# RuurdBijlsma/clip-embedder-rs

Measured on AMD Instinct MI355X. Metric: images/sec embedding, ViT-B/32-224 vision tower, batch 256 per GPU, higher is better.
Workload: dtype bf16; 1 GPU; BASELINE.json configs[1]: ViT-B/32-224 VisionEmbedder, batch 256 synthetic 224x224 per GPU, device-resident input; global_batch=256, seq_len=50, parallelism=dp1, 2 concurrent sub-batch lane(s)/GPU (committed MI355X tile table)

## Files before the change

clip-embedder-rs_amd/csrc/engine/api.hip:

```cpp
#include "engine.hpp"

namespace clipgpu {

namespace {

void destroy_engine(clipgpu_engine* e) {
  for (hipEvent_t ev : e->prof.pool) (void)hipEventDestroy(ev);
  destroy_comms(*e);
  for (auto& r : e->reps) destroy_replica(r);
  delete e;
}

std::unique_lock<std::mutex> device_call(clipgpu_engine* e, int tower, int64_t B, const char* null_arg = nullptr) {
  need_tower(e, tower);
  if (B <= 0) throw ClipErr(CLIPGPU_ERR_INVALID, "Empty batch");
  if (B > e->max_batch) throw ClipErr(CLIPGPU_ERR_INVALID, "B exceeds max_batch");
  if (null_arg) throw ClipErr(CLIPGPU_ERR_INVALID, null_arg);
  std::unique_lock<std::mutex> lk(e->mu);
  HIP_CHECK(hipSetDevice(e->reps[0].device));
  return lk;
}

bool file_exists(const std::string& p) {
  struct stat st;
  return ::stat(p.c_str(), &st) == 0 && S_ISREG(st.st_mode);
}

constexpr int kResidualDefault = CLIPGPU_RESIDUAL_F16;

}

}

using namespace clipgpu;

extern "C" {

int clipgpu_abi_version(void) { return CLIPGPU_ABI_VERSION; }

int clipgpu_options_init(clipgpu_options* o) {
  return guarded([&]() {
    if (!o) throw ClipErr(CLIPGPU_ERR_INVALID, "opts is NULL");
    std::memset(o, 0, sizeof(*o));
    o->struct_size = sizeof(*o);
  });
}

int clipgpu_create(const char* model_dir, int tower, const int* device_ids, int n_devices, int dtype, int max_batch,
                   clipgpu_engine** out) {
  return clipgpu_create_ex(model_dir, tower, device_ids, n_devices, dtype, max_batch, nullptr, out);
}

int clipgpu_create_ex(const char* model_dir, int tower, const int* device_ids, int n_devices, int dtype,
                      int max_batch, const clipgpu_options* opts_in, clipgpu_engine** out) {
  return guarded([&]() {
    if (!out) throw ClipErr(CLIPGPU_ERR_INVALID, "out is NULL");
    *out = nullptr;
    clipgpu_options opts;
    std::memset(&opts, 0, sizeof(opts));
    opts.struct_size = sizeof(opts);
    if (opts_in) {
      if (opts_in->struct_size != offsetof(clipgpu_options, graphs) &&
          opts_in->struct_size != offsetof(clipgpu_options, residual) && opts_in->struct_size != sizeof(opts))
        throw ClipErr(CLIPGPU_ERR_INVALID, "clipgpu_options.struct_size: call clipgpu_options_init first");
      std::memcpy(&opts, opts_in, opts_in->struct_size);
    }
    if (opts.mx_sites & ~(CLIPGPU_MX_QKV | CLIPGPU_MX_FC | CLIPGPU_MX_PROJ))
      throw ClipErr(CLIPGPU_ERR_INVALID, "clipgpu_options.mx_sites: unknown bits");
    if (opts.lanes < 0 || opts.lanes > 4) throw ClipErr(CLIPGPU_ERR_INVALID, "clipgpu_options.lanes must be 0..4");
    if (opts.tuning < 0 || opts.tuning > 2) throw ClipErr(CLIPGPU_ERR_INVALID, "clipgpu_options.tuning must be 0, 1 or 2");
    for (int32_t v : {opts.graphs, opts.prune_last, opts.trim_text})
      if (v < -1 || v > 1) throw ClipErr(CLIPGPU_ERR_INVALID, "clipgpu_options graphs / prune_last / trim_text: -1, 0 or 1");
    for (int i = 0; i < 5; ++i) {
      const int t = i < 4 ? opts.gemm_tiles[i] : opts.patch_tile;
      if (t != 0 && t != -1 && !gemm_tile_built(t))
        throw ClipErr(CLIPGPU_ERR_INVALID, "clipgpu_options.gemm_tiles / patch_tile: " + std::to_string(t) +
                                               " is not a GEMM tile this library builds");
    }
    if (opts.mx_layers != 0 && dtype != CLIPGPU_DTYPE_FP8)
      throw ClipErr(CLIPGPU_ERR_INVALID, "clipgpu_options.mx_layers needs dtype CLIPGPU_DTYPE_FP8");
    if (opts.residual < 0 || opts.residual > CLIPGPU_RESIDUAL_F16)
      throw ClipErr(CLIPGPU_ERR_INVALID, "clipgpu_options.residual must be 0, 1 (f32) or 2 (f16)");
    if (opts.ln_fold < -1 || opts.ln_fold > 1)
      throw ClipErr(CLIPGPU_ERR_INVALID, "clipgpu_options.ln_fold must be -1, 0 or 1");
    if (opts.communicator < 0 || opts.communicator > 1)
      throw ClipErr(CLIPGPU_ERR_INVALID, "clipgpu_options.communicator must be 0 or 1");
    if (!model_dir) throw ClipErr(CLIPGPU_ERR_INVALID, "model_dir is NULL");
    if (tower != CLIPGPU_TOWER_VISION && tower != CLIPGPU_TOWER_TEXT) throw ClipErr(CLIPGPU_ERR_INVALID, "bad tower");
    if (dtype != CLIPGPU_DTYPE_BF16 && dtype != CLIPGPU_DTYPE_F16 && dtype != CLIPGPU_DTYPE_FP8)
      throw ClipErr(CLIPGPU_ERR_INVALID, "bad dtype");
    if (max_batch <= 0) throw ClipErr(CLIPGPU_ERR_INVALID, "max_batch must be > 0");
    const std::string dir(model_dir);
    struct stat st;
    if (::stat(dir.c_str(), &st) != 0 || !S_ISDIR(st.st_mode))
      throw ClipErr(CLIPGPU_ERR_CONFIG, "Model folder not found: '" + dir + "'");
    for (const char* f : {"open_clip_config.json", "model_config.json"})
      if (!file_exists(dir + "/" + f))
        throw ClipErr(CLIPGPU_ERR_CONFIG, std::string("Missing model file '") + f + "' in folder '" + dir + "'");
    OpenClipConfig oc;
    try {
      oc = load_open_clip_config(dir + "/open_clip_config.json");
    } catch (const std::runtime_error& ex) {
      throw ClipErr(CLIPGPU_ERR_CONFIG, ex.what());
    }
    std::unique_ptr<clipgpu_engine, void (*)(clipgpu_engine*)> e(new clipgpu_engine(), destroy_engine);
    e->spec = tower == CLIPGPU_TOWER_VISION ? oc.vision : oc.text;
    e->pre = oc.pre;
    e->dt = dtype == CLIPGPU_DTYPE_F16 ? DT_F16 : DT_BF16;
    e->mx = dtype == CLIPGPU_DTYPE_FP8;
    if (e->mx) {
      const uint32_t bits = opts.mx_sites ? opts.mx_sites : (CLIPGPU_MX_QKV | CLIPGPU_MX_FC | CLIPGPU_MX_PROJ);
      e->mx_site[GS_QKV] = (bits & CLIPGPU_MX_QKV) != 0;
      e->mx_site[GS_FC] = (bits & CLIPGPU_MX_FC) != 0;
      e->mx_site[GS_PROJ] = (bits & CLIPGPU_MX_PROJ) != 0;
      if (e->mx_site[GS_PROJ] && !e->mx_site[GS_FC])
        throw ClipErr(CLIPGPU_ERR_INVALID, "MX sites: proj in MX needs fc in MX");
      if (e->spec.layers < 32 && (opts.mx_layers >> e->spec.layers) != 0)
        throw ClipErr(CLIPGPU_ERR_INVALID, "clipgpu_options.mx_layers: bit set at or beyond the tower's " +
                                               std::to_string(e->spec.layers) + " layers");
      e->mx_layers = opts.mx_layers ? (uint64_t)opts.mx_layers : ~0ull;
    } else if (opts.mx_sites) {
      throw ClipErr(CLIPGPU_ERR_INVALID, "clipgpu_options.mx_sites needs dtype CLIPGPU_DTYPE_FP8");
    }
    e->max_batch = max_batch;
    if (opts.lanes > 0) {
      e->lanes = opts.lanes;
      e->lanes_pinned = true;
    } else {
      e->lanes = 2;
    }
    e->tuning = opts.tuning;
    e->dev_lanes = e->lanes;
    e->graphs = opts.graphs != -1;
    e->prune = opts.prune_last != -1;
    e->trim = opts.trim_text != -1;
    {
      const int res = opts.residual ? opts.residual : kResidualDefault;
      const bool f16_ok = e->spec.family != FAMILY_SIGLIP;
      if (opts.residual == CLIPGPU_RESIDUAL_F16 && !f16_ok)
        throw ClipErr(CLIPGPU_ERR_INVALID, "clipgpu_options.residual = f16: CLIP-family engines only");
      e->x16 = res == CLIPGPU_RESIDUAL_F16 && f16_ok;
      const bool fold_ok = e->x16 && !e->mx && (e->spec.act == ACT_QUICK_GELU || e->spec.act == ACT_GELU);
      if (opts.ln_fold == 1 && !fold_ok)
        throw ClipErr(CLIPGPU_ERR_INVALID,
                      "clipgpu_options.ln_fold = 1: needs a bf16 / f16 engine, the f16 residual stream and a "
                      "QuickGELU / GELU MLP");
      e->lnf = fold_ok && opts.ln_fold != -1;
    }
    for (int i = 0; i < 4; ++i) e->pin_tiles[i] = opts.gemm_tiles[i];
    e->pin_patch = opts.patch_tile;
    const TowerSpec& s = e->spec;
    if (!s.unsupported.empty()) throw ClipErr(CLIPGPU_ERR_CONFIG, s.unsupported);
    if (s.heads <= 0 || s.width % s.heads || s.width % 64)
      throw ClipErr(CLIPGPU_ERR_CONFIG, "Configuration error: width must be a multiple of 64 and of heads");
    const int hd = s.width / s.heads;
    if (hd != 64 && hd != 72 && hd != 80)
      throw ClipErr(CLIPGPU_ERR_CONFIG, "Configuration error: head dim " + std::to_string(hd) + " not supported (64, 72, 80)");
    if (s.width > 1280) throw ClipErr(CLIPGPU_ERR_CONFIG, "Configuration error: width > 1280 not supported yet");
    if (e->mx && (s.width % 128 || mlp_pad(s) % 128))
      throw ClipErr(CLIPGPU_ERR_CONFIG, "Configuration error: the fp8 path needs width and MLP width % 128 == 0");
    if (s.tokens() > 1024) throw ClipErr(CLIPGPU_ERR_CONFIG, "Configuration error: > 1024 tokens not supported yet");
    if (s.tower == TOWER_VISION) {
      if (s.image_size % s.patch_size)
        throw ClipErr(CLIPGPU_ERR_CONFIG, "Configuration error: image_size must be a multiple of patch_size");
      e->in_bytes_per_row = (size_t)3 * s.image_size * s.image_size * 4;
    } else {
      e->in_bytes_per_row = (size_t)s.context_length * 8;
    }
    TensorMap m;
    try {
      m = load_tower_weights(dir, s);
    } catch (const std::runtime_error& ex) {
      throw ClipErr(CLIPGPU_ERR_CONFIG, ex.what());
    }
    int ndev = 0;
    HIP_CHECK(hipGetDeviceCount(&ndev));
    std::vector<int> devs;
    if (device_ids && n_devices > 0) devs.assign(device_ids, device_ids + n_devices);
    else devs.push_back(0);
    for (int d : devs)
      if (d < 0 || d >= ndev) throw ClipErr(CLIPGPU_ERR_DEVICE, "device id " + std::to_string(d) + " not available");
    e->reps.resize(devs.size());
    for (size_t i = 0; i < devs.size(); ++i) {
      Replica& r = e->reps[i];
      r.device = devs[i];
      HIP_CHECK(hipSetDevice(r.device));
      HIP_CHECK(hipStreamCreateWithFlags(&r.stream, hipStreamNonBlocking));
      upload_weights(*e, r, m);
      alloc_workspace(*e, r);
      if (i == 0) {
        if (e->tuning) {
          autotune_tiles(*e, r);
          apply_tile_pins(*e);
          tune_forward(*e, r);
        } else {
          table_tiles(*e);
          apply_tile_pins(*e);
        }
      }
    }
// ... 111 lines not shown
```

clip-embedder-rs_amd/csrc/engine/engine.hpp:

```cpp
#pragma once
#include <hip/hip_runtime.h>
#include <rccl/rccl.h>

#include <algorithm>
#include <cstring>
#include <memory>
#include <mutex>
#include <string>
#include <sys/stat.h>
#include <thread>
#include <vector>

#include "../../../include/clipgpu.h"
#include "../../../include/clipgpu_testing.h"
#include "../bounce.hpp"
#include "../hip_check.hpp"
#include "../host/api_util.hpp"
#include "../host/copy_pool.hpp"
#include "../host/json.hpp"
#include "../host/model.hpp"
#include "../host/resize_plan.hpp"
#include "../kernels/common.hpp"
#include "../kernels/kernels.hpp"


namespace clipgpu {

struct MxW {
  uint8_t* q = nullptr;
  uint8_t* s = nullptr;
};

struct LayerW {
  float *ln1_w, *ln1_b, *bqkv, *bo, *ln2_w, *ln2_b, *b1, *b2;
  float *cs_qkv = nullptr, *cs_1 = nullptr;
  void *wqkv, *wo, *w1, *w2;
  MxW mqkv, m1, m2;
};

struct MapHeadW {
  float* q = nullptr;
  void *wkv = nullptr, *wproj = nullptr, *w1 = nullptr, *w2 = nullptr;
  float *bkv = nullptr, *bproj = nullptr, *norm_w = nullptr, *norm_b = nullptr, *b1 = nullptr, *b2 = nullptr;
};

struct DevWeights {
  void* conv_w = nullptr;
  float* conv_b = nullptr;
  MapHeadW map;
  float *cls = nullptr, *pos = nullptr, *lnpre_w = nullptr, *lnpre_b = nullptr;
  float* tok = nullptr;
  std::vector<LayerW> layers;
  float *lnpost_w = nullptr, *lnpost_b = nullptr;
  void* proj_t = nullptr;
  float* proj_b = nullptr;
};

struct HostSet {
  void* in = nullptr;
  void* pin_in = nullptr;
  float* pin_out = nullptr;
  float* out = nullptr;
  hipEvent_t done[4] = {nullptr, nullptr, nullptr, nullptr};
  hipEvent_t copied[4] = {nullptr, nullptr, nullptr, nullptr};
  bool owns_device = false;
};

struct Replica {
  int device = 0;
  hipStream_t stream = nullptr;
  char* arena = nullptr;
  char* work = nullptr;
  DevWeights w;
  void* x = nullptr;
  float* xs = nullptr;
  void* h = nullptr;
  uint8_t* hs = nullptr;
  uint8_t* bigs = nullptr;
  void* big = nullptr;
  void* pooled = nullptr;
  float* emb = nullptr;
  HostSet hset[2];
  hipStream_t lane[4] = {nullptr, nullptr, nullptr, nullptr};
  hipEvent_t fork = nullptr, join[4] = {nullptr, nullptr, nullptr, nullptr};
  hipStream_t copy = nullptr, copy2 = nullptr;
  struct ImageSlot {
    char* pin = nullptr;
    size_t pin_cap = 0;
    char* dev = nullptr;
    size_t dev_cap = 0;
    uint8_t* tmp = nullptr;
    size_t tmp_cap = 0;
  } islot[4];
  struct GraphCache* graphs = nullptr;
  hipEvent_t gin = nullptr, gout = nullptr;
  ncclComm_t comm = nullptr;
  hipEvent_t coll = nullptr;
};

struct GraphCache {
  struct Entry {
    std::vector<uint64_t> key;
    hipGraphExec_t exec;
    uint64_t last_use;
  };
  std::vector<Entry> entries;
  uint64_t clock = 0;
  static constexpr size_t kMax = 32;
  void clear() {
    for (auto& en : entries) (void)hipGraphExecDestroy(en.exec);
    entries.clear();
  }
};

enum ProfCat { PC_PATCH = 0, PC_STEM, PC_QKV, PC_ATTN, PC_OUT_PROJ, PC_LN, PC_C_FC, PC_C_PROJ, PC_HEAD, PC_TAIL, PC_N };
struct Profiler {
  unsigned mask = 0;
  std::vector<hipEvent_t> pool;
  size_t used = 0;
  struct Rec { int cat; hipEvent_t a, b; hipStream_t st; };
  std::vector<Rec> pending;
  double total_ms[PC_N] = {0};
  long long count[PC_N] = {0};
  hipEvent_t get() {
    if (used == pool.size()) {
      hipEvent_t ev;
      if (hipEventCreate(&ev) != hipSuccess) return nullptr;
      pool.push_back(ev);
    }
    return pool[used++];
  }
};

}

struct clipgpu_engine {
  clipgpu::Profiler prof;
  int tile[4] = {0, 0, 0, 0};
  int mxtile[4] = {0, 0, 0, 0};
  int tile_patch = 0;
  int tuned_rows = 0;
  int lanes = 1;
  int dev_lanes = 1;
  bool lanes_pinned = false;
  bool graphs = true;
  bool prune = true;
  bool trim = true;
  bool x16 = false;
  bool lnf = false;

  int tuning = 0;
  int pin_tiles[4] = {0, 0, 0, 0};
  int pin_patch = 0;
  uint64_t mx_layers = ~0ull;
  bool comm_pending = false;
  std::vector<int> comm_devs;
  bool force_bcast = false;
  std::vector<int> host_part;
  bool rgb8_resize_always = false;
  clipgpu::TowerSpec spec;
  clipgpu::PreprocessCfg pre;
  clipgpu::DType dt = clipgpu::DT_BF16;
  bool mx = false;
  bool mx_site[4] = {false, false, false, false};
  int max_batch = 0;
  size_t in_bytes_per_row = 0;
  std::vector<clipgpu::Replica> reps;
  int comm_nranks = 0, comm_rank0 = 0;
  std::mutex mu;
};

#pragma GCC visibility push(hidden)
namespace clipgpu {

enum GemmSite { GS_QKV = 0, GS_OUT, GS_FC, GS_PROJ, GS_N };

inline bool mx_at(const clipgpu_engine& e, int l, int site) {
  return e.mx_site[site] && l >= 0 && l < 64 && ((e.mx_layers >> l) & 1ull);
}

inline size_t align256(size_t n) { return (n + 255) & ~size_t(255); }
inline int round64(int n) { return (n + 63) / 64 * 64; }
inline int mlp_pad(const TowerSpec& s) { return round64(s.mlp_width); }
inline int kpatch(const TowerSpec& s) { return 3 * s.patch_size * s.patch_size; }
inline int kpatch_pad(const TowerSpec& s) { return round64(kpatch(s)); }
inline size_t big_wide(const TowerSpec& s) {
  size_t w = std::max((size_t)3 * s.width, (size_t)mlp_pad(s));
  if (s.tower == TOWER_VISION) {
    const size_t G = (size_t)s.image_size / s.patch_size, T = (size_t)s.tokens();
    w = std::max(w, (G * G * (size_t)kpatch_pad(s) + T - 1) / T);
  }
  return w;
}

inline size_t xbytes(const clipgpu_engine& e) { return e.x16 ? 2 : 4; }
inline void* xrows(const clipgpu_engine& e, void* x, size_t rows) {
  return (char*)x + rows * (size_t)e.spec.width * xbytes(e);
}

enum InKind { IN_F32 = 0, IN_U8 = 1, IN_IDS = 2 };

struct HostRows {
// ... 115 lines not shown
```

clip-embedder-rs_amd/csrc/engine/forward.hip:

```cpp
#include "engine.hpp"

namespace clipgpu {

namespace {

struct ProfScope {
  Profiler* p;
  int cat;
  hipStream_t st;
  bool gemm;
  hipEvent_t a = nullptr, b = nullptr;
  ProfScope(const clipgpu_engine& e, int c, hipStream_t s, bool gemm_scope = false)
      : p(const_cast<Profiler*>(&e.prof)), cat(c), st(s), gemm(gemm_scope) {
    if (p->mask & (1u << cat)) {
      a = p->get();
      b = a ? p->get() : nullptr;
      if (!b) {
        a = nullptr;
      } else if (gemm) {
        g_gemm_events.start = a;
        g_gemm_events.stop = b;
      } else {
        (void)hipEventRecord(a, st);
      }
// ... 7 lines not shown
  }
};

GemmParams rows_gemm(const void* A, long lda, const void* W, const float* bias, void* out, long ldo, int M, int N,
                     int K) {
  GemmParams g{};
  g.A = A;
  g.lda = lda;
  g.W = W;
  g.ldw = K;
  g.bias = bias;
  g.out = out;
  g.ldo = ldo;
  g.M = M;
  g.N = N;
  g.K = K;
  return g;
}

}

SiteShape site_shape(const clipgpu_engine& e, int site) {
  const int D = e.spec.width, MLP = mlp_pad(e.spec);
  switch (site) {
    case GS_QKV: return {3 * D, D};
    case GS_OUT: return {D, D};
    case GS_FC: return {MLP, D};
    default: return {D, MLP};
  }
}

int site_epi(const clipgpu_engine& e, int site) {
  if (site == GS_OUT || site == GS_PROJ) return EPI_RESID;
  return e.lnf ? EPI_LNF : EPI_STORE16;
}

#ifndef CLIPGPU_SITE_GROUPS
#define CLIPGPU_SITE_GROUPS 1
#endif
constexpr int kSiteGroup[4] = {CLIPGPU_SITE_GROUPS ? 1 : 0, 0, 0, CLIPGPU_SITE_GROUPS ? 1 : 0};

GemmParams site_gemm(const clipgpu_engine& e, const Replica& r, const LayerW& L, int site, int rows) {
  const int D = e.spec.width, MLP = mlp_pad(e.spec);
  GemmParams g;
  const void* ln_in = e.lnf ? r.x : r.h;
  switch (site) {
    case GS_QKV: g = rows_gemm(ln_in, D, L.wqkv, L.bqkv, r.big, 3 * D, rows, 3 * D, D); break;
    case GS_OUT: g = rows_gemm(r.h, D, L.wo, L.bo, r.x, D, rows, D, D); break;
    case GS_FC: g = rows_gemm(ln_in, D, L.w1, L.b1, r.big, MLP, rows, MLP, D); break;
    default: g = rows_gemm(r.big, MLP, L.w2, L.b2, r.x, D, rows, D, MLP); break;
  }
  if (e.lnf && (site == GS_QKV || site == GS_FC)) {
    g.cs = site == GS_QKV ? L.cs_qkv : L.cs_1;
    g.rowstats = r.xs;
  }
  g.group = kSiteGroup[site];
  g.x16 = e.x16 ? 1 : 0;
  g.prio = e.spec.tower == TOWER_VISION ? 1 : 0;
  return g;
}

int site_epi_mx(const clipgpu_engine& e, int l, int site) {
  return site == GS_PROJ ? EPI_RESID : (site == GS_FC && mx_at(e, l, GS_PROJ) ? EPI_STOREQ : EPI_STORE16);
}
static inline uint8_t* ln_q(const clipgpu_engine& e, int l, int consumer_site, uint8_t* hs) {
  return mx_at(e, l, consumer_site) ? hs : nullptr;
}

MxGemmParams site_gemm_mx(const clipgpu_engine& e, const Replica& r, const LayerW& L, int site, int rows) {
  const int D = e.spec.width, MLP = mlp_pad(e.spec);
  MxGemmParams g{};
  g.M = rows;
  if (site == GS_PROJ) {
    g.A = (const uint8_t*)r.big; g.lda = MLP; g.As = r.bigs; g.ldas = MLP / 32;
    g.W = L.m2.q; g.ldw = MLP; g.Ws = L.m2.s; g.ldws = MLP / 32;
    g.bias = L.b2; g.out = r.x; g.ldo = D; g.N = D; g.K = MLP;
    g.x16 = e.x16 ? 1 : 0;
    return g;
  }
  g.A = (const uint8_t*)r.h; g.lda = D; g.As = r.hs; g.ldas = D / 32;
  g.K = D;
  if (site == GS_QKV) {
    g.W = L.mqkv.q; g.ldw = D; g.Ws = L.mqkv.s; g.ldws = D / 32;
    g.bias = L.bqkv; g.out = r.big; g.ldo = 3 * D; g.N = 3 * D;
  } else {
    g.W = L.m1.q; g.ldw = D; g.Ws = L.m1.s; g.ldws = D / 32;
    g.bias = L.b1; g.out = r.big; g.ldo = MLP; g.outs = r.bigs; g.ldos = MLP / 32; g.N = MLP;
  }
  return g;
}

#ifdef CLIPGPU_ABLATE
unsigned g_ablate = 0;
#define ABLATED(bit) ((g_ablate >> (bit)) & 1u)
extern "C" int clipgpu_test_ablate(unsigned mask) {
  g_ablate = mask;
  return 0;
}
#else
#define ABLATED(bit) false
#endif

namespace {

struct PoolSrc {
  const void* x;
  int tokens;
  const int64_t* ids;
};

inline size_t prune_off_x(const TowerSpec& s, int B) { return align256((size_t)B * mlp_pad(s) * 2); }
inline size_t prune_off_h(const TowerSpec& s, int B) {
  return prune_off_x(s, B) + align256((size_t)B * s.width * 4);
}
inline size_t prune_off_xs(const TowerSpec& s, int B) {
  return prune_off_h(s, B) + align256((size_t)B * s.width * 2);
}
inline bool prune_last(const clipgpu_engine& e, int B, int T) {
  const TowerSpec& s = e.spec;
  return e.prune && s.family != FAMILY_SIGLIP && s.layers > 0 &&
         prune_off_xs(s, B) + ((size_t)B + 256) * 8 <= (size_t)B * T * big_wide(s) * 2;
}

PoolSrc trunk(const clipgpu_engine& e, const Replica& r, int B, int causal, const int64_t* ids, hipStream_t st,
              int T, int pool_pos = 0) {
  const TowerSpec& s = e.spec;
  const int D = s.width;
  const bool prune = prune_last(e, B, T);
  for (int l = 0; l < s.layers; ++l) {
    const LayerW& L = r.w.layers[l];
    const bool compact = prune && l + 1 == s.layers;
    Replica c = r;
    int rows = B * T;
    auto gemm = [&](int site, int cat, const char* what) {
      if (ABLATED(site == GS_QKV ? 3 : site == GS_OUT ? 2 : site == GS_FC ? 4 : 5)) return;
      ProfScope ps(e, rows == B * T ? cat : PC_TAIL, st, true);
      const bool tuned = 2 * rows > e.tuned_rows;
      if (mx_at(e, l, site)) {
        MxGemmParams g = site_gemm_mx(e, c, L, site, rows);
        g.tile = tuned ? e.mxtile[site] : MX_TILE_AUTO;
        check(launch_gemm_mx(e.dt, site_epi_mx(e, l, site), site == GS_FC ? s.act : ACT_NONE, g, st), what);
        return;
      }
      GemmParams g = site_gemm(e, c, L, site, rows);
      g.tile = tuned ? e.tile[site] : TILE_AUTO;
      check(launch_gemm(e.dt, A_ROWS, site_epi(e, site), site == GS_FC ? s.act : ACT_NONE, g, st), what);
    };
    gemm(GS_QKV, PC_QKV, "qkv gemm");
    if (!ABLATED(1)) { ProfScope ps(e, PC_ATTN, st);
      check(launch_attention(e.dt, r.big, r.h, B, T, s.heads, D, causal, st), "attention"); }
    if (compact) {
      c.x = (char*)r.big + prune_off_x(s, B);
      c.h = (char*)r.big + prune_off_h(s, B);
      c.xs = (float*)((char*)r.big + prune_off_xs(s, B));
      rows = B;
      ProfScope ps(e, PC_TAIL, st);
      check(launch_gather_pooled(xrows(e, r.x, pool_pos), e.x16, (char*)r.h + (size_t)pool_pos * D * 2, ids, T, c.x, c.h,
                                 B, D, st),
            "gather pooled rows");
    }
    gemm(GS_OUT, PC_OUT_PROJ, "out_proj gemm");
    if (!ABLATED(0)) {
      ProfScope ps(e, compact ? PC_TAIL : PC_LN, st);
      if (e.lnf)
        check(launch_ln_stats(c.x, 1, s.ln_eps, c.xs, rows, D, st), "ln_2 statistics");
      else
        check(launch_ln_rows(e.dt, c.x, e.x16, L.ln2_w, L.ln2_b, s.ln_eps, c.h, rows, D, st, ln_q(e, l, GS_FC, c.hs)),
              "ln_2");
    }
    gemm(GS_FC, PC_C_FC, "c_fc gemm");
    gemm(GS_PROJ, PC_C_PROJ, "c_proj gemm");
    if (l + 1 < s.layers && !ABLATED(0)) {
      ProfScope ps(e, PC_LN, st);
      if (e.lnf)
        check(launch_ln_stats(r.x, 1, s.ln_eps, r.xs, rows, D, st), "ln_1 statistics");
      else
        check(launch_ln_rows(e.dt, r.x, e.x16, r.w.layers[l + 1].ln1_w, r.w.layers[l + 1].ln1_b, s.ln_eps, r.h, rows,
                             D, st, ln_q(e, l + 1, GS_QKV, r.hs)),
              "ln_1");
    }
    if (compact) return PoolSrc{c.x, 1, nullptr};
  }
  return PoolSrc{xrows(e, r.x, pool_pos), T, ids};
}

void head(const clipgpu_engine& e, const Replica& r, int B, const PoolSrc& src, float* d_out, hipStream_t st) {
  const TowerSpec& s = e.spec;
  const int D = s.width, E = s.embed_dim;
  ProfScope ps(e, PC_HEAD, st);
  check(launch_pool_ln(e.dt, src.x, e.x16, src.ids, src.tokens, r.w.lnpost_w, r.w.lnpost_b, s.ln_eps, r.pooled, B, D,
                       st),
        "pool+ln");
  check(launch_gemm(e.dt, A_ROWS, EPI_STORE32, ACT_NONE, rows_gemm(r.pooled, D, r.w.proj_t, r.w.proj_b, r.emb, E, B, E, D),
                    st),
        "proj gemm");
  check(launch_l2norm(r.emb, d_out, B, E, st), "l2norm");
}

void head_map(const clipgpu_engine& e, const Replica& r, int B, float* d_out, hipStream_t st) {
  const TowerSpec& s = e.spec;
  const int D = s.width, T = s.tokens(), M = mlp_pad(s);
  const MapHeadW& mw = r.w.map;
  ProfScope ps(e, PC_HEAD, st);
  check(launch_ln_rows(e.dt, r.x, 0, r.w.lnpost_w, r.w.lnpost_b, s.ln_eps, r.h, B * T, D, st), "norm");
  check(launch_gemm(e.dt, A_ROWS, EPI_STORE16, ACT_NONE, rows_gemm(r.h, D, mw.wkv, mw.bkv, r.big, 2 * D, B * T, 2 * D, D),
                    st), "attn_pool kv gemm");
  check(launch_map_attention(e.dt, mw.q, r.big, r.pooled, B, T, s.heads, D, st), "attn_pool attention");
  check(launch_gemm(e.dt, A_ROWS, EPI_STORE32, ACT_NONE, rows_gemm(r.pooled, D, mw.wproj, mw.bproj, r.x, D, B, D, D), st),
        "attn_pool proj gemm");
  check(launch_ln_rows(e.dt, r.x, 0, mw.norm_w, mw.norm_b, s.ln_eps, r.h, B, D, st), "attn_pool norm");
  check(launch_gemm(e.dt, A_ROWS, EPI_STORE16, s.act, rows_gemm(r.h, D, mw.w1, mw.b1, r.big, M, B, M, D), st),
        "attn_pool fc1 gemm");
  check(launch_gemm(e.dt, A_ROWS, EPI_RESID, ACT_NONE, rows_gemm(r.big, M, mw.w2, mw.b2, r.x, D, B, D, M), st),
        "attn_pool fc2 gemm");
  check(launch_l2norm((const float*)r.x, d_out, B, D, st), "l2norm");
}

}

GemmParams patch_gemm(const clipgpu_engine& e, const Replica& r, int rows) {
  const TowerSpec& s = e.spec;
  const int Kp = kpatch_pad(s);
  GemmParams g = rows_gemm(r.big, Kp, r.w.conv_w, r.w.conv_b, r.x, s.width, rows, s.width, Kp);
  g.G = s.grid();
  g.pos = r.w.pos;
  g.cls = s.cls() ? 1 : 0;
  g.x16 = e.x16 ? 1 : 0;
  return g;
}

void vision_forward(const clipgpu_engine& e, const Replica& r, const void* pixels, int asrc, const float* mean,
                    const float* stdv, int B, float* d_out, hipStream_t st) {
  const TowerSpec& s = e.spec;
  const int D = s.width, G = s.grid(), P = s.patch_size, Kp = kpatch_pad(s);
  { ProfScope ps(e, PC_PATCH, st);
    check(launch_patch_rows(e.dt, asrc, pixels, mean, stdv, r.big, B, s.image_size, P, kpatch(s), Kp, st),
          "patch rows");
    GemmParams g = patch_gemm(e, r, B * G * G);
    g.tile = 2 * B * s.tokens() > e.tuned_rows ? e.tile_patch : TILE_AUTO;
    check(launch_gemm(e.dt, A_ROWS, EPI_PATCH, ACT_NONE, g, st), "patch gemm"); }
  if (s.family == FAMILY_SIGLIP) {
    { ProfScope ps(e, PC_STEM, st);
      check(launch_ln_rows(e.dt, r.x, e.x16, r.w.layers[0].ln1_w, r.w.layers[0].ln1_b, s.ln_eps, r.h, B * s.tokens(), D, st,
                           ln_q(e, 0, GS_QKV, r.hs)),
            "ln_1"); }
    trunk(e, r, B, 0, nullptr, st, s.tokens());
    head_map(e, r, B, d_out, st);
    return;
  }
  {
  ProfScope ps(e, PC_STEM, st);
  check(launch_vision_embed_ln(e.dt, r.x, e.x16, r.w.cls, r.w.pos, r.w.lnpre_w, r.w.lnpre_b, r.w.layers[0].ln1_w,
                               r.w.layers[0].ln1_b, s.ln_eps, e.lnf ? nullptr : r.h, B, s.tokens(), D, st,
                               ln_q(e, 0, GS_QKV, r.hs), r.xs),
        "embed+ln_pre");
  }
  head(e, r, B, trunk(e, r, B, 0, nullptr, st, s.tokens()), d_out, st);
}

void text_forward(const clipgpu_engine& e, const Replica& r, const int64_t* d_ids, int B, float* d_out,
                  hipStream_t st, int T) {
  const TowerSpec& s = e.spec;
  if (T <= 0) T = s.context_length;
  {
  ProfScope ps(e, PC_STEM, st);
  check(launch_text_embed_ln(e.dt, d_ids, r.w.tok, r.w.pos, r.w.layers[0].ln1_w, r.w.layers[0].ln1_b, s.ln_eps,
                             r.x, e.x16, e.lnf ? nullptr : r.h, B, T, s.width, s.vocab_size, st,
                             ln_q(e, 0, GS_QKV, r.hs), r.xs),
        "token embed+ln_1");
  }
  head(e, r, B, trunk(e, r, B, s.causal ? 1 : 0, s.pool_last ? nullptr : d_ids, st, T, s.pool_last ? T - 1 : 0),
       d_out, st);
}

Replica lane_view(const clipgpu_engine& e, const Replica& r, int b0) {
  const TowerSpec& s = e.spec;
  const size_t rows = (size_t)b0 * s.tokens(), D = s.width;
  const size_t wide = big_wide(s);
  Replica v = r;
  v.x = (char*)r.x + rows * D * xbytes(e);
  v.xs = r.xs + rows * 2;
  v.h = (char*)r.h + rows * D * 2;
  v.big = (char*)r.big + rows * wide * 2;
  if (r.hs) v.hs = r.hs + rows * D / 32;
  if (r.bigs) v.bigs = r.bigs + rows * (size_t)mlp_pad(s) / 32;
  v.pooled = (char*)r.pooled + (size_t)b0 * D * 2;
  v.emb = r.emb + (size_t)b0 * s.embed_dim;
  return v;
}

namespace {

inline void lane_range(int B, int lanes, int i, int& b0, int& b1) {
  b0 = (int)((long)B * i / lanes);
  b1 = (int)((long)B * (i + 1) / lanes);
}

inline int lanes_for(const clipgpu_engine& e, int B) {
  return B < 8 * e.dev_lanes ? 1 : e.dev_lanes;
}

template <typename F>
void run_lanes(const clipgpu_engine& e, const Replica& r, int B, hipStream_t st, F fwd) {
  const int L = lanes_for(e, B);
  const bool serial = e.prof.mask != 0 && !(e.prof.mask & CLIPGPU_PROFILE_CONCURRENT);
  if (L == 1 || serial) {
    for (int i = 0; i < L; ++i) {
      int b0, b1;
      lane_range(B, L, i, b0, b1);
      fwd(lane_view(e, r, b0), b0, b1 - b0, st);
    }
    return;
  }
  HIP_CHECK(hipEventRecord(r.fork, st));
  for (int i = 0; i < L; ++i) {
    int b0, b1;
    lane_range(B, L, i, b0, b1);
    HIP_CHECK(hipStreamWaitEvent(r.lane[i], r.fork, 0));
    fwd(lane_view(e, r, b0), b0, b1 - b0, r.lane[i]);
    HIP_CHECK(hipEventRecord(r.join[i], r.lane[i]));
  }
  for (int i = 0; i < L; ++i) HIP_CHECK(hipStreamWaitEvent(st, r.join[i], 0));
}

}

void vision_forward_lanes(const clipgpu_engine& e, const Replica& r, const void* pixels, int asrc, const float* mean,
                          const float* stdv, int B, float* d_out, hipStream_t st) {
  const size_t S = e.spec.image_size;
  const size_t row_bytes = 3 * S * S * (asrc == A_IMG_F32 ? 4 : 1);
  const int E = e.spec.embed_dim;
  run_lanes(e, r, B, st, [&](const Replica& v, int b0, int n, hipStream_t ls) {
    vision_forward(e, v, (const char*)pixels + b0 * row_bytes, asrc, mean, stdv, n, d_out + (size_t)b0 * E, ls);
  });
// ... 12 lines not shown
```

clip-embedder-rs_amd/csrc/engine/weights.hip:

```cpp
#include "engine.hpp"

namespace clipgpu {

namespace {

const HostTensor& need(const TensorMap& m, const std::string& k) {
  auto it = m.find(k);
  if (it == m.end()) throw ClipErr(CLIPGPU_ERR_CONFIG, "Configuration error: missing tensor " + k);
  return it->second;
}

struct Bump {
  char* base;
  size_t off = 0;
  size_t cap;
  void* take(size_t n) {
    void* p = base + off;
    off += align256(n);
    if (off > cap) throw ClipErr(CLIPGPU_ERR_DEVICE, "internal: arena overflow");
    return p;
  }
};

size_t weight_bytes(const TowerSpec& s, const TensorMap& m) {
// ... 189 lines not shown
    w.layers.push_back(L);
  }
  if (siglip) {
    const std::string t = "visual.trunk.", a = "visual.trunk.attn_pool.";
    w.lnpost_w = f32(t + "norm.weight");
    w.lnpost_b = f32(t + "norm.bias");
    {
      const HostTensor& lat = need(m, a + "latent");
      const HostTensor& wq = need(m, a + "q.weight");
      const HostTensor& bq = need(m, a + "q.bias");
      std::vector<float> q((size_t)D);
      for (int j = 0; j < D; ++j) {
        double acc = bq.data[(size_t)j];
        for (int i = 0; i < D; ++i) acc += (double)lat.data[(size_t)i] * wq.data[(size_t)j * D + i];
        q[(size_t)j] = (float)acc;
      }
      w.map.q = (float*)a_take_f32(q);
    }
    w.map.wkv = w16(a + "kv.weight");
    w.map.bkv = f32(a + "kv.bias");
    w.map.wproj = w16(a + "proj.weight");
    w.map.bproj = f32(a + "proj.bias");
    w.map.norm_w = f32(a + "norm.weight");
    w.map.norm_b = f32(a + "norm.bias");
    w.map.w1 = w16_pad(a + "mlp.fc1.weight", mlp_pad(s), D);
    w.map.b1 = f32_pad(a + "mlp.fc1.bias", mlp_pad(s));
    w.map.w2 = w16_pad(a + "mlp.fc2.weight", D, mlp_pad(s));
    w.map.b2 = f32(a + "mlp.fc2.bias");
  } else if (s.tower == TOWER_VISION) {
    w.lnpost_w = f32("visual.ln_post.weight");
    w.lnpost_b = f32("visual.ln_post.bias");
    w.proj_t = w16_transposed("visual.proj");
  } else {
    w.lnpost_w = f32("ln_final.weight");
    w.lnpost_b = f32("ln_final.bias");
    if (s.proj_bias) {
      w.proj_t = w16("text_projection.weight");
      w.proj_b = f32("text_projection.bias");
    } else {
      w.proj_t = w16_transposed("text_projection");
    }
  }
}

void alloc_workspace(clipgpu_engine& e, Replica& r) {
  const TowerSpec& s = e.spec;
  const size_t B = (size_t)((e.max_batch + e.lanes - 1) / e.lanes * e.lanes);
  const size_t rows = B * (size_t)s.tokens(), D = s.width;
  const size_t wide = big_wide(s);
  const size_t E = s.embed_dim;
  const size_t MLP = (size_t)mlp_pad(s);
  const size_t sizes[] = {rows * D * 4, rows * D * 2, rows * wide * 2, B * D * 2, B * E * 4, B * E * 4,
                          B * e.in_bytes_per_row, e.mx ? rows * D / 32 : 0, e.mx ? rows * MLP / 32 : 0,
                          (rows + 256) * 8};
  size_t total = 0;
  for (size_t z : sizes) total += align256(z);
  HIP_CHECK(hipMalloc(&r.work, total));
  HIP_CHECK(hipMemset(r.work, 0, total));
  Bump a{r.work, 0, total};
  r.x = a.take(sizes[0]);
  r.h = a.take(sizes[1]);
  r.big = a.take(sizes[2]);
  r.pooled = a.take(sizes[3]);
  r.emb = (float*)a.take(sizes[4]);
  HostSet& hs = r.hset[0];
  hs.out = (float*)a.take(sizes[5]);
  hs.in = a.take(sizes[6]);
  r.hs = e.mx ? (uint8_t*)a.take(sizes[7]) : nullptr;
  r.bigs = e.mx ? (uint8_t*)a.take(sizes[8]) : nullptr;
  r.xs = (float*)a.take(sizes[9]);
  for (int i = 0; i < e.lanes; ++i) {
    HIP_CHECK(hipStreamCreateWithFlags(&r.lane[i], hipStreamNonBlocking));
    HIP_CHECK(hipEventCreateWithFlags(&r.join[i], hipEventDisableTiming));
  }
  for (int i = 0; i < 4; ++i) {
    HIP_CHECK(hipEventCreateWithFlags(&hs.done[i], hipEventDisableTiming));
    HIP_CHECK(hipEventCreateWithFlags(&hs.copied[i], hipEventDisableTiming));
  }
  HIP_CHECK(hipStreamCreateWithFlags(&r.copy, hipStreamNonBlocking));
  HIP_CHECK(hipStreamCreateWithFlags(&r.copy2, hipStreamNonBlocking));
  HIP_CHECK(hipEventCreateWithFlags(&r.fork, hipEventDisableTiming));
  HIP_CHECK(hipEventCreateWithFlags(&r.gin, hipEventDisableTiming));
  HIP_CHECK(hipEventCreateWithFlags(&r.gout, hipEventDisableTiming));
  r.graphs = new GraphCache();
  HIP_CHECK(hipHostMalloc(&hs.pin_in, B * e.in_bytes_per_row, hipHostMallocDefault));
  HIP_CHECK(hipHostMalloc((void**)&hs.pin_out, B * E * 4, hipHostMallocDefault));
}

void destroy_replica(Replica& r) {
  if (!r.stream) return;
  (void)hipSetDevice(r.device);
  (void)hipDeviceSynchronize();
  if (r.arena) (void)hipFree(r.arena);
  if (r.work) (void)hipFree(r.work);
  for (HostSet& hs : r.hset) {
    if (hs.pin_in) (void)hipHostFree(hs.pin_in);
    if (hs.pin_out) (void)hipHostFree(hs.pin_out);
    if (hs.owns_device && hs.in) (void)hipFree(hs.in);
    if (hs.owns_device && hs.out) (void)hipFree(hs.out);
  }
  if (r.stream) (void)hipStreamDestroy(r.stream);
  if (r.copy) (void)hipStreamDestroy(r.copy);
  if (r.copy2) (void)hipStreamDestroy(r.copy2);
  for (int i = 0; i < 4; ++i) {
    if (r.lane[i]) (void)hipStreamDestroy(r.lane[i]);
    if (r.join[i]) (void)hipEventDestroy(r.join[i]);
    for (HostSet& hs : r.hset) {
      if (hs.done[i]) (void)hipEventDestroy(hs.done[i]);
      if (hs.copied[i]) (void)hipEventDestroy(hs.copied[i]);
    }
  }
  if (r.fork) (void)hipEventDestroy(r.fork);
  if (r.gin) (void)hipEventDestroy(r.gin);
  if (r.gout) (void)hipEventDestroy(r.gout);
  if (r.coll) (void)hipEventDestroy(r.coll);
  if (r.graphs) {
    r.graphs->clear();
    delete r.graphs;
  }
  for (auto& sl : r.islot) {
    if (sl.pin) (void)hipHostFree(sl.pin);
    if (sl.dev) (void)hipFree(sl.dev);
    if (sl.tmp) (void)hipFree(sl.tmp);
// ... 6 lines not shown
```

clip-embedder-rs_amd/csrc/kernels/common.hpp:

```cpp
#pragma once
#include <hip/hip_runtime.h>
#include <stdint.h>

namespace clipgpu {

typedef float f32x4 __attribute__((ext_vector_type(4)));
typedef float f32x16 __attribute__((ext_vector_type(16)));
typedef __bf16 bf16x8 __attribute__((ext_vector_type(8)));
typedef _Float16 f16x8 __attribute__((ext_vector_type(8)));
typedef __bf16 bf16x4 __attribute__((ext_vector_type(4)));
typedef _Float16 f16x4 __attribute__((ext_vector_type(4)));

template <typename T> struct Vec8;
template <> struct Vec8<__bf16> { typedef bf16x8 type; };
template <> struct Vec8<_Float16> { typedef f16x8 type; };
template <typename T> struct Vec4;
template <> struct Vec4<__bf16> { typedef bf16x4 type; };
template <> struct Vec4<_Float16> { typedef f16x4 type; };

__device__ __forceinline__ float4 ldx4(const float* p) { return *(const float4*)p; }
__device__ __forceinline__ float4 ldx4(const _Float16* p) {
  const f16x4 h = *(const f16x4*)p;
  return make_float4((float)h[0], (float)h[1], (float)h[2], (float)h[3]);
}
// ... 37 lines not shown
  return e < 127 ? __uint_as_float((uint32_t)(127 - e) << 23) : __uint_as_float(0x00400000u);
}
__device__ __forceinline__ uint32_t mx_pack4(float a, float b, float c, float d, float inv) {
  int w = __builtin_amdgcn_cvt_pk_fp8_f32(a * inv, b * inv, 0, false);
  w = __builtin_amdgcn_cvt_pk_fp8_f32(c * inv, d * inv, w, true);
  return (uint32_t)w;
}

template <int CTRL>
__device__ __forceinline__ float dpp_f32(float v) {
  return __builtin_bit_cast(float, __builtin_amdgcn_update_dpp(0, __builtin_bit_cast(int, v), CTRL, 0xF, 0xF, false));
}
__device__ __forceinline__ float row16_sum(float v) {
  v += dpp_f32<0x128>(v);
  v += dpp_f32<0x124>(v);
  v += dpp_f32<0x122>(v);
  v += dpp_f32<0x121>(v);
  return v;
}
__device__ __forceinline__ float row16_max(float v) {
  v = fmaxf(v, dpp_f32<0x128>(v));
  v = fmaxf(v, dpp_f32<0x124>(v));
  v = fmaxf(v, dpp_f32<0x122>(v));
  v = fmaxf(v, dpp_f32<0x121>(v));
  return v;
}
__device__ __forceinline__ void swap16(float& a, float& b) {
  asm volatile("s_nop 1\n\tv_permlane16_swap_b32 %0, %1" : "+v"(a), "+v"(b));
}
__device__ __forceinline__ void swap32(float& a, float& b) {
  asm volatile("s_nop 1\n\tv_permlane32_swap_b32 %0, %1" : "+v"(a), "+v"(b));
}
__device__ __forceinline__ float xsum16(float v) {
  float a = v, b = v;
  swap16(a, b);
  return a + b;
}
__device__ __forceinline__ float xsum32(float v) {
  float a = v, b = v;
  swap32(a, b);
  return a + b;
}
__device__ __forceinline__ float xmax16(float v) {
  float a = v, b = v;
  swap16(a, b);
  return fmaxf(a, b);
}
__device__ __forceinline__ float xmax32(float v) {
  float a = v, b = v;
  swap32(a, b);
  return fmaxf(a, b);
}
__device__ __forceinline__ float wave_sum(float v) { return xsum32(xsum16(row16_sum(v))); }
__device__ __forceinline__ float wave_max(float v) { return xmax32(xmax16(row16_max(v))); }
__device__ __forceinline__ float group16_sum(float v) { return row16_sum(v); }
__device__ __forceinline__ float group16_max(float v) { return row16_max(v); }

typedef float f32x2 __attribute__((ext_vector_type(2)));
__device__ __forceinline__ float lnf_out(float acc, float mean, float rstd, float cs, float bias) {
  return fmaf(fmaf(-mean, cs, acc), rstd, bias);
}

enum Act { ACT_NONE = 0, ACT_QUICK_GELU = 1, ACT_GELU = 2, ACT_GELU_TANH = 3 };

__device__ __forceinline__ float fast_sigmoid_mul(float x, float z) {
  return x * __builtin_amdgcn_rcpf(1.0f + __expf(-z));
}
__device__ __forceinline__ float sigmoid_mul_exp2(float x, float t) {
  return x * __builtin_amdgcn_rcpf(1.0f + __builtin_amdgcn_exp2f(t));
}
__device__ __forceinline__ float fast_erf(float x) {
  const float ax = fabsf(x);
  const float t = __builtin_amdgcn_rcpf(fmaf(0.3275911f, ax, 1.0f));
  float p = fmaf(1.061405429f, t, -1.453152027f);
  p = fmaf(p, t, 1.421413741f);
  p = fmaf(p, t, -0.284496736f);
  p = fmaf(p, t, 0.254829592f);
  const float y = 1.0f - p * t * __expf(-ax * ax);
  return copysignf(y, x);
}

template <int ACT>
__device__ __forceinline__ float apply_act(float x) {
#ifdef CLIPGPU_TEST_NO_ACT
  return x;
#endif
  if constexpr (ACT == ACT_QUICK_GELU) {
    return sigmoid_mul_exp2(x, x * -2.4554669596f);
  } else if constexpr (ACT == ACT_GELU) {
    return 0.5f * x * (1.0f + fast_erf(x * 0.70710678118654752f));
  } else if constexpr (ACT == ACT_GELU_TANH) {
    const float k0 = 0.7978845608028654f, k1 = 0.044715f;
    return fast_sigmoid_mul(x, 2.0f * k0 * fmaf(k1 * x, x * x, x));
  } else {
    return x;
  }
}

__device__ __forceinline__ int xcd_remap(int pid, int nwg) {
  const int xcd = pid & 7, q = nwg >> 3, r = nwg & 7;
  const int start = xcd < r ? xcd * (q + 1) : r * (q + 1) + (xcd - r) * q;
  return start + (pid >> 3);
}

}
```

clip-embedder-rs_amd/csrc/kernels/gemm.hip:

```cpp
#include <algorithm>
#include <cstdlib>
#include <type_traits>
#include <utility>

#include <hip/hip_ext.h>

#include "common.hpp"
#include "kernels.hpp"
#include "gemm_util.hpp"

namespace clipgpu {

thread_local GemmLaunchEvents g_gemm_events;

#ifdef CLIPGPU_GEMM_STAMPS
constexpr int kStampBlocks = 2048, kStampSlots = 64;
__device__ unsigned long long g_gemm_stamps[kStampBlocks * kStampSlots];
#define GEMM_STAMP(slot)                                                                        \
  do {                                                                                          \
    if (threadIdx.x == 0 && blockIdx.x < kStampBlocks && (slot) < kStampSlots)                   \
      g_gemm_stamps[blockIdx.x * kStampSlots + (slot)] = __builtin_amdgcn_s_memtime();        \
  } while (0)
#define GEMM_STAMP_REAL(slot)                                                                   \
  do {                                                                                          \
// ... 36 lines not shown
#define CLIPGPU_GEMM_SPREAD_ALL 0
#endif
#ifndef CLIPGPU_GEMM_NONPERSIST
#define CLIPGPU_GEMM_NONPERSIST 0
#endif
#ifndef CLIPGPU_GEMM_EPI_DMA_WAIT
#define CLIPGPU_GEMM_EPI_DMA_WAIT 1
#endif

template <typename T>
__device__ __forceinline__ T to16(float v) { return (T)v; }
__device__ __forceinline__ float4 widen4(float4 v) { return v; }
__device__ __forceinline__ float4 widen4(f16x4 h) { return make_float4((float)h[0], (float)h[1], (float)h[2], (float)h[3]); }

template <int NW, int OCC>
struct PipeBounds {
  static constexpr int waves_per_eu = NW == 8 && OCC >= 2 ? 4 : 2;
};

template <typename T, int BM, int BN, int WGM, int WGN, int EPI, int ACT, int NS = 2, int OCC = 2, int RS = 0,
          int HM = 0>
__global__ __launch_bounds__(WGM* WGN * 64, (PipeBounds<WGM * WGN, OCC>::waves_per_eu)) void gemm_pipe_kernel(
    GemmParams p) {
  typedef typename Vec8<T>::type V8;
  constexpr bool LNF = epi_lnf(EPI);
  static_assert(!LNF || std::is_same<T, _Float16>::value, "LayerNorm fold: f16 operands");
  typedef typename std::conditional<EPI == EPI_LNF_BF, __bf16, T>::type OT;
  constexpr int SROWP = LNF ? (BM * 8 + 1023) / 1024 * 1024 : 0;
  constexpr int EXTRA = LNF ? 4096 + 2 * SROWP : 2048;
  constexpr int NW = WGM * WGN;
  constexpr int A_BYTES = BM * BK * 2, B_BYTES = BN * BK * 2, STAGE = A_BYTES + B_BYTES;
  constexpr int PW = BN / 8, PA = BM / 8, PT = PW + PA;
  constexpr int NP = (PT + NW - 1) / NW;
  constexpr bool EVEN = PT % NW == 0;
  constexpr bool WSPLIT = PW % NW == 0;
  constexpr int TM = BM / WGM, TN = BN / WGN, MI = TM / 16, NI = TN / 16;
  constexpr int LG = NI == 2 ? 1 : NI == 4 ? 2 : 3;
  constexpr int NG = MI;
  constexpr bool SPREAD = MI * NI >= 32 || (CLIPGPU_GEMM_SPREAD_W8 && NW == 8 && OCC < 2) || CLIPGPU_GEMM_SPREAD_ALL;
  (void)LG;
  static_assert(BM % 8 == 0 && BN % 8 == 0 && MI >= 1 && BN <= 256 && PT >= NW, "bad tile");
  static_assert(NI == 2 || NI == 3 || NI == 4 || NI == 6 || NI == 8, "column permutation: NI in {2,3,4,6,8}");
  static_assert(NS == 2 || NS == 3, "2 or 3 LDS stages");
  __shared__ __attribute__((aligned(16))) char smem[NS * STAGE + EXTRA];

  const int tid = threadIdx.x;
  const int lane = tid & 63;
  const int wave = __builtin_amdgcn_readfirstlane(tid >> 6);
  const int lda_i = (int)p.lda, ldw_i = (int)p.ldw, nb = gridDim.x;
  const char* const Ab = (const char*)p.A;
  const char* const Wb = (const char*)p.W;
  const float* const bias_p = p.bias;
  const float* const cs_p = p.cs;
  const float* const rs_p = p.rowstats;
  asm volatile("" ::"s"(lda_i), "s"(ldw_i), "s"(nb), "s"(Ab), "s"(Wb), "s"(bias_p));
  if constexpr (LNF) asm volatile("" ::"s"(cs_p), "s"(rs_p));
  const int nTn = (p.N + BN - 1) / BN;
  const int grp = p.group > 0 ? p.group : CLIPGPU_TILE_GROUP;
  asm volatile("" ::"s"(grp));
  const int nTm = (p.M + BM - 1) / BM;
  const int ntiles = nTn * nTm;
  const int nk = p.K / BK;

  static_assert(!HM || (NS == 2 && WGM == 2), "half tiles: 2 x N waves, 2-stage schedule");
  int t_first, t_stride, t_end;
  int hm_F = 0, hm_start = 0, hm_nbx = 1, hm_j = 0;
  if constexpr (HM) {
    const int x = blockIdx.x & 7, nbx = nb >> 3, j = blockIdx.x >> 3;
    const int q = ntiles >> 3, r = ntiles & 7;
    hm_start = x < r ? x * (q + 1) : r * (q + 1) + (x - r) * q;
    const int cnt = q + (x < r ? 1 : 0);
    hm_F = cnt / nbx;
    hm_nbx = nbx;
    hm_j = j;
    t_first = 0;
    t_stride = 1;
    t_end = hm_F + (j < 2 * (cnt % nbx) ? 1 : 0);
  } else if (nb % 8 == 0 && nb < ntiles) {
    const int x = blockIdx.x & 7, nbx = nb >> 3;
    const int q = ntiles >> 3, r = ntiles & 7;
    const int start = x < r ? x * (q + 1) : r * (q + 1) + (x - r) * q;
    t_first = start + (blockIdx.x >> 3);
    t_stride = nbx;
    t_end = start + q + (x < r ? 1 : 0);
  } else {
    t_first = xcd_remap(blockIdx.x, nb);
    t_stride = ntiles;
    t_end = t_first + 1;
  }
  if (t_first >= t_end) return;
  const int total = ((t_end - t_first + t_stride - 1) / t_stride) * nk;
  auto unit_coords = [&](int u, int& m0, int& n0) {
    if constexpr (HM) {
      if (u < hm_F) {
        tile_coords(hm_start + hm_j + u * hm_nbx, nTm, nTn, BM, BN, m0, n0, grp);
      } else {
        tile_coords(hm_start + hm_F * hm_nbx + (hm_j >> 1), nTm, nTn, BM, BN, m0, n0, grp);
        m0 += (hm_j & 1) * (BM / 2);
      }
      return;
    }
    tile_coords(u, nTm, nTn, BM, BN, m0, n0, grp);
  };

  auto swW = [](int r) {
    if constexpr (NI == 3 || NI == 6) {
      const int j = (r % (16 * NI)) / (4 * NI);
      return ((j == 1 || j == 2) ? 1 : 0) ^ (2 * j + ((r & 3) >> 1));
    } else {
// ... 3 lines not shown

  uint32_t poff[NP];
  auto piece_is_w = [&](int i, int q) { return WSPLIT ? (i < PW / NW) : (q < PW); };
  auto set_tile = [&](int m0, int n0) {
#pragma unroll
    for (int i = 0; i < NP; ++i) {
      const int q = wave + NW * i;
      if (!EVEN && q >= PT) {
        poff[i] = 0;
      } else if (piece_is_w(i, q)) {
        const int r = q * 8 + (lane >> 3);
        const int c = (lane & 7) ^ swW(r);
        poff[i] = (uint32_t)(min(n0 + r, p.N - 1) * ldw_i + c * 8) * 2u;
      } else {
        const int r = (q - PW) * 8 + (lane >> 3);
        const int c = (lane & 7) ^ ((r >> 1) & 7);
        poff[i] = (uint32_t)(min(m0 + r, p.M - 1) * lda_i + c * 8) * 2u;
      }
    }
  };
  int d_g = 0, d_kt = 0, d_t = t_first, d_n0 = 0, d_m0 = 0, d_ti = 0;
  {
    int m0, n0;
    unit_coords(d_t, m0, n0);
    set_tile(m0, n0);
    d_n0 = n0;
    d_m0 = m0;
  }
  const bool last_piece = EVEN || wave < PT % NW;
  int d_stage = 0;
  auto dma_piece = [&](auto ic) {
    constexpr int i = decltype(ic)::value;
    if constexpr (!EVEN && i == NP - 1) {
      if (!last_piece) return;
    }
#ifdef CLIPGPU_GEMM_STAMPS
    if (p.diag & 4) return;
#endif
    const int q = wave + NW * i;
    const bool w = piece_is_w(i, q);
    char* const dst = smem + d_stage * STAGE + (w ? A_BYTES + q * 1024 : (q - PW) * 1024);
    const char* const src = (w ? Wb : Ab) + (size_t)d_kt * (BK * 2);
    GEMM_POISON(dst);
    glds16(src + poff[i], dst);
  };
  auto dma_bias = [&]() {
    if (bias_p != nullptr && wave == 0 && d_kt == 0) {
      const int n = min(d_n0 + lane * 4, ((p.N - 1) / 4) * 4);
      GEMM_POISON(smem + NS * STAGE + (d_ti & 1) * 1024);
      glds16(bias_p + n, smem + NS * STAGE + (d_ti & 1) * 1024);
      if constexpr (LNF) {
        GEMM_POISON(smem + NS * STAGE + 2048 + (d_ti & 1) * 1024);
        glds16(cs_p + n, smem + NS * STAGE + 2048 + (d_ti & 1) * 1024);
        char* const sst = smem + NS * STAGE + 4096 + (d_ti & 1) * SROWP;
#pragma unroll
        for (int i = 0; i < SROWP / 1024; ++i) {
          GEMM_POISON(sst + i * 1024);
          glds16(rs_p + (size_t)d_m0 * 2 + i * 256 + lane * 4, sst + i * 1024);
        }
      }
    }
  };
  auto dma_advance = [&]() {
    ++d_g;
    if (++d_stage == NS) d_stage = 0;
    if (++d_kt == nk) {
      d_kt = 0;
      d_t += t_stride;
      ++d_ti;
      if (d_t < t_end) {
        int m0, n0;
        unit_coords(d_t, m0, n0);
        set_tile(m0, n0);
        d_n0 = n0;
        d_m0 = m0;
      }
    }
  };
  auto dma_step = [&]() {
    if (d_g < total) {
      static_for<NP>([&](auto j) { dma_piece(j); });
      dma_bias();
    }
    dma_advance();
  };

  const int wm = (wave / WGN) * TM, wn = (wave % WGN) * TN;
  const int fr = lane & 15, fq = lane >> 4;
  uint32_t offA[2], offB[2];
  {
    const int rowB = wn + (fr >> 2) * (4 * NI) + (fr & 3);
#pragma unroll
    for (int kk = 0; kk < 2; ++kk) {
      offA[kk] = (uint32_t)((wm + fr) * 128 + (((kk * 4 + fq) ^ (fr >> 1)) << 4));
      offB[kk] = (uint32_t)(A_BYTES + rowB * 128 + (((kk * 4 + fq) ^ swW(rowB)) << 4));
    }
  }
  int wm_cur = wm, mi_lim = MI;
  uint32_t offA_cur[2] = {offA[0], offA[1]};
  auto set_layout = [&](int u) {
    if constexpr (HM) {
      const bool half = u >= hm_F;
      wm_cur = half ? (wave / WGN) * (TM / 2) : wm;
      mi_lim = half ? MI / 2 : MI;
#pragma unroll
      for (int kk = 0; kk < 2; ++kk) offA_cur[kk] = offA[kk] - (uint32_t)((wm - wm_cur) * 128);
    }
    (void)u;
  };
  const uint32_t lds0 = lds_addr(smem);
  f32x4 acc[NI][MI];
  V8 a0[MI], b0[NI], a1[MI], b1[NI];

  auto rd_b = [&](auto kc, V8(&b)[NI], uint32_t buf, int kk) {
    constexpr int k = decltype(kc)::value;
    ds_read_b128<k * 512>(b[k], buf + offB[kk]);
  };
  auto rd_a = [&](auto kc, V8(&a)[MI], uint32_t buf, int kk) {
    constexpr int k = decltype(kc)::value;
    ds_read_b128<k * 2048>(a[k], buf + offA_cur[kk]);
  };
  auto read_b = [&](V8(&b)[NI], uint32_t buf, int kk) { static_for<NI>([&](auto k) { rd_b(k, b, buf, kk); }); };
  auto read_a = [&](V8(&a)[MI], uint32_t buf, int kk) { static_for<MI>([&](auto k) { rd_a(k, a, buf, kk); }); };
  constexpr int NR = NI + MI, RG = RS ? (NG > 2 ? NG - 2 : 1) : NG, RPG = (NR + RG - 1) / RG;
  auto read_k = [&](auto kc, V8(&a)[MI], V8(&b)[NI], uint32_t buf, int kk) {
    constexpr int k = decltype(kc)::value;
    if constexpr (k < NI) rd_b(kc, b, buf, kk);
    else rd_a(std::integral_constant<int, k - NI>{}, a, buf, kk);
  };
  auto reads_after_group = [&](auto gc, V8(&a)[MI], V8(&b)[NI], uint32_t buf, int kk) {
    static_for<RPG>([&](auto j) {
      constexpr int k = (int)decltype(gc)::value * RPG + (int)decltype(j)::value;
      if constexpr ((int)decltype(gc)::value < RG && k < NR) read_k(std::integral_constant<int, k>{}, a, b, buf, kk);
    });
  };
  auto mfma_group = [&](auto gc, V8(&a)[MI], V8(&b)[NI], auto zero) {
    constexpr int g = decltype(gc)::value;
    constexpr bool Z = decltype(zero)::value;
    if (!HM || g < mi_lim) {
#pragma unroll
      for (int ni = 0; ni < NI; ++ni)
        acc[ni][g] = mfma_16x16x32(b[ni], a[g], Z ? f32x4{0.f, 0.f, 0.f, 0.f} : acc[ni][g]);
    }
  };
  auto phase0 = [&](auto zero, uint32_t buf) {
    if constexpr (!RS) read_b(b1, buf, 1);
    static_for<NG>([&](auto g) {
      mfma_group(g, a0, b0, zero);
      __builtin_amdgcn_sched_barrier(0);
      if constexpr (RS) {
        reads_after_group(g, a1, b1, buf, 1);
        __builtin_amdgcn_sched_barrier(0);
      } else {
        rd_a(g, a1, buf, 1);
      }
    });
    lgkm_wait_all(a1, b1);
  };
  auto phase1 = [&](bool next, uint32_t nbuf) {
    const bool dma = d_g < total;
    (void)next;
    if constexpr (!RS) read_b(b0, nbuf, 0);
    if (dma) {
      dma_bias();
      if constexpr (!SPREAD) static_for<NP>([&](auto j) { dma_piece(j); });
    }
    static_for<NG>([&](auto g) {
      mfma_group(g, a1, b1, std::false_type{});
      __builtin_amdgcn_sched_barrier(0);
      if constexpr (RS) reads_after_group(g, a0, b0, nbuf, 0);
      else rd_a(g, a0, nbuf, 0);
      if constexpr (SPREAD) {
        static_for<NP>([&](auto j) {
          if constexpr (((int)j * NG) / NP == (int)g) {
            if (dma) dma_piece(j);
          }
        });
      }
      __builtin_amdgcn_sched_barrier(0);
    });
    dma_advance();
    lgkm_wait_all(a0, b0);
  };

  auto epilogue = [&](int m0, int n0, int bpar) {
    typedef typename std::conditional<epi_x16(EPI), _Float16, float>::type XE;
    const int nc = n0 + wn + fq * (4 * NI);
    const bool nfull = nc + 4 * NI <= p.N;
    f32x4 bias[NI], csv[NI];
    constexpr bool RST_ALL = MI * NI < 32;
    f32x2 rst[RST_ALL ? MI : 1];
    const uint32_t rst_a = lds0 + NS * STAGE + 4096 + bpar * SROWP + (wm_cur + fr) * 8;
#pragma unroll
    for (int ni = 0; ni < NI; ++ni) bias[ni] = f32x4{0.f, 0.f, 0.f, 0.f};
    if (bias_p != nullptr) {
      const uint32_t ba = lds0 + NS * STAGE + bpar * 1024 + (wn + fq * (4 * NI)) * 4;
      static_for<NI>([&](auto ni) { ds_read_b128<(int)ni * 16>(bias[ni], ba); });
      if constexpr (LNF) {
        static_for<NI>([&](auto ni) { ds_read_b128<2048 + (int)ni * 16>(csv[ni], ba); });
        if constexpr (RST_ALL) static_for<MI>([&](auto mi) { ds_read_b64<(int)mi * 128>(rst[mi], rst_a); });
      }
      asm volatile("s_waitcnt lgkmcnt(0)" ::: "memory");
#pragma unroll
      for (int ni = 0; ni < NI; ++ni) asm volatile("" : "+v"(bias[ni]));
      if constexpr (LNF) {
#pragma unroll
        for (int ni = 0; ni < NI; ++ni) asm volatile("" : "+v"(csv[ni]));
        if constexpr (RST_ALL) {
#pragma unroll
          for (int mi = 0; mi < MI; ++mi) asm volatile("" : "+v"(rst[mi]));
        }
      }
    }
    constexpr bool ADDX = epi_resid(EPI) || epi_patch(EPI);
    const int G2 = p.G * p.G;
    auto out_row = [&](int m) -> long {
// ... 42 lines not shown
        if constexpr (RST_ALL) {
          rs = rst[mi];
        } else {
          asm volatile("ds_read_b64 %0, %1\n\ts_waitcnt lgkmcnt(0)" : "=v"(rs) : "v"(rst_a + (uint32_t)mi * 128) : "memory");
        }
      }
      float v[NI][4];
#pragma unroll
      for (int ni = 0; ni < NI; ++ni)
#pragma unroll
        for (int j = 0; j < 4; ++j)
          v[ni][j] = LNF ? lnf_out(acc[ni][mi][j], rs[0], rs[1], csv[ni][j], bias[ni][j])
                         : acc[ni][mi][j] + bias[ni][j];
#ifdef CLIPGPU_GEMM_STAMPS
      if (p.diag & 1) {
        float s = 0.f;
#pragma unroll
        for (int ni = 0; ni < NI; ++ni)
#pragma unroll
          for (int j = 0; j < 4; ++j) s += EPI == EPI_STORE16 ? (float)to16<T>(apply_act<ACT>(v[ni][j])) : v[ni][j];
        if (s == 12345.678f) ((float*)p.out)[0] = s;
        continue;
      }
#endif
      if constexpr (epi_st16(EPI)) {
        OT* o = (OT*)p.out + (long)m * p.ldo + nc;
        if (nfull) {
          if constexpr (NI % 2 == 0) {
#pragma unroll
            for (int h = 0; h < NI / 2; ++h) {
              typename Vec8<OT>::type w;
#pragma unroll
              for (int e = 0; e < 8; ++e) w[e] = to16<OT>(apply_act<ACT>(v[2 * h + e / 4][e % 4]));
              *(typename Vec8<OT>::type*)(o + h * 8) = w;
            }
          } else {
#pragma unroll
            for (int ni = 0; ni < NI; ++ni) {
              typename Vec4<OT>::type w;
#pragma unroll
              for (int j = 0; j < 4; ++j) w[j] = to16<OT>(apply_act<ACT>(v[ni][j]));
              *(typename Vec4<OT>::type*)(o + ni * 4) = w;
            }
          }
        } else {
#pragma unroll
          for (int ni = 0; ni < NI; ++ni)
#pragma unroll
            for (int j = 0; j < 4; ++j)
              if (nc + ni * 4 + j < p.N) o[ni * 4 + j] = to16<OT>(apply_act<ACT>(v[ni][j]));
        }
      } else {
        XE* o = (XE*)p.out + out_row(m) + nc;
        if (nfull) {
#pragma unroll
          for (int ni = 0; ni < NI; ++ni) {
            float4 w = make_float4(v[ni][0], v[ni][1], v[ni][2], v[ni][3]);
            if constexpr (ADDX) {
              const float4 x = widen4(xr[XALL ? mi : mi % XR][ni]);
              w.x += x.x; w.y += x.y; w.z += x.z; w.w += x.w;
            }
            stx4(o + ni * 4, w);
          }
        } else {
#pragma unroll
          for (int ni = 0; ni < NI; ++ni)
#pragma unroll
            for (int j = 0; j < 4; ++j) {
              if (nc + ni * 4 + j >= p.N) continue;
              float r = v[ni][j];
              if constexpr (ADDX) r += (float)add_src(m)[ni * 4 + j];
              o[ni * 4 + j] = (XE)r;
            }
        }
      }
    }
  };
  constexpr int EPI_VM = epi_st16(EPI) ? (NI % 2 ? MI * NI : MI * NI / 2)
                                            : ((epi_resid(EPI) || epi_patch(EPI)) ? 2 * MI * NI : MI * NI);
  auto vm_wait_step = [&](auto xc) {
    constexpr int X = decltype(xc)::value;
    if (EVEN || wave < PT % NW) vm_wait<(NP + X < 63 ? NP + X : 63)>();
    else vm_wait<(NP - 1 + X < 63 ? NP - 1 + X : 63)>();
  };

  GEMM_STAMP_REAL(62);
  GEMM_STAMP_HWID();
  GEMM_STAMP(0);
  if constexpr (NW == 8) {
    if (p.prio && wave >= NW / 2) __builtin_amdgcn_s_setprio(1);
  }
  dma_step();
  vm_wait<0>();
  __builtin_amdgcn_s_barrier();
  dma_step();
  if constexpr (NS == 3) dma_step();
  read_b(b0, lds0, 0);
  read_a(a0, lds0, 0);
  lgkm_wait_all(a0, b0);
  GEMM_STAMP(1);

  int g = 0;
  int gs = 0;
  bool after_full_epi = false;
  int ti = 0;
  for (int t = t_first; t < t_end; t += t_stride, ++ti) {
    int m0, n0;
    unit_coords(t, m0, n0);
    GEMM_STAMP(2 + ti * 4);
    for (int kt = 0; kt < nk; ++kt, ++g) {
      if (kt + 1 == nk) GEMM_STAMP(3 + ti * 4);
      const int gs1 = gs + 1 == NS ? 0 : gs + 1;
      const uint32_t buf = lds0 + gs * STAGE;
      if (kt == 0) phase0(std::true_type{}, buf);
      else phase0(std::false_type{}, buf);
      constexpr int EW = EPI_VM < 63 ? EPI_VM : 63;
      if (NS == 3 && g + 2 < total) {
        if (after_full_epi) vm_wait_step(std::integral_constant<int, EPI_VM>{});
        else vm_wait_step(std::integral_constant<int, 0>{});
      } else {
#if CLIPGPU_GEMM_POISON_SELFTEST
        (void)EW;
#else
        if (after_full_epi) vm_wait<EW>();
        else vm_wait<0>();
#endif
      }
      after_full_epi = false;
#ifdef CLIPGPU_GEMM_STAMPS
      if (!(p.diag & 8)) __builtin_amdgcn_s_barrier();
#else
      __builtin_amdgcn_s_barrier();
#endif
      phase1(kt + 1 < nk, lds0 + gs1 * STAGE);
      gs = gs1;
      if (ti == 0 && kt + 1 < nk && 34 + kt < 61) GEMM_STAMP(34 + kt);
    }
    GEMM_STAMP(4 + ti * 4);
#if CLIPGPU_GEMM_EPI_DMA_WAIT
    if constexpr (NS == 3) vm_wait_step(std::integral_constant<int, 0>{});
    else vm_wait<0>();
#endif
    epilogue(m0, n0, ti & 1);
    after_full_epi = m0 + BM <= p.M && n0 + BN <= p.N && (!HM || t < hm_F);
    if (!after_full_epi) vm_wait<0>();
    if (t + t_stride < t_end) {
      const uint32_t buf = lds0 + gs * STAGE;
      set_layout(t + t_stride);
      read_b(b0, buf, 0);
      read_a(a0, buf, 0);
      lgkm_wait_all(a0, b0);
    }
    GEMM_STAMP(5 + ti * 4);
  }
  GEMM_STAMP_REAL(63);
}

constexpr int pipe_kocc(int NW, int OCC) { return NW == 8 ? (OCC >= 2 ? 2 : 1) : 2; }
inline int pipe_grid(int BM, int BN, int NW, int OCC, int M, int N) {
  const int ntiles = ((N + BN - 1) / BN) * ((M + BM - 1) / BM);
  const int lds = 2 * (BM + BN) * BK * 2 + 2048;
  const int per_cu = std::max(1, std::min(NW == 8 ? pipe_kocc(NW, OCC) : OCC, (160 * 1024) / lds));
  const int resident = device_cus() * per_cu;
  if (CLIPGPU_GEMM_NONPERSIST) return ntiles;
  return ntiles <= resident ? ntiles : resident;
}
inline bool half_round_applies(int M, int N) {
  const int nb = device_cus();
  const int ntiles = ((N + 255) / 256) * ((M + 255) / 256);
  bool ok = nb % 8 == 0 && ntiles % nb != 0;
  const int nbx = nb >> 3, q = ntiles >> 3, r = ntiles & 7;
  for (int x = 0; ok && x < 8; ++x) {
    const int cnt = q + (x < r ? 1 : 0);
    ok = cnt >= nbx && 2 * (cnt % nbx) <= nbx;
  }
  return ok;
}
inline int grid_224(int M, int N) { return std::min(((N + 191) / 192) * ((M + 223) / 224), device_cus()); }

template <typename T, int BM, int BN, int WGM, int WGN, int EPI, int ACT, int OCC = 3, int RS = 0>
hipError_t launch_pipe(const GemmParams& p, hipStream_t s) {
// ... 29 lines not shown
  static_assert(!LNF || std::is_same<T, _Float16>::value, "LayerNorm fold: f16 operands");
  static_assert(!epi_patch(EPI), "the patch GEMM always has K >= 128 (pipelined tiles)");
  typedef typename std::conditional<EPI == EPI_LNF_BF, __bf16, T>::type OT;
  const int lane = threadIdx.x & 63;
  const long wid = (long)blockIdx.x * 4 + (threadIdx.x >> 6);
  const int nTn = GEN ? (p.N + 15) >> 4 : p.N >> 4;
  const long tm = wid / nTn;
  const int tn = (int)(wid - tm * nTn);
  if (tm * 16 >= p.M) return;
  const int fr = lane & 15, fq = lane >> 4;
  const int m = (int)tm * 16 + fr;
  const T* a = (const T*)p.A + (long)min(m, p.M - 1) * p.lda + fq * 8;
  const T* w = (const T*)p.W + (long)(GEN ? min(tn * 16 + fr, p.N - 1) : tn * 16 + fr) * p.ldw + fq * 8;
  const int nc = p.K >> 5;
  V8 w0[U], a0[U], w1[U], a1[U], w2[U], a2[U];
  auto load = [&](V8(&wv)[U], V8(&av)[U], int c) {
#pragma unroll
    for (int u = 0; u < U; ++u) {
      wv[u] = *(const V8*)(w + (c + u) * 32);
      av[u] = *(const V8*)(a + (c + u) * 32);
    }
  };
  load(w0, a0, 0);
  if (U < nc) load(w1, a1, U);
  f32x4 acc = {0.f, 0.f, 0.f, 0.f};
  for (int c0 = 0; c0 < nc; c0 += U) {
    if (c0 + 2 * U < nc) load(w2, a2, c0 + 2 * U);
#pragma unroll
    for (int u = 0; u < U; ++u) acc = mfma_16x16x32(w0[u], a0[u], acc);

#pragma unroll
    for (int u = 0; u < U; ++u) {
      w0[u] = w1[u];
      a0[u] = a1[u];
      w1[u] = w2[u];
      a1[u] = a2[u];
    }
  }
  if (m >= p.M) return;
  const int n = tn * 16 + fq * 4;
  if (GEN && n >= p.N) return;
  const bool vec = !GEN || (n + 4 <= p.N && p.ldo % 4 == 0);
  f32x4 bias = {0.f, 0.f, 0.f, 0.f}, csv = {0.f, 0.f, 0.f, 0.f};
  f32x2 rst = {0.f, 0.f};
  if (p.bias != nullptr) {
    if (!GEN || n + 4 <= p.N) bias = *(const f32x4*)(p.bias + n);
    else
      for (int j = 0; j < 4; ++j) bias[j] = n + j < p.N ? p.bias[n + j] : 0.f;
  }
  if constexpr (LNF) {
    if (!GEN || n + 4 <= p.N) csv = *(const f32x4*)(p.cs + n);
    else
      for (int j = 0; j < 4; ++j) csv[j] = n + j < p.N ? p.cs[n + j] : 0.f;
    rst = *(const f32x2*)(p.rowstats + (long)m * 2);
  }
  float v[4];
#pragma unroll
  for (int j = 0; j < 4; ++j) v[j] = LNF ? lnf_out(acc[j], rst[0], rst[1], csv[j], bias[j]) : acc[j] + bias[j];
  if constexpr (epi_st16(EPI)) {
    OT* o = (OT*)p.out + (long)m * p.ldo + n;
    if (vec) {
      typename Vec4<OT>::type ov;
#pragma unroll
      for (int j = 0; j < 4; ++j) ov[j] = to16<OT>(apply_act<ACT>(v[j]));
      *(typename Vec4<OT>::type*)o = ov;
    } else {
      for (int j = 0; j < 4; ++j)
        if (n + j < p.N) o[j] = to16<OT>(apply_act<ACT>(v[j]));
    }
  } else {
    typedef typename std::conditional<epi_x16(EPI), _Float16, float>::type XE;
    XE* o = (XE*)p.out + (long)m * p.ldo + n;
    if (vec) {
      float4 r = make_float4(v[0], v[1], v[2], v[3]);
      if constexpr (epi_resid(EPI)) {
        const float4 x = ldx4(o);
        r.x += x.x; r.y += x.y; r.z += x.z; r.w += x.w;
      }
      stx4(o, r);
    } else {
      for (int j = 0; j < 4; ++j) {
        if (n + j >= p.N) continue;
        float r = v[j];
        if constexpr (epi_resid(EPI)) r += (float)o[j];
        o[j] = (XE)r;
      }
    }
  }
}

inline bool skinny_ok(const GemmParams& p) {
  return p.M > 0 && p.M <= SKINNY_MAX_M && p.N % 16 == 0 && p.K % (32 * SKINNY_U) == 0 && p.lda % 8 == 0 &&
         p.ldw % 8 == 0 && p.ldo % 4 == 0;
}
inline bool general_ok(const GemmParams& p) { return p.lda % 8 == 0 && p.ldw % 8 == 0; }
inline long skinny_waves(int M, int N) { return (long)((M + 15) / 16) * ((N + 15) / 16); }

template <typename T, int EPI, int ACT, int U = SKINNY_U, int GEN = 0>
hipError_t launch_skinny(const GemmParams& p, hipStream_t s) {
  const long blocks = (skinny_waves(p.M, p.N) + 3) / 4;
  if (blocks > 0x7fffffffL) return hipErrorInvalidValue;
  gemm_launch(gemm_skinny_kernel<T, EPI, ACT, U, GEN>, (int)blocks, 256, s, p);
  return hipGetLastError();
}

template <typename T, int EPI, int ACT>
hipError_t launch_tile(const GemmParams& p, hipStream_t s) {
  if constexpr (!epi_patch(EPI)) {
    if ((p.tile == TILE_AUTO || p.tile == TILE_SKINNY) && skinny_ok(p)) return launch_skinny<T, EPI, ACT>(p, s);
  }
  if (p.tile == TILE_SKINNY) return hipErrorInvalidValue;
  const int tile = p.tile == TILE_AUTO ? pick_gemm_tile(p.M, p.N, p.K) : p.tile;
  if (tile != TILE_GENERAL && !gemm_tile_built(tile)) return hipErrorInvalidValue;
  const bool pipe = tile != TILE_GENERAL && p.K >= 2 * BK && (!epi_st16(EPI) || p.ldo % 8 == 0);
  if (!pipe) {
    if constexpr (epi_patch(EPI)) {
      return hipErrorInvalidValue;
    } else {
      if (!general_ok(p)) return hipErrorInvalidValue;
      return launch_skinny<T, EPI, ACT, 2, 1>(p, s);
    }
  }
  if constexpr (epi_lnf(EPI)) {
    switch (tile) {
      case TILE_256x128: return launch_pipe<T, 256, 128, 4, 2, EPI, ACT>(p, s);
      case TILE_256x256: return launch_pipe<T, 256, 256, 2, 4, EPI, ACT>(p, s);
      case TILE_192x256_W8: return launch_pipe<T, 192, 256, 2, 4, EPI, ACT, 1>(p, s);
      case TILE_256x256_RS: return launch_pipe<T, 256, 256, 2, 4, EPI, ACT, 3, 1>(p, s);
      case TILE_160x128_RS: return launch_pipe<T, 160, 128, 2, 2, EPI, ACT, 3, 1>(p, s);
      case TILE_160x128_W8_RS: return launch_pipe<T, 160, 128, 2, 4, EPI, ACT, 2, 1>(p, s);
      case TILE_256x256_HALF: return launch_pipe_half<T, EPI, ACT>(p, s);
      case TILE_224x192_W8: return launch_pipe<T, 160, 128, 2, 2, EPI, ACT, 3, 1>(p, s);
      default: break;
    }
  } else {
    switch (tile) {
      case TILE_256x128: return launch_pipe<T, 256, 128, 4, 2, EPI, ACT>(p, s);
      case TILE_256x256: return launch_pipe<T, 256, 256, 2, 4, EPI, ACT>(p, s);
      case TILE_192x256_W8: return launch_pipe<T, 192, 256, 2, 4, EPI, ACT, 1>(p, s);
      case TILE_256x256_RS: return launch_pipe<T, 256, 256, 2, 4, EPI, ACT, 3, 1>(p, s);
      case TILE_160x128_RS: return launch_pipe<T, 160, 128, 2, 2, EPI, ACT, 3, 1>(p, s);
      case TILE_160x128_W8_RS: return launch_pipe<T, 160, 128, 2, 4, EPI, ACT, 2, 1>(p, s);
      case TILE_256x256_HALF: return launch_pipe_half<T, EPI, ACT>(p, s);
      case TILE_224x192_W8: return launch_pipe_224<T, EPI, ACT>(p, s);
      default: break;
    }
  }
  return hipErrorInvalidValue;
}

template <typename T>
hipError_t launch_typed(int epi, int act, const GemmParams& p, hipStream_t s) {
  switch (epi) {
    case EPI_STORE16:
      switch (act) {
        case ACT_NONE: return launch_tile<T, EPI_STORE16, ACT_NONE>(p, s);
// ... 46 lines not shown

int gemm_grid(int tile, int M, int N, int K) {
  GemmParams p{};
  p.M = M;
  p.N = N;
  p.K = K;
  p.lda = p.ldw = K;
  p.ldo = N;
  if ((tile == TILE_AUTO || tile == TILE_SKINNY) && skinny_ok(p)) return (int)((skinny_waves(M, N) + 3) / 4);
  if (tile == TILE_AUTO) tile = pick_gemm_tile(M, N, K);
  if (K >= 2 * BK && tile != TILE_GENERAL) {
    switch (tile) {
      case TILE_256x128: return pipe_grid(256, 128, 8, 3, M, N);
      case TILE_256x256: return pipe_grid(256, 256, 8, 3, M, N);
      case TILE_192x256_W8: return pipe_grid(192, 256, 8, 1, M, N);
      case TILE_256x256_RS: return pipe_grid(256, 256, 8, 3, M, N);
      case TILE_160x128_RS: return pipe_grid(160, 128, 4, 3, M, N);
      case TILE_160x128_W8_RS: return pipe_grid(160, 128, 8, 2, M, N);
      case TILE_256x256_HALF: return half_round_applies(M, N) ? device_cus() : pipe_grid(256, 256, 8, 3, M, N);
      case TILE_224x192_W8: return grid_224(M, N);
      default: break;
    }
  }
  return (int)std::min<long>((skinny_waves(M, N) + 3) / 4, 0x7fffffffL);
}

int pick_gemm_tile(int M, int N, int K) {
  (void)K;
  if (M < 2048) return TILE_160x128_RS;
  const int cus = 256;
  auto eff = [&](int bm, int bn) {
    const long tiles = (long)((M + bm - 1) / bm) * ((N + bn - 1) / bn);
    const long rounds = (tiles + cus - 1) / cus;
    return (double)tiles / (double)(rounds * cus);
  };
  return eff(256, 256) >= 0.85 * eff(256, 128) ? TILE_256x256 : TILE_256x128;
}

long g_gemm_chunk_cap = 0;

long gemm_chunk_rows(long lda, int G) {
  long rows = ((1L << 31) - 1) / (2 * lda);
  if (g_gemm_chunk_cap > 0) rows = std::min(rows, g_gemm_chunk_cap);
  rows -= rows % 256;
  if (G > 0) rows -= rows % ((long)G * G);
  return rows;
}

hipError_t launch_dt(DType dt, int epi, int act, const GemmParams& p, hipStream_t s) {
  if (epi == EPI_LNF) return launch_typed<_Float16>(dt == DT_BF16 ? EPI_LNF_BF : EPI_LNF, act, p, s);
  return dt == DT_BF16 ? launch_typed<__bf16>(epi, act, p, s) : launch_typed<_Float16>(epi, act, p, s);
}

hipError_t launch_gemm(DType dt, int asrc, int epi, int act, const GemmParams& p, hipStream_t s) {
  if (p.K % BK != 0 || p.M <= 0 || p.N <= 0) return hipErrorInvalidValue;
  if (epi == EPI_LNF && (p.bias == nullptr || p.cs == nullptr || p.rowstats == nullptr || p.N % 4 != 0))
    return hipErrorInvalidValue;
  if (epi == EPI_LNF_BF) return hipErrorInvalidValue;
  if (p.bias != nullptr && p.N % 4 != 0) return hipErrorInvalidValue;
  if ((long)p.N * p.ldw * 2 >= (1L << 31) || p.lda <= 0) return hipErrorInvalidValue;
  if (asrc != A_ROWS) return hipErrorInvalidValue;
  if ((long)p.M * p.lda * 2 >= (1L << 31) || (g_gemm_chunk_cap > 0 && p.M > g_gemm_chunk_cap)) {
    const int G = epi == EPI_PATCH ? p.G : 0;
    const long chunk = gemm_chunk_rows(p.lda, G);
    if (chunk <= 0) return hipErrorInvalidValue;
    const long osz = (epi_st16(epi) || ((epi == EPI_RESID || epi == EPI_PATCH) && p.x16)) ? 2 : 4;
    for (long m0 = 0; m0 < p.M; m0 += chunk) {
      GemmParams q = p;
      q.M = (int)std::min<long>(chunk, p.M - m0);
      q.A = (const char*)p.A + m0 * p.lda * 2;
      if (epi == EPI_LNF) q.rowstats = p.rowstats + 2 * m0;
      const long orow = G > 0 ? m0 / ((long)G * G) * ((long)G * G + p.cls) : m0;
      q.out = (char*)p.out + orow * p.ldo * osz;
      const hipError_t err = launch_dt(dt, epi, act, q, s);
      if (err != hipSuccess) return err;
    }
    return hipSuccess;
  }
  return launch_dt(dt, epi, act, p, s);
}

#ifdef CLIPGPU_GEMM_STAMPS
hipError_t read_gemm_stamps(unsigned long long* host, int nblocks, bool clear) {
  const size_t n = (size_t)std::min(nblocks, kStampBlocks) * kStampSlots * sizeof(unsigned long long);
  if (clear) {
    static unsigned long long zeros[kStampBlocks * kStampSlots];
    return hipMemcpyToSymbol(HIP_SYMBOL(g_gemm_stamps), zeros, sizeof(zeros));
  }
  return hipMemcpyFromSymbol(host, HIP_SYMBOL(g_gemm_stamps), n);
}
#endif

}
```

clip-embedder-rs_amd/csrc/kernels/kernels.hpp:

```cpp
#pragma once
#include <hip/hip_runtime.h>
#include <stdint.h>

#include <atomic>

namespace clipgpu {

enum DType { DT_BF16 = 0, DT_F16 = 1 };

enum ASrc {
  A_ROWS = 0,
  A_IMG_F32 = 1,
  A_IMG_U8 = 2,
};
enum Epi {
  EPI_STORE16 = 0,
  EPI_RESID = 1,
  EPI_STORE32 = 2,
  EPI_PATCH = 3,
  EPI_STOREQ = 4,
  EPI_RESID16 = 5,
  EPI_PATCH16 = 6,
  EPI_LNF = 7,
  EPI_LNF_BF = 8,
};
constexpr bool epi_resid(int e) { return e == EPI_RESID || e == EPI_RESID16; }
constexpr bool epi_patch(int e) { return e == EPI_PATCH || e == EPI_PATCH16; }
constexpr bool epi_x16(int e) { return e == EPI_RESID16 || e == EPI_PATCH16; }
constexpr bool epi_lnf(int e) { return e == EPI_LNF || e == EPI_LNF_BF; }
constexpr bool epi_st16(int e) { return e == EPI_STORE16 || epi_lnf(e); }

struct GemmParams {
  const void* A; long lda;
  const void* W; long ldw;
  const float* bias;
  void* out; long ldo;
  int M, N, K;
  int G;
  int cls;
  const float* pos;
  int tile;
  int diag;
  int group;
  int prio;
  int x16;
  const float* cs;
  const float* rowstats;
};

enum GemmTile {
  TILE_AUTO = 0,
  TILE_256x128 = 2,
  TILE_256x256 = 3,
  TILE_192x256_W8 = 13,
  TILE_256x256_RS = 14,
  TILE_160x128_RS = 15,
  TILE_160x128_W8_RS = 17,
  TILE_256x256_HALF = 18,
  TILE_224x192_W8 = 26,
  TILE_SKINNY = 100,
  TILE_GENERAL = 101,
};
constexpr int kGemmTiles[] = {TILE_256x128, TILE_256x256, TILE_192x256_W8, TILE_256x256_RS,
                              TILE_160x128_RS, TILE_160x128_W8_RS, TILE_256x256_HALF, TILE_224x192_W8};
inline bool gemm_tile_built(int t) {
  for (int k : kGemmTiles)
    if (k == t) return true;
  return false;
}
int pick_gemm_tile(int M, int N, int K);
extern long g_gemm_chunk_cap;
int gemm_grid(int tile, int M, int N, int K);
int device_cus();

hipError_t launch_gemm(DType dt, int asrc, int epi, int act, const GemmParams& p, hipStream_t s);
struct GemmLaunchEvents {
  hipEvent_t start = nullptr, stop = nullptr;
};
extern thread_local GemmLaunchEvents g_gemm_events;

hipError_t launch_map_attention(DType dt, const float* q, const void* kv, void* out, int B, int N, int H, int D,
                                hipStream_t s);
hipError_t launch_attention(DType dt, const void* qkv, void* out, int B, int N, int H, int D,
                            int causal, hipStream_t s);

hipError_t launch_ln_stats(const void* x, int x16, float eps, float* stats, int rows, int D, hipStream_t s);
hipError_t launch_ln_rows(DType dt, const void* x, int x16, const float* w, const float* b, float eps,
                          void* out16, int rows, int D, hipStream_t s, uint8_t* qs = nullptr);

hipError_t launch_vision_embed_ln(DType dt, void* x, int x16, const float* cls, const float* pos,
                                  const float* lnpre_w, const float* lnpre_b,
                                  const float* ln1_w, const float* ln1_b, float eps,
                                  void* h, int B, int tokens, int D, hipStream_t s, uint8_t* qs = nullptr,
                                  float* stats = nullptr);

hipError_t launch_text_embed_ln(DType dt, const int64_t* ids, const float* tok, const float* pos,
                                const float* ln1_w, const float* ln1_b, float eps, void* x, int x16,
                                void* h, int B, int T, int D, int vocab, hipStream_t s, uint8_t* qs = nullptr,
                                float* stats = nullptr);

hipError_t launch_pool_ln(DType dt, const void* x, int x16, const int64_t* ids, int tokens,
                          const float* w, const float* b, float eps, void* out16, int B, int D,
                          hipStream_t s);

hipError_t launch_gather_pooled(const void* x, int x16, const void* h16, const int64_t* ids, int tokens, void* xc,
                                void* hc16, int B, int D, hipStream_t s);

hipError_t launch_patch_rows(DType dt, int src, const void* img, const float* mean, const float* stdv, void* out,
                             int B, int S, int P, int Kv, int Kp, hipStream_t s);

struct ResizeImage {
  long src, tmp;
  long h_bounds, h_coef;
  long v_bounds, v_coef;
  int W, th, yfirst, h_ksize, v_ksize, need_h, need_v, h_prec, v_prec, pad[3];
};
hipError_t launch_resize(const uint8_t* raw, uint8_t* tmp, const int* ints, const ResizeImage* d_imgs, int n,
                         int max_th, int S, uint8_t* out, hipStream_t s);

enum SimAct { SIM_SOFTMAX = 0, SIM_SIGMOID = 1, SIM_LOGITS = 2 };
hipError_t launch_similarity(const float* img, int ni, const float* txt, int nt, int E, float scale, float bias,
                             int activation, int axis, float* out, hipStream_t s);

constexpr int kTopkMax = 128;
struct TopkPlan { int span_cols, n_spans; };
extern std::atomic<long> g_topk_span_cols;
TopkPlan topk_plan(long N, int q_tiles, int max_blocks);
hipError_t launch_topk(const float* q, int nq, const float* g, int N, int E, float scale, float bias, int k,
                       const TopkPlan& p, void* ws, int64_t* out_idx, float* out_score, hipStream_t s);

hipError_t launch_l2norm(const float* in, float* out, int B, int E, hipStream_t s);

hipError_t launch_cast_f32(DType dt, const float* in, void* out, long n, hipStream_t s);
hipError_t launch_pull_copy(const void* src_mapped, void* dst, size_t bytes, hipStream_t s);

#ifdef CLIPGPU_GEMM_STAMPS
hipError_t read_gemm_stamps(unsigned long long* host, int nblocks, bool clear);
#endif

struct MxGemmParams {
  const uint8_t* A; long lda; const uint8_t* As; long ldas;
  const uint8_t* W; long ldw; const uint8_t* Ws; long ldws;
  const float* bias;
  void* out; long ldo;
  uint8_t* outs; long ldos;
  int M, N, K;
  int tile;
  int x16;
};
enum MxTile {
  MX_TILE_AUTO = 0,
  MX_TILE_256x256 = 1,
// ... 10 lines not shown
```

clip-embedder-rs_amd/csrc/kernels/rowwise.hip:

```cpp
#include <type_traits>

#include "common.hpp"
#include "kernels.hpp"

namespace clipgpu {

namespace {

constexpr int MAXV = 5;

template <int NV>
struct Row {
  float4 v[NV];
};

template <int NV>
__device__ __forceinline__ bool in_row(int i, int lane, int D4) {
  return i + 1 < NV || i * 64 + lane < D4;
}

template <int NV>
__device__ __forceinline__ void load_row(const float* src, int D4, int lane, Row<NV>& r) {
#pragma unroll
  for (int i = 0; i < NV; ++i)
    r.v[i] = in_row<NV>(i, lane, D4) ? ((const float4*)src)[i * 64 + lane] : make_float4(0.f, 0.f, 0.f, 0.f);
}

typedef _Float16 Half4 __attribute__((ext_vector_type(4)));
template <int NV>
__device__ __forceinline__ void load_row(const _Float16* src, int D4, int lane, Row<NV>& r) {
#pragma unroll
  for (int i = 0; i < NV; ++i) {
    if (in_row<NV>(i, lane, D4)) {
      const Half4 h = ((const Half4*)src)[i * 64 + lane];
      r.v[i] = make_float4((float)h[0], (float)h[1], (float)h[2], (float)h[3]);
    } else {
      r.v[i] = make_float4(0.f, 0.f, 0.f, 0.f);
    }
  }
}

template <int NV>
__device__ __forceinline__ void ln_stats_regs(const Row<NV>& in, float eps, int D, int lane, float& mean_out,
                                              float& rstd_out) {
  const int D4 = D >> 2;
  float s = 0.f;
#pragma unroll
  for (int i = 0; i < NV; ++i) s += in.v[i].x + in.v[i].y + in.v[i].z + in.v[i].w;
  const float mean = wave_sum(s) / (float)D;
  float q = 0.f;
#pragma unroll
  for (int i = 0; i < NV; ++i) {
    if (in_row<NV>(i, lane, D4)) {
      const float a = in.v[i].x - mean, bb = in.v[i].y - mean, cc = in.v[i].z - mean, d = in.v[i].w - mean;
      q += a * a + bb * bb + cc * cc + d * d;
    }
  }
  const float var = wave_sum(q) / (float)D;
  mean_out = mean;
  rstd_out = 1.0f / sqrtf(var + eps);
}

template <int NV>
__device__ __forceinline__ void layer_norm_regs(const Row<NV>& in, Row<NV>& out, const Row<NV>& g, const Row<NV>& b,
                                                float eps, int D, int lane) {
  float mean, rstd;
  ln_stats_regs(in, eps, D, lane, mean, rstd);
#pragma unroll
  for (int i = 0; i < NV; ++i) {
    out.v[i].x = (in.v[i].x - mean) * rstd * g.v[i].x + b.v[i].x;
    out.v[i].y = (in.v[i].y - mean) * rstd * g.v[i].y + b.v[i].y;
    out.v[i].z = (in.v[i].z - mean) * rstd * g.v[i].z + b.v[i].z;
    out.v[i].w = (in.v[i].w - mean) * rstd * g.v[i].w + b.v[i].w;
  }
}

template <typename T, int NV>
__device__ __forceinline__ void store_row16(T* dst, const Row<NV>& r, int D4, int lane) {
  typedef typename Vec4<T>::type V4;
#pragma unroll
  for (int i = 0; i < NV; ++i) {
    if (in_row<NV>(i, lane, D4)) {
      V4 o;
      o[0] = (T)r.v[i].x; o[1] = (T)r.v[i].y; o[2] = (T)r.v[i].z; o[3] = (T)r.v[i].w;
      ((V4*)dst)[i * 64 + lane] = o;
    }
  }
}

template <int NV>
__device__ __forceinline__ void store_row_mx(uint8_t* q, uint8_t* qs, const Row<NV>& r, int D4, int lane) {
#pragma unroll
  for (int i = 0; i < NV; ++i) {
    const float4 v = r.v[i];
    float amax = fmaxf(fmaxf(fabsf(v.x), fabsf(v.y)), fmaxf(fabsf(v.z), fabsf(v.w)));
    amax = fmaxf(amax, __shfl_xor(amax, 1, 64));
    amax = fmaxf(amax, __shfl_xor(amax, 2, 64));
    amax = fmaxf(amax, __shfl_xor(amax, 4, 64));
    if (in_row<NV>(i, lane, D4)) {
      const int e = mx_exp(amax);
      const int c = i * 64 + lane;
      ((uint32_t*)q)[c] = mx_pack4(v.x, v.y, v.z, v.w, mx_inv(e));
      if ((lane & 7) == 0) qs[c >> 3] = (uint8_t)(e + 127);
    }
  }
}

template <typename T, int NV>
__device__ __forceinline__ void store_ln_out(T* out, uint8_t* qs, long row, int D, const Row<NV>& r, int lane) {
  if (qs != nullptr) store_row_mx((uint8_t*)out + row * D, qs + row * (D >> 5), r, D >> 2, lane);
  else store_row16(out + row * D, r, D >> 2, lane);
}

// ... 36 lines not shown
  }
}


template <typename T, int NV, typename XT>
__global__ __launch_bounds__(256) void ln_rows_kernel(const XT* __restrict__ x, const float* w, const float* b,
                                                      float eps,
                                                      T* __restrict__ out, uint8_t* __restrict__ qs, int rows,
                                                      int D) {
  const int stride = gridDim.x * 4, lane = threadIdx.x & 63;
  int row = blockIdx.x * 4 + (threadIdx.x >> 6);
  if (row >= rows) return;
  const int D4 = D >> 2;
  Row<NV> r, g, bb;
  load_row(x + (long)row * D, D4, lane, r);
  load_row(w, D4, lane, g);
  load_row(b, D4, lane, bb);
  for (;;) {
    const int next = row + stride;
    Row<NV> nr;
    if (next < rows) load_row(x + (long)next * D, D4, lane, nr);
    Row<NV> o;
    layer_norm_regs(r, o, g, bb, eps, D, lane);
    store_ln_out(out, qs, row, D, o, lane);
    if (next >= rows) break;
    row = next;
    r = nr;
  }
}

template <typename T, int NV, typename XT>
__global__ __launch_bounds__(256) void ln_stats_kernel(const XT* __restrict__ x, float eps, float* __restrict__ stats,
                                                       int rows, int D) {
  const int stride = gridDim.x * 4, lane = threadIdx.x & 63;
  int row = blockIdx.x * 4 + (threadIdx.x >> 6);
  if (row >= rows) return;
  const int D4 = D >> 2;
  Row<NV> r;
  load_row(x + (long)row * D, D4, lane, r);
  for (;;) {
    const int next = row + stride;
    Row<NV> nr;
    if (next < rows) load_row(x + (long)next * D, D4, lane, nr);
    float mean, rstd;
    ln_stats_regs(r, eps, D, lane, mean, rstd);
    if (lane == 0) *(float2*)(stats + 2L * row) = make_float2(mean, rstd);
    if (next >= rows) break;
    row = next;
    r = nr;
  }
}

template <typename T, int NV, typename XT>
__global__ __launch_bounds__(256) void vision_embed_ln_kernel(XT* __restrict__ x, const float* cls,
                                                              const float* pos, const float* lnpre_w,
                                                              const float* lnpre_b, const float* ln1_w,
                                                              const float* ln1_b, float eps, T* __restrict__ h,
                                                              uint8_t* __restrict__ qs, int rows, int tokens, int D,
                                                              float* __restrict__ stats) {
  const int row = blockIdx.x * 4 + (threadIdx.x >> 6), lane = threadIdx.x & 63;
  if (row >= rows) return;
  const int D4 = D >> 2;
  Row<NV> r, y, z, g0, b0, g1, b1;
  if (row % tokens == 0) {
    Row<NV> c, p;
    load_row(cls, D4, lane, c);
    load_row(pos, D4, lane, p);
    r = c;
    add_row(r, p);
  } else {
    load_row(x + (long)row * D, D4, lane, r);
  }
  load_row(lnpre_w, D4, lane, g0);
  load_row(lnpre_b, D4, lane, b0);
  if (h != nullptr) {
    load_row(ln1_w, D4, lane, g1);
    load_row(ln1_b, D4, lane, b1);
  }
  layer_norm_regs(r, y, g0, b0, eps, D, lane);
  round_rowx<XT>(y);
  store_rowx(x + (long)row * D, y, D4, lane);
  if (h == nullptr) {
    float mean, rstd;
    ln_stats_regs(y, eps, D, lane, mean, rstd);
    if (lane == 0) *(float2*)(stats + 2L * row) = make_float2(mean, rstd);
    return;
  }
  layer_norm_regs(y, z, g1, b1, eps, D, lane);
  store_ln_out(h, qs, row, D, z, lane);
}

template <typename T, int NV, typename XT>
__global__ __launch_bounds__(256) void text_embed_ln_kernel(const int64_t* __restrict__ ids, const float* tok,
                                                            const float* pos, const float* ln1_w,
                                                            const float* ln1_b, float eps, XT* __restrict__ x,
                                                            T* __restrict__ h, uint8_t* __restrict__ qs, int rows,
                                                            int Tctx, int D, int vocab, float* __restrict__ stats) {
  const int row = blockIdx.x * 4 + (threadIdx.x >> 6), lane = threadIdx.x & 63;
  if (row >= rows) return;
  const int D4 = D >> 2;
  long id = ids[row];
  id = id < 0 ? 0 : (id >= vocab ? vocab - 1 : id);
  Row<NV> e, p, y, g, bb;
  load_row(tok + id * D, D4, lane, e);
  load_row(pos + (long)(row % Tctx) * D, D4, lane, p);
  if (h != nullptr) {
    load_row(ln1_w, D4, lane, g);
    load_row(ln1_b, D4, lane, bb);
  }
  add_row(e, p);
  round_rowx<XT>(e);
  store_rowx(x + (long)row * D, e, D4, lane);
  if (h == nullptr) {
    float mean, rstd;
    ln_stats_regs(e, eps, D, lane, mean, rstd);
    if (lane == 0) *(float2*)(stats + 2L * row) = make_float2(mean, rstd);
    return;
  }
  layer_norm_regs(e, y, g, bb, eps, D, lane);
  store_ln_out(h, qs, row, D, y, lane);
}

__device__ inline int pooled_token(const int64_t* __restrict__ ids, int bi, int tokens, int lane) {
  if (ids == nullptr) return 0;
  long best = -1;
  int bidx = 0x7fffffff;
  for (int t = lane; t < tokens; t += 64) {
    const long v = ids[(long)bi * tokens + t];
    if (v > best) { best = v; bidx = t; }
  }
#pragma unroll
  for (int o = 32; o > 0; o >>= 1) {
    const long ov = __shfl_xor(best, o, 64);
    const int oi = __shfl_xor(bidx, o, 64);
    if (ov > best || (ov == best && oi < bidx)) { best = ov; bidx = oi; }
  }
  return bidx;
}

template <typename T, int NV, typename XT>
__global__ __launch_bounds__(256) void pool_ln_kernel(const XT* __restrict__ x,
                                                      const int64_t* __restrict__ ids, int tokens, const float* w,
                                                      const float* b, float eps, T* __restrict__ out, int B, int D) {
  const int bi = blockIdx.x * 4 + (threadIdx.x >> 6), lane = threadIdx.x & 63;
  if (bi >= B) return;
  const int D4 = D >> 2;
  const int src = pooled_token(ids, bi, tokens, lane);
  Row<NV> r, y, g, bb;
  load_row(x + ((long)bi * tokens + src) * D, D4, lane, r);
  load_row(w, D4, lane, g);
  load_row(b, D4, lane, bb);
  layer_norm_regs(r, y, g, bb, eps, D, lane);
  store_row16(out + (long)bi * D, y, D4, lane);
}

__global__ __launch_bounds__(256) void gather_pooled_kernel(const char* __restrict__ x,
                                                            const uint16_t* __restrict__ h,
                                                            const int64_t* __restrict__ ids, int tokens,
                                                            char* __restrict__ xc, uint16_t* __restrict__ hc, int B,
                                                            int D, int xbytes) {
  const int bi = blockIdx.x * 4 + (threadIdx.x >> 6), lane = threadIdx.x & 63;
  if (bi >= B) return;
  const long src = (long)bi * tokens + pooled_token(ids, bi, tokens, lane);
  const long rb = (long)D * xbytes;
  const uint2* xs = (const uint2*)(x + src * rb);
  uint2* xd = (uint2*)(xc + (long)bi * rb);
// ... 30 lines not shown
    auto go_ = [&](auto nvc) {                                                                          \
      constexpr int NVC = decltype(nvc)::value;                                                         \
      hipLaunchKernelGGL((KERNEL<T, NVC, XT>), GRID, dim3(256), 0, s, __VA_ARGS__);                     \
    };                                                                                                  \
    switch (nv_) {                                                                                      \
      case 1: go_(std::integral_constant<int, 1>{}); break;                                             \
      case 2: go_(std::integral_constant<int, 2>{}); break;                                             \
      case 3: go_(std::integral_constant<int, 3>{}); break;                                             \
      case 4: go_(std::integral_constant<int, 4>{}); break;                                             \
      default: go_(std::integral_constant<int, 5>{}); break;                                            \
    }                                                                                                   \
  } while (0)
template <typename F>
inline void dispatch_dx(DType dt, int x16, F f) {
  if (dt == DT_BF16) {
    if (x16) f((__bf16*)nullptr, (_Float16*)nullptr);
    else f((__bf16*)nullptr, (float*)nullptr);
  } else {
    if (x16) f((_Float16*)nullptr, (_Float16*)nullptr);
    else f((_Float16*)nullptr, (float*)nullptr);
  }
}
#define CLIPGPU_TX_TYPES                                  \
  using T = std::remove_pointer_t<decltype(tp_)>;          \
  using XT = std::remove_pointer_t<decltype(xp_)>;         \
  (void)tp_;                                              \
  (void)xp_

hipError_t launch_ln_rows(DType dt, const void* x, int x16, const float* w, const float* b, float eps, void* out16,
                          int rows, int D, hipStream_t s, uint8_t* qs) {
  if (D % 4 || D > 256 * MAXV || D <= 0 || (qs != nullptr && D % 32)) return hipErrorInvalidValue;
  dim3 grid = rows_grid(rows);
  const int cap = device_cus() * 8;
  if ((int)grid.x > cap) grid.x = cap;
  dispatch_dx(dt, x16, [&](auto tp_, auto xp_) {
    CLIPGPU_TX_TYPES;
    CLIPGPU_ROW_LAUNCH_X(ln_rows_kernel, T, XT, grid, D, (const XT*)x, w, b, eps, (T*)out16, qs, rows, D);
  });
  return hipGetLastError();
}

hipError_t launch_ln_stats(const void* x, int x16, float eps, float* stats, int rows, int D, hipStream_t s) {
  if (D % 4 || D > 256 * MAXV || D <= 0 || rows <= 0 || stats == nullptr) return hipErrorInvalidValue;
  dim3 grid = rows_grid(rows);
  const int cap = device_cus() * 8;
  if ((int)grid.x > cap) grid.x = cap;
  dispatch_dx(DT_BF16, x16, [&](auto tp_, auto xp_) {
    CLIPGPU_TX_TYPES;
    CLIPGPU_ROW_LAUNCH_X(ln_stats_kernel, T, XT, grid, D, (const XT*)x, eps, stats, rows, D);
  });
  return hipGetLastError();
}

hipError_t launch_vision_embed_ln(DType dt, void* x, int x16, const float* cls, const float* pos, const float* lnpre_w,
                                  const float* lnpre_b, const float* ln1_w, const float* ln1_b, float eps,
                                  void* h, int B, int tokens, int D, hipStream_t s, uint8_t* qs, float* stats) {
  if (h == nullptr && stats == nullptr) return hipErrorInvalidValue;
  if (D % 4 || D > 256 * MAXV || D <= 0 || (qs != nullptr && D % 32)) return hipErrorInvalidValue;
  const int rows = B * tokens;
  dispatch_dx(dt, x16, [&](auto tp_, auto xp_) {
    CLIPGPU_TX_TYPES;
    CLIPGPU_ROW_LAUNCH_X(vision_embed_ln_kernel, T, XT, rows_grid(rows), D, (XT*)x, cls, pos, lnpre_w, lnpre_b, ln1_w,
                         ln1_b, eps, (T*)h, qs, rows, tokens, D, stats);
  });
  return hipGetLastError();
}

hipError_t launch_text_embed_ln(DType dt, const int64_t* ids, const float* tok, const float* pos,
                                const float* ln1_w, const float* ln1_b, float eps, void* x, int x16, void* h,
                                int B, int Tctx, int D, int vocab, hipStream_t s, uint8_t* qs, float* stats) {
  if (h == nullptr && stats == nullptr) return hipErrorInvalidValue;
  if (D % 4 || D > 256 * MAXV || D <= 0 || (qs != nullptr && D % 32)) return hipErrorInvalidValue;
  const int rows = B * Tctx;
  dispatch_dx(dt, x16, [&](auto tp_, auto xp_) {
    CLIPGPU_TX_TYPES;
    CLIPGPU_ROW_LAUNCH_X(text_embed_ln_kernel, T, XT, rows_grid(rows), D, ids, tok, pos, ln1_w, ln1_b, eps, (XT*)x,
                         (T*)h, qs, rows, Tctx, D, vocab, stats);
  });
  return hipGetLastError();
}

hipError_t launch_gather_pooled(const void* x, int x16, const void* h16, const int64_t* ids, int tokens, void* xc,
                                void* hc16, int B, int D, hipStream_t s) {
  if (D % 4 || D <= 0 || B <= 0 || tokens <= 0) return hipErrorInvalidValue;
  hipLaunchKernelGGL(gather_pooled_kernel, rows_grid(B), dim3(256), 0, s, (const char*)x, (const uint16_t*)h16, ids,
                     tokens, (char*)xc, (uint16_t*)hc16, B, D, x16 ? 2 : 4);
  return hipGetLastError();
}

hipError_t launch_pool_ln(DType dt, const void* x, int x16, const int64_t* ids, int tokens,
                          const float* w, const float* b, float eps, void* out16, int B, int D, hipStream_t s) {
  if (D % 4 || D > 256 * MAXV || D <= 0) return hipErrorInvalidValue;
  dispatch_dx(dt, x16, [&](auto tp_, auto xp_) {
    CLIPGPU_TX_TYPES;
    CLIPGPU_ROW_LAUNCH_X(pool_ln_kernel, T, XT, rows_grid(B), D, (const XT*)x, ids, tokens, w, b, eps, (T*)out16, B, D);
  });
  return hipGetLastError();
}

hipError_t launch_l2norm(const float* in, float* out, int B, int E, hipStream_t s) {
  hipLaunchKernelGGL(l2norm_kernel, rows_grid(B), dim3(256), 0, s, in, out, B, E);
  return hipGetLastError();
}

__global__ __launch_bounds__(256) void pull_copy_kernel(const uint4* __restrict__ src, uint4* __restrict__ dst,
                                                        long n16) {
  for (long i = (long)blockIdx.x * 256 + threadIdx.x; i < n16; i += (long)gridDim.x * 256) dst[i] = src[i];
}

hipError_t launch_pull_copy(const void* src_mapped, void* dst, size_t bytes, hipStream_t s) {
  if (((uintptr_t)src_mapped | (uintptr_t)dst | bytes) & 15) return hipErrorInvalidValue;
  const long n16 = (long)(bytes / 16);
  const long blocks = (n16 + 255) / 256 < 2048 ? (n16 + 255) / 256 : 2048;
  if (n16 == 0) return hipSuccess;
  hipLaunchKernelGGL(pull_copy_kernel, dim3((unsigned)blocks), dim3(256), 0, s, (const uint4*)src_mapped, (uint4*)dst,
                     n16);
  return hipGetLastError();
}

hipError_t launch_cast_f32(DType dt, const float* in, void* out, long n, hipStream_t s) {
  const long blocks = (n + 255) / 256 < 4096 ? (n + 255) / 256 : 4096;
  if (dt == DT_BF16)
    hipLaunchKernelGGL(cast_kernel<__bf16>, dim3((unsigned)blocks), dim3(256), 0, s, in, (__bf16*)out, n);
  else
    hipLaunchKernelGGL(cast_kernel<_Float16>, dim3((unsigned)blocks), dim3(256), 0, s, in, (_Float16*)out, n);
  return hipGetLastError();
}

}
```

clip-embedder-rs_amd/csrc/testing.hip:

```cpp
#include <hip/hip_runtime.h>

#include <chrono>
#include <csignal>
#include <cstdio>
#include <dlfcn.h>
#include <execinfo.h>
#include <unistd.h>
#include <cstdlib>
#include <cstring>
#include <exception>
#include <vector>

#include "../../include/clipgpu.h"
#include "../../include/clipgpu_testing.h"
#include "bounce.hpp"
#include "hip_check.hpp"
#include "host/copy_pool.hpp"
#include "host/api_util.hpp"
#include "kernels/common.hpp"
#include "kernels/kernels.hpp"
#include "kernels/topk_key.hpp"

using namespace clipgpu;

// ... 31 lines not shown
    r = __builtin_amdgcn_s_memrealtime();
  }
  const unsigned long long t1 = __builtin_amdgcn_s_memtime();
  const int lane = threadIdx.x;
  if (lane < 2) out[lane] = lane == 0 ? t1 - t0 : r - r0;
}

void up(void* d, const void* h, size_t n) { HIP_CHECK(copy_h2d(d, h, n)); }
void down(void* h, const void* d, size_t n) { HIP_CHECK(copy_d2h(h, d, n)); }

void up16(DType dt, void* d16, const float* h, size_t n) {
  DevBuf tmp(n * 4);
  up(tmp.p, h, n * 4);
  HIP_CHECK(launch_cast_f32(dt, tmp.as<float>(), d16, (long)n, nullptr));
  HIP_CHECK(hipDeviceSynchronize());
}

template <typename T>
__global__ void widen(const T* in, float* out, long n) {
  for (long i = (long)blockIdx.x * blockDim.x + threadIdx.x; i < n; i += (long)gridDim.x * blockDim.x)
    out[i] = (float)in[i];
}

void down16(DType dt, float* h, const void* d16, size_t n) {
  DevBuf tmp(n * 4);
  if (dt == DT_BF16) hipLaunchKernelGGL(widen<__bf16>, dim3(1024), dim3(256), 0, nullptr, (const __bf16*)d16, tmp.as<float>(), (long)n);
  else hipLaunchKernelGGL(widen<_Float16>, dim3(1024), dim3(256), 0, nullptr, (const _Float16*)d16, tmp.as<float>(), (long)n);
  HIP_CHECK(hipGetLastError());
  HIP_CHECK(hipDeviceSynchronize());
  down(h, tmp.p, n * 4);
}

void launched(hipError_t e, const char* what) {
  if (e == hipErrorInvalidValue) {
    (void)hipGetLastError();
    throw ClipErr(CLIPGPU_ERR_INVALID, std::string(what) + ": refused (hipErrorInvalidValue)");
  }
  check(e, what);
}

void up_stream(int x16, void* d, const float* h, size_t n) {
  if (x16) up16(DT_F16, d, h, n);
  else up(d, h, n * 4);
}
void down_stream(int x16, float* h, const void* d, size_t n) {
  if (x16) down16(DT_F16, h, d, n);
  else down(h, d, n * 4);
}

void require(bool ok, const char* msg) {
  if (!ok) throw ClipErr(CLIPGPU_ERR_INVALID, msg);
}

}

extern "C" {

int clipgpu_test_ln_rows(int dtype, int x16, int64_t rows, int64_t D, float eps, const float* x, const float* w,
                         const float* b, float* out, float* stats, uint8_t* q, uint8_t* qs) {
  return guarded([&]() {
    const DType dt = dt_of(dtype);
    require(rows > 0 && D > 0 && rows * D < INT32_MAX && x && w && b && out && stats && (q == nullptr) == (qs == nullptr),
            "bad LN arguments");
    DevBuf dx(rows * D * 4), dw(D * 4), db(D * 4), dO(rows * D * 2), dS(rows * 8), dq(rows * D), ds(rows * (D / 32 + 1));
    up_stream(x16, dx.p, x, rows * D);
    up(dw.p, w, D * 4);
    up(db.p, b, D * 4);
    if (qs != nullptr)
      launched(launch_ln_rows(dt, dx.p, x16, dw.as<float>(), db.as<float>(), eps, dq.p, (int)rows, (int)D, nullptr,
                              ds.as<uint8_t>()),
               "launch_ln_rows (MX)");
    launched(launch_ln_rows(dt, dx.p, x16, dw.as<float>(), db.as<float>(), eps, dO.p, (int)rows, (int)D, nullptr),
             "launch_ln_rows");
    launched(launch_ln_stats(dx.p, x16, eps, dS.as<float>(), (int)rows, (int)D, nullptr), "launch_ln_stats");
    HIP_CHECK(hipDeviceSynchronize());
    down16(dt, out, dO.p, rows * D);
    down(stats, dS.p, rows * 8);
    if (qs != nullptr) {
      down(q, dq.p, rows * D);
      down(qs, ds.p, rows * (D / 32));
    }
  });
}

}

namespace {
template <typename Go>
void run_stem(DType dt, int x16, int mode, int64_t rows, int64_t D, const void* dx, Go go, const char* what,
              float* x_out, float* h_out, float* stats_out, uint8_t* q_out, uint8_t* qs_out) {
  require(mode >= 0 && mode <= 2 && x_out, "bad stem mode");
  require(mode == 0 ? h_out != nullptr : mode == 1 ? stats_out != nullptr : (q_out && qs_out), "missing stem output");
  DevBuf dH(rows * D * 2), dS(rows * 8), ds(rows * (D / 32 + 1));
  launched(go(mode == 1 ? nullptr : dH.p, mode == 2 ? ds.as<uint8_t>() : nullptr, mode == 1 ? dS.as<float>() : nullptr),
           what);
  HIP_CHECK(hipDeviceSynchronize());
  down_stream(x16, x_out, dx, rows * D);
  if (mode == 0) down16(dt, h_out, dH.p, rows * D);
  if (mode == 1) down(stats_out, dS.p, rows * 8);
  if (mode == 2) {
    down(q_out, dH.p, rows * D);
    down(qs_out, ds.p, rows * (D / 32));
  }
}
}

extern "C" {

int clipgpu_test_vision_stem(int dtype, int x16, int mode, int64_t B, int64_t tokens, int64_t D, float eps,
                             const float* x_in, const float* cls, const float* pos, const float* lnpre_w,
                             const float* lnpre_b, const float* ln1_w, const float* ln1_b, float* x_out, float* h_out,
                             float* stats_out, uint8_t* q_out, uint8_t* qs_out) {
  return guarded([&]() {
    const DType dt = dt_of(dtype);
    require(B > 0 && tokens > 0 && D > 0 && B * tokens * D < INT32_MAX, "bad stem shape");
    const int64_t rows = B * tokens;
    DevBuf dx(rows * D * 4), dc(D * 4), dp(D * 4), g0(D * 4), b0(D * 4), g1(D * 4), b1(D * 4);
    up_stream(x16, dx.p, x_in, rows * D);
    const float* hs[6] = {cls, pos, lnpre_w, lnpre_b, ln1_w, ln1_b};
    DevBuf* dev[6] = {&dc, &dp, &g0, &b0, &g1, &b1};
    for (int i = 0; i < 6; ++i) up(dev[i]->p, hs[i], D * 4);
    run_stem(dt, x16, mode, rows, D, dx.p,
             [&](void* h, uint8_t* qs, float* stats) {
               return launch_vision_embed_ln(dt, dx.p, x16, dc.as<float>(), dp.as<float>(), g0.as<float>(),
                                             b0.as<float>(), g1.as<float>(), b1.as<float>(), eps, h, (int)B,
                                             (int)tokens, (int)D, nullptr, qs, stats);
             },
             "launch_vision_embed_ln", x_out, h_out, stats_out, q_out, qs_out);
  });
}

int clipgpu_test_text_stem(int dtype, int x16, int mode, int64_t B, int64_t T, int64_t D, int64_t vocab, int64_t npos,
                           float eps, const int64_t* ids, const float* tok, const float* pos, const float* ln1_w,
                           const float* ln1_b, float* x_out, float* h_out, float* stats_out, uint8_t* q_out,
                           uint8_t* qs_out) {
  return guarded([&]() {
    const DType dt = dt_of(dtype);
    require(B > 0 && T > 0 && D > 0 && vocab > 0 && npos >= T && B * T * D < INT32_MAX && vocab * D < INT32_MAX,
            "bad stem shape");
    const int64_t rows = B * T;
    DevBuf dx(rows * D * 4), di(rows * 8), dtok(vocab * D * 4), dp(npos * D * 4), g1(D * 4), b1(D * 4);
    up(di.p, ids, rows * 8);
    up(dtok.p, tok, vocab * D * 4);
    up(dp.p, pos, npos * D * 4);
    up(g1.p, ln1_w, D * 4);
    up(b1.p, ln1_b, D * 4);
    run_stem(dt, x16, mode, rows, D, dx.p,
             [&](void* h, uint8_t* qs, float* stats) {
               return launch_text_embed_ln(dt, di.as<int64_t>(), dtok.as<float>(), dp.as<float>(), g1.as<float>(),
                                           b1.as<float>(), eps, dx.p, x16, h, (int)B, (int)T, (int)D, (int)vocab,
                                           nullptr, qs, stats);
             },
             "launch_text_embed_ln", x_out, h_out, stats_out, q_out, qs_out);
  });
}

int clipgpu_test_pool(int dtype, int x16, int64_t B, int64_t tokens, int64_t D, const float* x, const uint16_t* h16_bits,
                      const int64_t* ids, const float* w, const float* b, float eps, float* pooled_out,
                      void* xc_out_bits, uint16_t* hc_out_bits) {
  return guarded([&]() {
    const DType dt = dt_of(dtype);
    require(B > 0 && tokens > 0 && D > 0 && B * tokens * D < INT32_MAX && x, "bad pool shape");
    require((xc_out_bits == nullptr) == (hc_out_bits == nullptr) && (hc_out_bits == nullptr) == (h16_bits == nullptr) &&
                (pooled_out || xc_out_bits) && (!pooled_out || (w && b)),
            "bad pool arguments");
    const int64_t rows = B * tokens, xb = x16 ? 2 : 4;
    DevBuf dx(rows * D * 4), dh(rows * D * 2), di(rows * 8), dw(D * 4), db(D * 4), dP(B * D * 2), dxc(B * D * 4),
        dhc(B * D * 2);
    up_stream(x16, dx.p, x, rows * D);
    if (ids) up(di.p, ids, rows * 8);
    const int64_t* dids = ids ? di.as<int64_t>() : nullptr;
    if (pooled_out) {
      up(dw.p, w, D * 4);
      up(db.p, b, D * 4);
      launched(launch_pool_ln(dt, dx.p, x16, dids, (int)tokens, dw.as<float>(), db.as<float>(), eps, dP.p, (int)B,
                              (int)D, nullptr),
               "launch_pool_ln");
    }
    if (xc_out_bits) {
      up(dh.p, h16_bits, rows * D * 2);
      launched(launch_gather_pooled(dx.p, x16, dh.p, dids, (int)tokens, dxc.p, dhc.p, (int)B, (int)D, nullptr),
               "launch_gather_pooled");
    }
    HIP_CHECK(hipDeviceSynchronize());
    if (pooled_out) down16(dt, pooled_out, dP.p, B * D);
    if (xc_out_bits) {
      down(xc_out_bits, dxc.p, B * D * xb);
      down(hc_out_bits, dhc.p, B * D * 2);
    }
  });
}

int clipgpu_test_map_attention(int dtype, int64_t B, int64_t N, int64_t H, int64_t D, const float* q, const float* kv,
                               float* out) {
  return guarded([&]() {
    const DType dt = dt_of(dtype);
    require(B > 0 && N > 0 && H > 0 && D > 0 && B * N * 2 * D < INT32_MAX && q && kv && out, "bad MAP arguments");
    DevBuf dq(D * 4), dkv(B * N * 2 * D * 2), dO(B * D * 2);
    up(dq.p, q, D * 4);
    up16(dt, dkv.p, kv, B * N * 2 * D);
    launched(launch_map_attention(dt, dq.as<float>(), dkv.p, dO.p, (int)B, (int)N, (int)H, (int)D, nullptr),
             "launch_map_attention");
    HIP_CHECK(hipDeviceSynchronize());
    down16(dt, out, dO.p, B * D);
// ... 37 lines not shown
    g.A = dA.p; g.lda = K; g.W = dW.p; g.ldw = K; g.bias = bias ? dB.as<float>() : nullptr;
    g.out = dO.p; g.ldo = N; g.M = (int)M; g.N = (int)N; g.K = (int)K;
    int epi = EPI_STORE16;
    if (mode == 1) {
      epi = EPI_RESID;
      if (resid) up(dO.p, resid, M * N * 4);
    } else if (mode == 2) {
      epi = EPI_STORE32;
    } else if (mode == 3) {
      epi = EPI_RESID;
      g.x16 = 1;
      if (resid) up16(DT_F16, dO.p, resid, M * N);
    } else if (mode != 0) {
      throw ClipErr(CLIPGPU_ERR_INVALID, "bad mode");
    }
    HIP_CHECK(launch_gemm(dt, A_ROWS, epi, mode == 0 ? act : 0, g, nullptr));
    HIP_CHECK(hipDeviceSynchronize());
    if (mode == 0) down16(dt, out, dO.p, M * N);
    else if (mode == 3) down16(DT_F16, out, dO.p, M * N);
    else down(out, dO.p, M * N * 4);
  });
}

int clipgpu_test_gemm_chunk_rows(int64_t rows) {
  return guarded([&]() {
    if (rows < 0) throw ClipErr(CLIPGPU_ERR_INVALID, "rows < 0");
    g_gemm_chunk_cap = (long)rows;
  });
}

int clipgpu_test_topk_span_cols(int64_t cols) {
  return guarded([&]() {
    if (cols < 0 || cols % 64) throw ClipErr(CLIPGPU_ERR_INVALID, "cols must be a multiple of 64 (0 = default)");
    g_topk_span_cols.store((long)cols);
  });
}

int clipgpu_test_topk_key(float score, uint32_t index, uint64_t* key) {
  return guarded([&]() {
    if (!key) throw ClipErr(CLIPGPU_ERR_INVALID, "NULL key");
    uint32_t bits;
    std::memcpy(&bits, &score, 4);
    *key = topk_key(bits, index);
  });
}

int clipgpu_test_gemm_lnf(int dtype, int act, int64_t M, int64_t N, int64_t K, const float* x, const float* wf,
                          const float* cs, const float* bias, float eps, int tile, float* out) {
  return guarded([&]() {
    const DType dt = dt_of(dtype);
    if (M <= 0 || N <= 0 || K <= 0 || K % 64 || N % 4) throw ClipErr(CLIPGPU_ERR_INVALID, "bad GEMM shape");
    if (tile != 0 && tile != TILE_SKINNY && tile != TILE_GENERAL && !gemm_tile_built(tile))
      throw ClipErr(CLIPGPU_ERR_INVALID, "bad tile");
    DevBuf dA(M * K * 2), dW(N * K * 2), dB(N * 4), dC(N * 4), dO(M * N * 2), dS((M + 256) * 8);
    up16(DT_F16, dA.p, x, M * K);
    up16(DT_F16, dW.p, wf, N * K);
    up(dB.p, bias, N * 4);
    up(dC.p, cs, N * 4);
    HIP_CHECK(launch_ln_stats(dA.p, 1, eps, dS.as<float>(), (int)M, (int)K, nullptr));
    GemmParams g{};
    g.tile = tile;
    g.A = dA.p; g.lda = K; g.W = dW.p; g.ldw = K; g.bias = dB.as<float>(); g.cs = dC.as<float>();
    g.rowstats = dS.as<float>();
    g.out = dO.p; g.ldo = N; g.M = (int)M; g.N = (int)N; g.K = (int)K;
    HIP_CHECK(launch_gemm(dt, A_ROWS, EPI_LNF, act, g, nullptr));
    HIP_CHECK(hipDeviceSynchronize());
    down16(dt, out, dO.p, M * N);
  });
}

int clipgpu_test_attention(int dtype, int64_t B, int64_t N, int64_t H, int64_t HD, int causal, const float* qkv,
                           float* out) {
  return guarded([&]() {
    const DType dt = dt_of(dtype);
    require(B > 0 && N > 0 && H > 0 && HD > 0 && B * N * 3 * H * HD < INT32_MAX && qkv && out,
            "bad attention arguments");
    const int64_t D = H * HD;
    constexpr size_t GUARD = 4096;
    const size_t out_bytes = (size_t)(B * N * D) * 2;
    DevBuf dq(B * N * 3 * D * 2), dO(out_bytes + GUARD);
    HIP_CHECK(hipMemset((char*)dO.p + out_bytes, 0xA5, GUARD));
    up16(dt, dq.p, qkv, B * N * 3 * D);
    launched(launch_attention(dt, dq.p, dO.p, (int)B, (int)N, (int)H, (int)D, causal, nullptr), "launch_attention");
    HIP_CHECK(hipDeviceSynchronize());
    std::vector<unsigned char> guard(GUARD);
    down(guard.data(), (char*)dO.p + out_bytes, GUARD);
    for (size_t i = 0; i < GUARD; ++i)
      if (guard[i] != 0xA5)
        throw ClipErr(CLIPGPU_ERR_DEVICE, "launch_attention wrote past its output (guard byte " + std::to_string(i) + ")");
    down16(dt, out, dO.p, B * N * D);
  });
}

int clipgpu_test_layernorm(int dtype, int64_t rows, int64_t D, float eps, const float* x, const float* w,
                           const float* b, float* out) {
  return guarded([&]() {
    const DType dt = dt_of(dtype);
    DevBuf dx(rows * D * 4), dw(D * 4), db(D * 4), dO(rows * D * 2);
    up(dx.p, x, rows * D * 4);
    up(dw.p, w, D * 4);
    up(db.p, b, D * 4);
    HIP_CHECK(launch_ln_rows(dt, dx.as<float>(), 0, dw.as<float>(), db.as<float>(), eps, dO.p, (int)rows, (int)D, nullptr));
    HIP_CHECK(hipDeviceSynchronize());
    down16(dt, out, dO.p, rows * D);
  });
}

int clipgpu_test_patch_embed(int dtype, int mode, int64_t B, int64_t S, int64_t P, int64_t D, const void* pixels,
                             const float mean[3], const float stdv[3], const float* conv_w, const float* pos,
                             float* x_out) {
  return guarded([&]() {
    const DType dt = dt_of(dtype);
    const int64_t G = S / P, K = 3 * P * P, Kp = (K + 63) / 64 * 64, tokens = G * G + 1;
    const size_t pix_bytes = mode == 0 ? (size_t)B * 3 * S * S * 4 : (size_t)B * S * S * 3;
    DevBuf dpix(pix_bytes), dw(D * Kp * 2), dpos(tokens * D * 4), dx(B * tokens * D * 4);
    up(dpix.p, pixels, pix_bytes);
    std::vector<float> wpad((size_t)(D * Kp), 0.f);
    for (int64_t r = 0; r < D; ++r)
      for (int64_t k = 0; k < K; ++k) wpad[(size_t)(r * Kp + k)] = conv_w[r * K + k];
    up16(dt, dw.p, wpad.data(), D * Kp);
// ... 423 lines not shown
```

clip-embedder-rs_amd/open_clip_inference/_lib.py:

```python
from __future__ import annotations

import ctypes
import os
from ctypes import POINTER, c_char_p, c_double, c_float, c_int, c_int64, c_uint64, c_void_p

from .error import ClipError, error_for_status

_HERE = os.path.dirname(os.path.abspath(__file__))
LIB_PATH = os.environ.get("CLIPGPU_LIB", os.path.join(os.path.dirname(_HERE), "lib", "libclipgpu.so"))

TOWER_VISION = 0
TOWER_TEXT = 1
DTYPE_BF16 = 0
DTYPE_F16 = 1
DTYPE_FP8 = 2

_PROTOS = [
    ("clipgpu_last_error", c_char_p, []),
    ("clipgpu_abi_version", c_int, []),
    ("clipgpu_build_source_hash", c_char_p, []),
    ("clipgpu_create", c_int, [c_char_p, c_int, POINTER(c_int), c_int, c_int, c_int, POINTER(c_void_p)]),
    ("clipgpu_options_init", c_int, [c_void_p]),
    ("clipgpu_create_ex", c_int, [c_char_p, c_int, POINTER(c_int), c_int, c_int, c_int, c_void_p, POINTER(c_void_p)]),
    ("clipgpu_engine_info", c_int, [c_void_p, POINTER(c_int), POINTER(c_int), POINTER(ctypes.c_uint32)]),
    ("clipgpu_destroy", None, [c_void_p]),
    ("clipgpu_embed_dim", c_int, [c_void_p]),
    ("clipgpu_input_size", c_int, [c_void_p]),
    ("clipgpu_num_devices", c_int, [c_void_p]),
    ("clipgpu_embed_pixels", c_int, [c_void_p, c_void_p, c_int64, c_int64, c_void_p]),
    ("clipgpu_embed_u8", c_int, [c_void_p, c_void_p, c_int64, c_int64, POINTER(c_float), POINTER(c_float), c_void_p]),
    ("clipgpu_host_register", c_int, [c_void_p, ctypes.c_size_t]),
    ("clipgpu_host_unregister", c_int, [c_void_p]),
    ("clipgpu_embed_tokens", c_int, [c_void_p, c_void_p, c_void_p, c_int64, c_int64, c_void_p]),
    ("clipgpu_embed_pixels_device", c_int, [c_void_p, c_void_p, c_int64, c_void_p, c_void_p]),
    ("clipgpu_embed_u8_device", c_int, [c_void_p, c_void_p, c_int64, POINTER(c_float), POINTER(c_float), c_void_p, c_void_p]),
    ("clipgpu_embed_tokens_device", c_int, [c_void_p, c_void_p, c_int64, c_void_p, c_void_p]),
    ("clipgpu_embed_images_rgb8", c_int, [c_void_p, POINTER(c_void_p), POINTER(c_int), POINTER(c_int), c_int64, c_void_p]),
    ("clipgpu_preprocess_rgb8", c_int, [c_void_p, c_int, c_int, c_int, c_char_p, c_char_p, POINTER(c_float), POINTER(c_float), c_void_p]),
    ("clipgpu_resize_rgb8", c_int, [c_void_p, c_int, c_int, c_int, c_char_p, c_char_p, c_void_p]),
    ("clipgpu_preprocess_batch", c_int, [POINTER(c_void_p), POINTER(c_int), POINTER(c_int), c_int64, c_int, c_char_p, c_char_p, POINTER(c_float), POINTER(c_float), c_void_p]),
    ("clipgpu_resize_rgb8_image", c_int, [c_void_p, c_int, c_int, c_int, c_char_p, c_char_p, c_void_p]),
    ("clipgpu_preprocess_batch_image", c_int, [POINTER(c_void_p), POINTER(c_int), POINTER(c_int), c_int64, c_int, c_char_p, c_char_p, POINTER(c_float), POINTER(c_float), c_void_p]),
    ("clipgpu_tokenizer_create", c_int, [c_char_p, c_int, c_int64, POINTER(c_void_p)]),
    ("clipgpu_tokenizer_destroy", None, [c_void_p]),
    ("clipgpu_tokenize", c_int, [c_void_p, POINTER(c_char_p), c_void_p, c_int64, c_int, c_void_p, c_void_p]),
    ("clipgpu_tokenizer_token_id", c_int64, [c_void_p, c_char_p]),
    ("clipgpu_tokenizer_vocab_size", c_int64, [c_void_p]),
    ("clipgpu_similarity", c_int, [c_int, c_void_p, c_int64, c_void_p, c_int64, c_int64, c_float, c_float, c_int, c_int, c_void_p]),
    ("clipgpu_similarity_device", c_int, [c_void_p, c_int64, c_void_p, c_int64, c_int64, c_float, c_float, c_int, c_int, c_void_p, c_void_p]),
    ("clipgpu_index_create", c_int, [c_int, c_int64, c_int64, POINTER(c_void_p)]),
    ("clipgpu_index_destroy", None, [c_void_p]),
    ("clipgpu_index_size", c_int64, [c_void_p]),
    ("clipgpu_index_clear", c_int, [c_void_p]),
    ("clipgpu_index_add", c_int, [c_void_p, c_void_p, c_int64]),
    ("clipgpu_index_add_device", c_int, [c_void_p, c_void_p, c_int64, c_void_p]),
    ("clipgpu_index_search", c_int, [c_void_p, c_void_p, c_int64, c_int64, c_float, c_float, c_void_p, c_void_p]),
    ("clipgpu_index_search_device", c_int, [c_void_p, c_void_p, c_int64, c_int64, c_float, c_float, c_void_p, c_void_p,
                                            c_void_p]),
    ("clipgpu_comm_unique_id", c_int, [c_void_p]),
    ("clipgpu_comm_init_rank", c_int, [c_void_p, c_void_p, c_int, c_int]),
    ("clipgpu_comm_info", c_int, [c_void_p, POINTER(c_int), POINTER(c_int)]),
    ("clipgpu_embed_pixels_gather_device", c_int, [c_void_p, POINTER(c_void_p), POINTER(c_int64), POINTER(c_void_p), POINTER(c_void_p)]),
    ("clipgpu_embed_tokens_gather_device", c_int, [c_void_p, POINTER(c_void_p), POINTER(c_int64), POINTER(c_void_p), POINTER(c_void_p)]),
    ("clipgpu_facade_scores", c_int, [c_void_p, c_int64, c_void_p, c_int64, c_float, c_float, c_int, c_void_p]),
    ("clipgpu_profile_enable", c_int, [c_void_p, ctypes.c_uint]),
    ("clipgpu_profile_read", c_int, [c_void_p, c_int, POINTER(c_double), POINTER(c_int64)]),
    ("clipgpu_profile_category_name", c_char_p, [c_int]),
    ("clipgpu_synth_tensor", c_int, [c_uint64, c_char_p, c_double, c_double, c_void_p, c_int64]),
    ("clipgpu_test_gemm", c_int, [c_int, c_int, c_int, c_int64, c_int64, c_int64, c_void_p, c_void_p, c_void_p, c_void_p, c_void_p]),
    ("clipgpu_test_gemm_chunk_rows", c_int, [c_int64]),
    ("clipgpu_test_topk_span_cols", c_int, [c_int64]),
    ("clipgpu_test_topk_key", c_int, [c_float, ctypes.c_uint32, POINTER(c_uint64)]),
    ("clipgpu_test_gemm_lnf", c_int, [c_int, c_int, c_int64, c_int64, c_int64, c_void_p, c_void_p, c_void_p,
                               c_void_p, c_float, c_int, c_void_p]),
    ("clipgpu_test_attention", c_int, [c_int, c_int64, c_int64, c_int64, c_int64, c_int, c_void_p, c_void_p]),
    ("clipgpu_test_layernorm", c_int, [c_int, c_int64, c_int64, c_float, c_void_p, c_void_p, c_void_p, c_void_p]),
    ("clipgpu_test_ln_rows", c_int, [c_int, c_int, c_int64, c_int64, c_float] + [c_void_p] * 7),
    ("clipgpu_test_vision_stem", c_int, [c_int, c_int, c_int, c_int64, c_int64, c_int64, c_float] + [c_void_p] * 12),
    ("clipgpu_test_text_stem", c_int, [c_int, c_int, c_int, c_int64, c_int64, c_int64, c_int64, c_int64, c_float]
                                      + [c_void_p] * 10),
    ("clipgpu_test_pool", c_int, [c_int, c_int, c_int64, c_int64, c_int64, c_void_p, c_void_p, c_void_p, c_void_p,
                                  c_void_p, c_float, c_void_p, c_void_p, c_void_p]),
    ("clipgpu_test_map_attention", c_int, [c_int, c_int64, c_int64, c_int64, c_int64, c_void_p, c_void_p, c_void_p]),
    ("clipgpu_test_l2norm", c_int, [c_int64, c_int64, c_void_p, c_void_p]),
    ("clipgpu_test_cast", c_int, [c_int, c_int64, c_void_p, c_void_p]),
    ("clipgpu_test_gemm_grid", c_int, [c_int, c_int64, c_int64, c_int64, POINTER(c_int)]),
    ("clipgpu_test_gemm_bench", c_int, [c_int, c_int, c_int, c_int64, c_int64, c_int64, c_int, c_int, POINTER(c_double)]),
    ("clipgpu_test_h2d_bench", c_int, [c_int64, c_int, c_int, POINTER(c_double)]),
    ("clipgpu_test_host_copy", c_int, [c_int64, c_int, c_int, POINTER(c_double)]),
    ("clipgpu_test_install_crash_handler", c_int, []),
    ("clipgpu_test_gemm_bench_ld", c_int, [c_int, c_int, c_int, c_int64, c_int64, c_int64, c_int64, c_int64, c_int, c_int,
                                           POINTER(c_double)]),
    ("clipgpu_test_engine_tiles", c_int, [c_void_p, POINTER(c_int)]),
    ("clipgpu_test_engine_lanes", c_int, [c_void_p, POINTER(c_int)]),
    ("clipgpu_test_engine_residual", c_int, [c_void_p, POINTER(c_int), POINTER(c_int)]),
    ("clipgpu_test_host_plan", c_int, [c_void_p, c_int, POINTER(c_int), c_int]),
    ("clipgpu_test_force_broadcast", c_int, [c_void_p, c_int]),
    ("clipgpu_test_rgb8_resize_always", c_int, [c_void_p, c_int]),
    ("clipgpu_test_comm_lazy", c_int, [c_void_p]),
    ("clipgpu_test_profile_timeline", c_int, [c_void_p, c_int64, POINTER(c_double), POINTER(c_double), POINTER(c_int),
                                              POINTER(c_int), POINTER(c_int64)]),
    ("clipgpu_test_gather_plan", c_int, [c_int, POINTER(c_int64), POINTER(c_int64), POINTER(c_int)]),
    ("clipgpu_test_read_weights", c_int, [c_char_p, c_int, c_char_p, c_void_p, c_int64]),
    ("clipgpu_test_patch_embed", c_int, [c_int, c_int, c_int64, c_int64, c_int64, c_int64, c_void_p, POINTER(c_float), POINTER(c_float), c_void_p, c_void_p, c_void_p]),
    ("clipgpu_test_resize_rgb8_gpu", c_int, [POINTER(c_void_p), POINTER(c_int), POINTER(c_int), c_int64, c_int, c_char_p, c_char_p, c_void_p]),
    ("clipgpu_test_lane_reduce", c_int, [c_void_p, c_void_p]),
    ("clipgpu_test_patch_rows", c_int, [c_int, c_int, c_int64, c_int64, c_int64, c_void_p, POINTER(c_float), POINTER(c_float), c_void_p]),
    ("clipgpu_test_clock_probe", c_int, [c_void_p, c_int64, c_void_p]),
    ("clipgpu_test_attention_bench", c_int, [c_int, c_int64, c_int64, c_int64, c_int64, c_int, c_int, POINTER(c_double)]),
    ("clipgpu_test_quant_rows", c_int, [c_int64, c_int64, c_void_p, c_void_p, c_void_p]),
    ("clipgpu_test_layernorm_mx", c_int, [c_int64, c_int64, c_float, c_void_p, c_void_p, c_void_p, c_void_p, c_void_p]),
    ("clipgpu_test_gemm_mx", c_int, [c_int, c_int, c_int, c_int64, c_int64, c_int64, c_void_p, c_void_p, c_void_p, c_void_p, c_void_p, c_void_p, c_void_p, c_void_p, c_void_p]),
    ("clipgpu_test_gemm_mx_bench", c_int, [c_int, c_int, c_int64, c_int64, c_int64, c_int, c_int, POINTER(c_double)]),
]

SYMBOLS = [p[0] for p in _PROTOS]

_lib = None


def lib():
    global _lib
    if _lib is None:
        if not os.path.exists(LIB_PATH):
            raise ClipError(f"clipgpu native library not found at {LIB_PATH}; "
                            "run `make -C clip-embedder-rs_amd` (or __graft_entry__.build())")
        L = ctypes.CDLL(LIB_PATH)
# ... 56 lines not shown
```

clip-embedder-rs_amd/open_clip_inference/engine.py:

```python
from __future__ import annotations

import ctypes
from ctypes import POINTER, c_char_p, c_int, c_void_p
from typing import Optional, Sequence

import numpy as np

from . import _lib
from ._lib import check, f3, lib


class Options(ctypes.Structure):
    _fields_ = [("struct_size", ctypes.c_uint32), ("mx_sites", ctypes.c_uint32), ("lanes", ctypes.c_int32),
                ("tuning", ctypes.c_int32), ("communicator", ctypes.c_int32),
                ("graphs", ctypes.c_int32), ("prune_last", ctypes.c_int32), ("trim_text", ctypes.c_int32),
                ("gemm_tiles", ctypes.c_int32 * 4), ("patch_tile", ctypes.c_int32), ("mx_layers", ctypes.c_uint32),
                ("residual", ctypes.c_int32), ("ln_fold", ctypes.c_int32)]


def _tristate(v) -> int:
    return 0 if v is None else (1 if v else -1)


MX_SITE_BITS = {"qkv": 1, "fc": 2, "proj": 4}


def mx_site_bits(sites) -> int:
    if sites is None:
        return 0
    if isinstance(sites, str):
        sites = [s for s in sites.split(",") if s]
    bits = 0
    for s in sites:
        if s not in MX_SITE_BITS:
            raise ValueError(f"unknown MX site {s!r}: one of {sorted(MX_SITE_BITS)}")
        bits |= MX_SITE_BITS[s]
    return bits


class Engine:
    def __init__(self, model_dir: str, tower: int, devices: Optional[Sequence[int]] = None,
                 dtype: str = "bf16", max_batch: int = 256, mx_sites=None, lanes: int = 0, tuning=False,
                 communicator: bool = False, graphs: Optional[bool] = None, prune_last: Optional[bool] = None,
                 trim_text: Optional[bool] = None, gemm_tiles: Optional[Sequence[int]] = None, patch_tile: int = 0,
                 mx_layers=None, residual: Optional[str] = None, ln_fold: Optional[bool] = None):
        self.model_dir = model_dir
        self.tower = tower
        self.devices = list(devices) if devices else [0]
        self.dtype = dtype
        self.max_batch = int(max_batch)
        self.opts = {"mx_sites": mx_sites, "lanes": int(lanes), "tuning": tuning, "communicator": bool(communicator),
                     "graphs": graphs, "prune_last": prune_last, "trim_text": trim_text,
                     "gemm_tiles": list(gemm_tiles) if gemm_tiles else None, "patch_tile": int(patch_tile),
                     "mx_layers": mx_layers, "residual": residual,
                     "ln_fold": ln_fold}
        dt = {"bf16": _lib.DTYPE_BF16, "f16": _lib.DTYPE_F16, "fp16": _lib.DTYPE_F16, "fp8": _lib.DTYPE_FP8}[dtype]
        devs = (c_int * len(self.devices))(*self.devices)
        opts = Options()
        check(lib().clipgpu_options_init(ctypes.byref(opts)))
        opts.mx_sites = mx_site_bits(mx_sites)
        opts.lanes = int(lanes)
        opts.tuning = int(tuning) if not isinstance(tuning, bool) else (1 if tuning else 0)
        opts.communicator = 1 if communicator else 0
        opts.graphs = _tristate(graphs)
        opts.prune_last = _tristate(prune_last)
        opts.trim_text = _tristate(trim_text)
        if gemm_tiles:
            if len(gemm_tiles) != 4:
                raise ValueError("gemm_tiles: four GemmTile ids (qkv, out_proj, c_fc, c_proj)")
            for i, t in enumerate(gemm_tiles):
                opts.gemm_tiles[i] = int(t)
        opts.patch_tile = int(patch_tile)
        if mx_layers is not None:
            if not isinstance(mx_layers, int):
                layers = [int(l) for l in mx_layers]
                if any(l < 0 or l >= 32 for l in layers):
                    raise ValueError("mx_layers: layer indices 0..31 (clipgpu_options.mx_layers is a 32-bit mask)")
                mx_layers = sum(1 << l for l in set(layers))
            if mx_layers < 0 or mx_layers > 0xFFFFFFFF:
                raise ValueError("mx_layers: a 32-bit layer mask (clipgpu_options.mx_layers)")
            if mx_layers == 0:
                raise ValueError("mx_layers: at least one layer (None = every layer)")
            opts.mx_layers = int(mx_layers)
        if residual not in (None, "f32", "f16"):
            raise ValueError('residual: "f32" or "f16"')
        opts.residual = {None: 0, "f32": 1, "f16": 2}[residual]
        opts.ln_fold = _tristate(ln_fold)
        h = c_void_p()
        check(lib().clipgpu_create_ex(model_dir.encode(), tower, devs, len(self.devices), dt, self.max_batch,
                                      ctypes.byref(opts), ctypes.byref(h)))
        self._h = h

    def info(self):
        tiles = (c_int * 4)()
        lanes = c_int()
        bits = ctypes.c_uint32()
        check(lib().clipgpu_engine_info(self.handle, tiles, ctypes.byref(lanes), ctypes.byref(bits)))
        sites = [s for s, b in MX_SITE_BITS.items() if bits.value & b]
        return list(tiles), lanes.value, sites

    @property
    def handle(self):
        if self._h is None:
            raise RuntimeError("engine destroyed")
        return self._h

    def close(self):
        if getattr(self, "_h", None) is not None:
            lib().clipgpu_destroy(self._h)
            self._h = None

    def __del__(self):
        try:
            self.close()
        except Exception:
            pass

    @property
    def embed_dim(self) -> int:
        return lib().clipgpu_embed_dim(self.handle)

    @property
    def input_size(self) -> int:
        return lib().clipgpu_input_size(self.handle)

    def _out(self, B: int, out: Optional[np.ndarray]) -> np.ndarray:
        if out is None:
            return np.empty((B, self.embed_dim), np.float32)
        if out.dtype != np.float32 or out.shape != (B, self.embed_dim) or not out.flags["C_CONTIGUOUS"]:
            raise ValueError(f"out must be a C-contiguous float32 [{B}, {self.embed_dim}] array")
        return out

    def embed_pixels(self, nchw: np.ndarray, out: Optional[np.ndarray] = None) -> np.ndarray:
        x = np.ascontiguousarray(nchw, dtype=np.float32)
        if x.ndim != 4 or x.shape[1] != 3 or x.shape[2] != x.shape[3]:
            from .error import ShapeError
            raise ShapeError(f"Shape error: expected [B,3,S,S], got {x.shape}")
        out = self._out(x.shape[0], out)
        check(lib().clipgpu_embed_pixels(self.handle, x.ctypes.data, x.shape[0], x.shape[2], out.ctypes.data))
        return out
# ... 213 lines not shown
```

include/clipgpu.h:

```cpp
#ifndef CLIPGPU_H
#define CLIPGPU_H

#include <stddef.h>
#include <stdint.h>

#ifdef __cplusplus
extern "C" {
#endif

#define CLIPGPU_ABI_VERSION 4

enum clipgpu_status {
  CLIPGPU_OK = 0,
  CLIPGPU_ERR_INVALID = 1,
  CLIPGPU_ERR_CONFIG = 2,
  CLIPGPU_ERR_IO = 3,
  CLIPGPU_ERR_DEVICE = 4,
  CLIPGPU_ERR_TOKENIZER = 5
};

enum clipgpu_tower { CLIPGPU_TOWER_VISION = 0, CLIPGPU_TOWER_TEXT = 1 };
enum clipgpu_dtype { CLIPGPU_DTYPE_BF16 = 0, CLIPGPU_DTYPE_F16 = 1, CLIPGPU_DTYPE_FP8 = 2 };

typedef struct clipgpu_engine clipgpu_engine;
typedef struct clipgpu_tokenizer clipgpu_tokenizer;

const char* clipgpu_last_error(void);
int clipgpu_abi_version(void);
const char* clipgpu_build_source_hash(void);

int clipgpu_create(const char* model_dir, int tower, const int* device_ids, int n_devices, int dtype,
                   int max_batch, clipgpu_engine** out);
void clipgpu_destroy(clipgpu_engine* e);

#define CLIPGPU_MX_QKV 1u
#define CLIPGPU_MX_FC 2u
#define CLIPGPU_MX_PROJ 4u
#define CLIPGPU_RESIDUAL_F32 1
#define CLIPGPU_RESIDUAL_F16 2
typedef struct clipgpu_options {
  uint32_t struct_size;
  uint32_t mx_sites;
  int32_t lanes;
  int32_t tuning;
  int32_t communicator;
  int32_t graphs;
  int32_t prune_last;
  int32_t trim_text;
  int32_t gemm_tiles[4];
  int32_t patch_tile;
  uint32_t mx_layers;
  int32_t residual;
  int32_t ln_fold;
} clipgpu_options;
int clipgpu_options_init(clipgpu_options* opts);
int clipgpu_create_ex(const char* model_dir, int tower, const int* device_ids, int n_devices, int dtype,
                      int max_batch, const clipgpu_options* opts, clipgpu_engine** out);
int clipgpu_engine_info(const clipgpu_engine* e, int tiles[4], int* lanes, uint32_t* mx_sites);

int clipgpu_embed_dim(const clipgpu_engine* e);
int clipgpu_input_size(const clipgpu_engine* e);
int clipgpu_num_devices(const clipgpu_engine* e);

int clipgpu_embed_pixels(clipgpu_engine* e, const float* nchw, int64_t B, int64_t S, float* out);

int clipgpu_embed_u8(clipgpu_engine* e, const uint8_t* nhwc, int64_t B, int64_t S, const float mean[3],
                     const float std[3], float* out);

int clipgpu_host_register(void* ptr, size_t bytes);
int clipgpu_host_unregister(void* ptr);

int clipgpu_embed_tokens(clipgpu_engine* e, const int64_t* ids, const int64_t* mask, int64_t B, int64_t T,
                         float* out);

int clipgpu_embed_pixels_device(clipgpu_engine* e, const float* d_nchw, int64_t B, float* d_out, void* stream);
int clipgpu_embed_u8_device(clipgpu_engine* e, const uint8_t* d_nhwc, int64_t B, const float mean[3],
                            const float std[3], float* d_out, void* stream);
int clipgpu_embed_tokens_device(clipgpu_engine* e, const int64_t* d_ids, int64_t B, float* d_out, void* stream);

int clipgpu_embed_images_rgb8(clipgpu_engine* e, const uint8_t* const* images, const int* widths, const int* heights,
                              int64_t n, float* out);

int clipgpu_preprocess_rgb8(const uint8_t* rgb, int width, int height, int size, const char* interpolation,
                            const char* resize_mode, const float mean[3], const float std[3], float* out_chw);
int clipgpu_resize_rgb8(const uint8_t* rgb, int width, int height, int size, const char* interpolation,
                        const char* resize_mode, uint8_t* out_rgb);
int clipgpu_preprocess_batch(const uint8_t* const* images, const int* widths, const int* heights, int64_t n,
                             int size, const char* interpolation, const char* resize_mode, const float mean[3],
                             const float std[3], float* out);
int clipgpu_resize_rgb8_image(const uint8_t* rgb, int width, int height, int size, const char* interpolation,
                              const char* resize_mode, uint8_t* out_rgb);
int clipgpu_preprocess_batch_image(const uint8_t* const* images, const int* widths, const int* heights, int64_t n,
                                   int size, const char* interpolation, const char* resize_mode, const float mean[3],
                                   const float std[3], float* out);

int clipgpu_tokenizer_create(const char* tokenizer_json, int context_length, int64_t pad_id,
                             clipgpu_tokenizer** out);
void clipgpu_tokenizer_destroy(clipgpu_tokenizer* t);
int clipgpu_tokenize(clipgpu_tokenizer* t, const char* const* texts, const int64_t* lengths, int64_t n,
                     int lowercase, int64_t* ids, int64_t* mask);
int64_t clipgpu_tokenizer_token_id(const clipgpu_tokenizer* t, const char* token);
int64_t clipgpu_tokenizer_vocab_size(const clipgpu_tokenizer* t);

enum clipgpu_sim_activation { CLIPGPU_SIM_SOFTMAX = 0, CLIPGPU_SIM_SIGMOID = 1, CLIPGPU_SIM_LOGITS = 2 };
int clipgpu_similarity(int device, const float* img, int64_t n_img, const float* txt, int64_t n_txt, int64_t E,
                       float logit_scale, float logit_bias, int activation, int axis, float* out);
// ... 41 lines not shown
```

include/clipgpu_testing.h:

```cpp
#ifndef CLIPGPU_TESTING_H
#define CLIPGPU_TESTING_H

#include <stdint.h>

#ifdef __cplusplus
extern "C" {
#endif

int clipgpu_test_gemm(int dtype, int mode, int act, int64_t M, int64_t N, int64_t K, const float* A,
                      const float* W, const float* bias, const float* resid, float* out);
int clipgpu_test_gemm_lnf(int dtype, int act, int64_t M, int64_t N, int64_t K, const float* x, const float* wf,
                          const float* cs, const float* bias, float eps, int tile, float* out);

int clipgpu_test_gemm_chunk_rows(int64_t rows);

int clipgpu_test_attention(int dtype, int64_t B, int64_t N, int64_t H, int64_t HD, int causal, const float* qkv,
                           float* out);

int clipgpu_test_layernorm(int dtype, int64_t rows, int64_t D, float eps, const float* x, const float* w,
                           const float* b, float* out);

int clipgpu_test_ln_rows(int dtype, int x16, int64_t rows, int64_t D, float eps, const float* x, const float* w,
                         const float* b, float* out, float* stats, uint8_t* q, uint8_t* qs);

int clipgpu_test_vision_stem(int dtype, int x16, int mode, int64_t B, int64_t tokens, int64_t D, float eps,
                             const float* x_in, const float* cls, const float* pos, const float* lnpre_w,
                             const float* lnpre_b, const float* ln1_w, const float* ln1_b, float* x_out, float* h_out,
                             float* stats_out, uint8_t* q_out, uint8_t* qs_out);
int clipgpu_test_text_stem(int dtype, int x16, int mode, int64_t B, int64_t T, int64_t D, int64_t vocab, int64_t npos,
                           float eps, const int64_t* ids, const float* tok, const float* pos, const float* ln1_w,
                           const float* ln1_b, float* x_out, float* h_out, float* stats_out, uint8_t* q_out,
                           uint8_t* qs_out);
int clipgpu_test_pool(int dtype, int x16, int64_t B, int64_t tokens, int64_t D, const float* x,
                      const uint16_t* h16_bits, const int64_t* ids, const float* w, const float* b, float eps,
                      float* pooled_out, void* xc_out_bits, uint16_t* hc_out_bits);
int clipgpu_test_map_attention(int dtype, int64_t B, int64_t N, int64_t H, int64_t D, const float* q, const float* kv,
                               float* out);
int clipgpu_test_l2norm(int64_t B, int64_t E, const float* in, float* out);
int clipgpu_test_cast(int dtype, int64_t n, const float* in, float* out);

int clipgpu_test_patch_embed(int dtype, int mode, int64_t B, int64_t S, int64_t P, int64_t D, const void* pixels,
                             const float mean[3], const float std[3], const float* conv_w, const float* pos,
                             float* x_out);

int clipgpu_test_resize_rgb8_gpu(const uint8_t* const* images, const int* widths, const int* heights, int64_t n,
                                 int size, const char* interpolation, const char* resize_mode, uint8_t* out);

int clipgpu_test_lane_reduce(const float* in64, float* out512);

int clipgpu_test_patch_rows(int dtype, int mode, int64_t B, int64_t S, int64_t P, const void* pixels,
                            const float mean[3], const float std[3], float* rows_out);

int clipgpu_test_gemm_bench(int dtype, int epi, int act, int64_t M, int64_t N, int64_t K, int tile, int iters,
                            double* us_per_launch);
int clipgpu_test_gemm_grid(int tile, int64_t M, int64_t N, int64_t K, int* grid);
int clipgpu_test_gemm_bench_ld(int dtype, int epi, int act, int64_t M, int64_t N, int64_t K, int64_t lda,
                               int64_t ldw, int tile, int iters, double* us_per_launch);

int clipgpu_test_host_copy(int64_t bytes, int mode, int iters, double* us_per_copy);
int clipgpu_test_install_crash_handler(void);
int clipgpu_test_h2d_bench(int64_t bytes, int mode, int iters, double* us_per_copy);
int clipgpu_test_clock_probe(void* stream, int64_t duration_us, uint64_t* d_out);

int clipgpu_test_attention_bench(int dtype, int64_t B, int64_t N, int64_t H, int64_t HD, int causal, int iters,
                                 double* us_per_launch);
// ... 36 lines not shown
```

Baseline: 93580 images/s.

## Fuse LayerNorm row-sum statistics into residual GEMM epilogue

The out_proj and c_proj GEMMs with the f16 residual epilogue now accumulate per-row sums and split sums of squares in f64 and write them atomically to a stats buffer. This replaces the separate ln_stats pass that reread the residual stream before the folded-LN QKV and FC GEMMs. The folded-LN GEMM prologue now finalises mean and rstd from these sums itself. The cost is extra epilogue work (f64 math, wave reductions, atomics), a clear buffer that is double-buffered between the two sites, and a larger stats workspace. It is on by default and falls back to a standalone sums kernel when the tile cannot fuse.

```diff
diff --git a/clip-embedder-rs_amd/csrc/engine/api.hip b/clip-embedder-rs_amd/csrc/engine/api.hip
--- a/clip-embedder-rs_amd/csrc/engine/api.hip
+++ b/clip-embedder-rs_amd/csrc/engine/api.hip
@@ -34,6 +34,11 @@
 
 using namespace clipgpu;
 
+#ifndef CLIPGPU_LN_STATS_FUSED_DEFAULT
+#define CLIPGPU_LN_STATS_FUSED_DEFAULT 1
+#endif
+constexpr bool kLnStatsFusedDefault = CLIPGPU_LN_STATS_FUSED_DEFAULT != 0;
+
 extern "C" {
 
 int clipgpu_abi_version(void) { return CLIPGPU_ABI_VERSION; }
@@ -61,7 +66,8 @@
     opts.struct_size = sizeof(opts);
     if (opts_in) {
       if (opts_in->struct_size != offsetof(clipgpu_options, graphs) &&
-          opts_in->struct_size != offsetof(clipgpu_options, residual) && opts_in->struct_size != sizeof(opts))
+          opts_in->struct_size != offsetof(clipgpu_options, residual) &&
+          opts_in->struct_size != offsetof(clipgpu_options, ln_stats) && opts_in->struct_size != sizeof(opts))
         throw ClipErr(CLIPGPU_ERR_INVALID, "clipgpu_options.struct_size: call clipgpu_options_init first");
       std::memcpy(&opts, opts_in, opts_in->struct_size);
     }
@@ -83,6 +89,8 @@
       throw ClipErr(CLIPGPU_ERR_INVALID, "clipgpu_options.residual must be 0, 1 (f32) or 2 (f16)");
     if (opts.ln_fold < -1 || opts.ln_fold > 1)
       throw ClipErr(CLIPGPU_ERR_INVALID, "clipgpu_options.ln_fold must be -1, 0 or 1");
+    if (opts.ln_stats < -1 || opts.ln_stats > 1)
+      throw ClipErr(CLIPGPU_ERR_INVALID, "clipgpu_options.ln_stats must be -1, 0 or 1");
     if (opts.communicator < 0 || opts.communicator > 1)
       throw ClipErr(CLIPGPU_ERR_INVALID, "clipgpu_options.communicator must be 0 or 1");
     if (!model_dir) throw ClipErr(CLIPGPU_ERR_INVALID, "model_dir is NULL");
@@ -146,6 +154,7 @@
                       "clipgpu_options.ln_fold = 1: needs a bf16 / f16 engine, the f16 residual stream and a "
                       "QuickGELU / GELU MLP");
       e->lnf = fold_ok && opts.ln_fold != -1;
+      e->fuse_stats = opts.ln_stats ? opts.ln_stats == 1 : kLnStatsFusedDefault;
     }
     for (int i = 0; i < 4; ++i) e->pin_tiles[i] = opts.gemm_tiles[i];
     e->pin_patch = opts.patch_tile;
diff --git a/clip-embedder-rs_amd/csrc/engine/engine.hpp b/clip-embedder-rs_amd/csrc/engine/engine.hpp
--- a/clip-embedder-rs_amd/csrc/engine/engine.hpp
+++ b/clip-embedder-rs_amd/csrc/engine/engine.hpp
@@ -73,7 +73,9 @@
   char* work = nullptr;
   DevWeights w;
   void* x = nullptr;
-  float* xs = nullptr;
+  double* xs = nullptr;
+  double* xs2 = nullptr;
+  long xs_ld = 0;
   void* h = nullptr;
   uint8_t* hs = nullptr;
   uint8_t* bigs = nullptr;
@@ -148,6 +150,7 @@
   bool trim = true;
   bool x16 = false;
   bool lnf = false;
+  bool fuse_stats = true;
 
   int tuning = 0;
   int pin_tiles[4] = {0, 0, 0, 0};
diff --git a/clip-embedder-rs_amd/csrc/engine/forward.hip b/clip-embedder-rs_amd/csrc/engine/forward.hip
--- a/clip-embedder-rs_amd/csrc/engine/forward.hip
+++ b/clip-embedder-rs_amd/csrc/engine/forward.hip
@@ -83,7 +83,8 @@
   }
   if (e.lnf && (site == GS_QKV || site == GS_FC)) {
     g.cs = site == GS_QKV ? L.cs_qkv : L.cs_1;
-    g.rowstats = r.xs;
+    g.rowsums = LnSums{site == GS_QKV ? r.xs : r.xs2, r.xs_ld};
+    g.ln_eps = e.spec.ln_eps;
   }
   g.group = kSiteGroup[site];
   g.x16 = e.x16 ? 1 : 0;
@@ -150,7 +151,7 @@
 inline bool prune_last(const clipgpu_engine& e, int B, int T) {
   const TowerSpec& s = e.spec;
   return e.prune && s.family != FAMILY_SIGLIP && s.layers > 0 &&
-         prune_off_xs(s, B) + ((size_t)B + 256) * 8 <= (size_t)B * T * big_wide(s) * 2;
+         prune_off_xs(s, B) + 3 * ((size_t)B + 256) * 8 <= (size_t)B * T * big_wide(s) * 2;
 }
 
 PoolSrc trunk(const clipgpu_engine& e, const Replica& r, int B, int causal, const int64_t* ids, hipStream_t st,
@@ -163,19 +164,27 @@
     const bool compact = prune && l + 1 == s.layers;
     Replica c = r;
     int rows = B * T;
-    auto gemm = [&](int site, int cat, const char* what) {
-      if (ABLATED(site == GS_QKV ? 3 : site == GS_OUT ? 2 : site == GS_FC ? 4 : 5)) return;
+    auto gemm = [&](int site, int cat, const char* what) -> bool {
+      if (ABLATED(site == GS_QKV ? 3 : site == GS_OUT ? 2 : site == GS_FC ? 4 : 5)) return false;
       ProfScope ps(e, rows == B * T ? cat : PC_TAIL, st, true);
       const bool tuned = 2 * rows > e.tuned_rows;
       if (mx_at(e, l, site)) {
         MxGemmParams g = site_gemm_mx(e, c, L, site, rows);
         g.tile = tuned ? e.mxtile[site] : MX_TILE_AUTO;
         check(launch_gemm_mx(e.dt, site_epi_mx(e, l, site), site == GS_FC ? s.act : ACT_NONE, g, st), what);
-        return;
+        return false;
       }
       GemmParams g = site_gemm(e, c, L, site, rows);
       g.tile = tuned ? e.tile[site] : TILE_AUTO;
+      bool fused = false;
+      if (e.lnf && e.fuse_stats && !compact && (site == GS_OUT || (site == GS_PROJ && l + 1 < s.layers))) {
+        g.stats_out = LnSums{site == GS_OUT ? r.xs2 : r.xs, r.xs_ld};
+        g.stats_clear = LnSums{site == GS_OUT ? r.xs : r.xs2, r.xs_ld};
+        fused = gemm_fuses_stats(site_epi(e, site), g);
+        if (!fused) g.stats_out = g.stats_clear = LnSums();
+      }
       check(launch_gemm(e.dt, A_ROWS, site_epi(e, site), site == GS_FC ? s.act : ACT_NONE, g, st), what);
+      return fused;
     };
     gemm(GS_QKV, PC_QKV, "qkv gemm");
     if (!ABLATED(1)) { ProfScope ps(e, PC_ATTN, st);
@@ -183,28 +192,30 @@
     if (compact) {
       c.x = (char*)r.big + prune_off_x(s, B);
       c.h = (char*)r.big + prune_off_h(s, B);
-      c.xs = (float*)((char*)r.big + prune_off_xs(s, B));
+      c.xs2 = (double*)((char*)r.big + prune_off_xs(s, B));
+      c.xs_ld = (long)B + 256;
       rows = B;
       ProfScope ps(e, PC_TAIL, st);
       check(launch_gather_pooled(xrows(e, r.x, pool_pos), e.x16, (char*)r.h + (size_t)pool_pos * D * 2, ids, T, c.x, c.h,
                                  B, D, st),
             "gather pooled rows");
     }
-    gemm(GS_OUT, PC_OUT_PROJ, "out_proj gemm");
-    if (!ABLATED(0)) {
+    const bool stats2 = gemm(GS_OUT, PC_OUT_PROJ, "out_proj gemm");
+    if (!ABLATED(0) && !stats2) {
       ProfScope ps(e, compact ? PC_TAIL : PC_LN, st);
       if (e.lnf)
-        check(launch_ln_stats(c.x, 1, s.ln_eps, c.xs, rows, D, st), "ln_2 statistics");
+        check(launch_ln_sums(c.x, LnSums{c.xs2, c.xs_ld}, compact ? LnSums() : LnSums{r.xs, r.xs_ld}, rows, D, st),
+              "ln_2 statistics");
       else
         check(launch_ln_rows(e.dt, c.x, e.x16, L.ln2_w, L.ln2_b, s.ln_eps, c.h, rows, D, st, ln_q(e, l, GS_FC, c.hs)),
               "ln_2");
     }
     gemm(GS_FC, PC_C_FC, "c_fc gemm");
-    gemm(GS_PROJ, PC_C_PROJ, "c_proj gemm");
-    if (l + 1 < s.layers && !ABLATED(0)) {
+    const bool stats1 = gemm(GS_PROJ, PC_C_PROJ, "c_proj gemm");
+    if (l + 1 < s.layers && !ABLATED(0) && !stats1) {
       ProfScope ps(e, PC_LN, st);
       if (e.lnf)
-        check(launch_ln_stats(r.x, 1, s.ln_eps, r.xs, rows, D, st), "ln_1 statistics");
+        check(launch_ln_sums(r.x, LnSums{r.xs, r.xs_ld}, LnSums{r.xs2, r.xs_ld}, rows, D, st), "ln_1 statistics");
       else
         check(launch_ln_rows(e.dt, r.x, e.x16, r.w.layers[l + 1].ln1_w, r.w.layers[l + 1].ln1_b, s.ln_eps, r.h, rows,
                              D, st, ln_q(e, l + 1, GS_QKV, r.hs)),
@@ -283,7 +294,8 @@
   ProfScope ps(e, PC_STEM, st);
   check(launch_vision_embed_ln(e.dt, r.x, e.x16, r.w.cls, r.w.pos, r.w.lnpre_w, r.w.lnpre_b, r.w.layers[0].ln1_w,
                                r.w.layers[0].ln1_b, s.ln_eps, e.lnf ? nullptr : r.h, B, s.tokens(), D, st,
-                               ln_q(e, 0, GS_QKV, r.hs), r.xs),
+                               ln_q(e, 0, GS_QKV, r.hs), nullptr, e.lnf ? LnSums{r.xs, r.xs_ld} : LnSums(),
+                               e.lnf ? LnSums{r.xs2, r.xs_ld} : LnSums()),
         "embed+ln_pre");
   }
   head(e, r, B, trunk(e, r, B, 0, nullptr, st, s.tokens()), d_out, st);
@@ -297,7 +309,8 @@
   ProfScope ps(e, PC_STEM, st);
   check(launch_text_embed_ln(e.dt, d_ids, r.w.tok, r.w.pos, r.w.layers[0].ln1_w, r.w.layers[0].ln1_b, s.ln_eps,
                              r.x, e.x16, e.lnf ? nullptr : r.h, B, T, s.width, s.vocab_size, st,
-                             ln_q(e, 0, GS_QKV, r.hs), r.xs),
+                             ln_q(e, 0, GS_QKV, r.hs), nullptr, e.lnf ? LnSums{r.xs, r.xs_ld} : LnSums(),
+                             e.lnf ? LnSums{r.xs2, r.xs_ld} : LnSums()),
         "token embed+ln_1");
   }
   head(e, r, B, trunk(e, r, B, s.causal ? 1 : 0, s.pool_last ? nullptr : d_ids, st, T, s.pool_last ? T - 1 : 0),
@@ -310,7 +323,8 @@
   const size_t wide = big_wide(s);
   Replica v = r;
   v.x = (char*)r.x + rows * D * xbytes(e);
-  v.xs = r.xs + rows * 2;
+  v.xs = r.xs + rows;
+  v.xs2 = r.xs2 + rows;
   v.h = (char*)r.h + rows * D * 2;
   v.big = (char*)r.big + rows * wide * 2;
   if (r.hs) v.hs = r.hs + rows * D / 32;
diff --git a/clip-embedder-rs_amd/csrc/engine/weights.hip b/clip-embedder-rs_amd/csrc/engine/weights.hip
--- a/clip-embedder-rs_amd/csrc/engine/weights.hip
+++ b/clip-embedder-rs_amd/csrc/engine/weights.hip
@@ -265,7 +265,7 @@
   const size_t MLP = (size_t)mlp_pad(s);
   const size_t sizes[] = {rows * D * 4, rows * D * 2, rows * wide * 2, B * D * 2, B * E * 4, B * E * 4,
                           B * e.in_bytes_per_row, e.mx ? rows * D / 32 : 0, e.mx ? rows * MLP / 32 : 0,
-                          (rows + 256) * 8};
+                          2 * 3 * (rows + 256) * 8};
   size_t total = 0;
   for (size_t z : sizes) total += align256(z);
   HIP_CHECK(hipMalloc(&r.work, total));
@@ -281,7 +281,9 @@
   hs.in = a.take(sizes[6]);
   r.hs = e.mx ? (uint8_t*)a.take(sizes[7]) : nullptr;
   r.bigs = e.mx ? (uint8_t*)a.take(sizes[8]) : nullptr;
-  r.xs = (float*)a.take(sizes[9]);
+  r.xs = (double*)a.take(sizes[9]);
+  r.xs_ld = (long)rows + 256;
+  r.xs2 = r.xs + 3 * r.xs_ld;
   for (int i = 0; i < e.lanes; ++i) {
     HIP_CHECK(hipStreamCreateWithFlags(&r.lane[i], hipStreamNonBlocking));
     HIP_CHECK(hipEventCreateWithFlags(&r.join[i], hipEventDisableTiming));
diff --git a/clip-embedder-rs_amd/csrc/kernels/common.hpp b/clip-embedder-rs_amd/csrc/kernels/common.hpp
--- a/clip-embedder-rs_amd/csrc/kernels/common.hpp
+++ b/clip-embedder-rs_amd/csrc/kernels/common.hpp
@@ -113,6 +113,28 @@
   return fmaxf(a, b);
 }
 __device__ __forceinline__ float wave_sum(float v) { return xsum32(xsum16(row16_sum(v))); }
+__device__ __forceinline__ double f64_from_halves(float lo, float hi) {
+  return __hiloint2double(__builtin_bit_cast(int, hi), __builtin_bit_cast(int, lo));
+}
+__device__ __forceinline__ double xsum16_f64(double v) {
+  float a0 = __builtin_bit_cast(float, __double2loint(v)), a1 = __builtin_bit_cast(float, __double2hiint(v));
+  float b0 = a0, b1 = a1;
+  swap16(a0, b0);
+  swap16(a1, b1);
+  return f64_from_halves(a0, a1) + f64_from_halves(b0, b1);
+}
+__device__ __forceinline__ double xsum32_f64(double v) {
+  float a0 = __builtin_bit_cast(float, __double2loint(v)), a1 = __builtin_bit_cast(float, __double2hiint(v));
+  float b0 = a0, b1 = a1;
+  swap32(a0, b0);
+  swap32(a1, b1);
+  return f64_from_halves(a0, a1) + f64_from_halves(b0, b1);
+}
+__device__ __forceinline__ double wave_sum_f64(double v) {
+#pragma unroll
+  for (int o = 32; o > 0; o >>= 1) v += __shfl_xor(v, o, 64);
+  return v;
+}
 __device__ __forceinline__ float wave_max(float v) { return xmax32(xmax16(row16_max(v))); }
 __device__ __forceinline__ float group16_sum(float v) { return row16_sum(v); }
 __device__ __forceinline__ float group16_max(float v) { return row16_max(v); }
@@ -120,6 +142,24 @@
 typedef float f32x2 __attribute__((ext_vector_type(2)));
 __device__ __forceinline__ float lnf_out(float acc, float mean, float rstd, float cs, float bias) {
   return fmaf(fmaf(-mean, cs, acc), rstd, bias);
+}
+
+__host__ __device__ __forceinline__ void ln_sums_add(double x, double& sx, double& qhi, double& qlo) {
+  const double c = 26388279066624.0;
+  const double q = x * x;
+  const double hi = (q + c) - c;
+  sx += x;
+  qhi += hi;
+  qlo += q - hi;
+}
+__host__ __device__ __forceinline__ void ln_sums_finalize(double sx, double qhi, double qlo, int D, float eps,
+                                                          float& mean_out, float& rstd_out) {
+  const double inv_d = 1.0 / (double)D;
+  const double mean = sx * inv_d;
+  double var = __builtin_fma(-mean, mean, (qhi + qlo) * inv_d);
+  var = var < 0.0 ? 0.0 : var;
+  mean_out = (float)mean;
+  rstd_out = 1.0f / sqrtf((float)var + eps);
 }
 
 enum Act { ACT_NONE = 0, ACT_QUICK_GELU = 1, ACT_GELU = 2, ACT_GELU_TANH = 3 };
diff --git a/clip-embedder-rs_amd/csrc/kernels/gemm.hip b/clip-embedder-rs_amd/csrc/kernels/gemm.hip
--- a/clip-embedder-rs_amd/csrc/kernels/gemm.hip
+++ b/clip-embedder-rs_amd/csrc/kernels/gemm.hip
@@ -112,9 +112,14 @@
   const char* const Wb = (const char*)p.W;
   const float* const bias_p = p.bias;
   const float* const cs_p = p.cs;
-  const float* const rs_p = p.rowstats;
+  const double* const rs_p = p.rowsums.p;
+  const long rs_ld = p.rowsums.ld;
+  double* const so_p = p.stats_out.p;
+  double* const sc_p = p.stats_clear.p;
+  const long so_ld = p.stats_out.ld, sc_ld = p.stats_clear.ld;
   asm volatile("" ::"s"(lda_i), "s"(ldw_i), "s"(nb), "s"(Ab), "s"(Wb), "s"(bias_p));
-  if constexpr (LNF) asm volatile("" ::"s"(cs_p), "s"(rs_p));
+  if constexpr (LNF) asm volatile("" ::"s"(cs_p), "s"(rs_p), "s"(rs_ld));
+  if constexpr (EPI == EPI_RESID16) asm volatile("" ::"s"(so_p), "s"(sc_p), "s"(so_ld), "s"(sc_ld));
   const int nTn = (p.N + BN - 1) / BN;
   const int grp = p.group > 0 ? p.group : CLIPGPU_TILE_GROUP;
   asm volatile("" ::"s"(grp));
@@ -224,12 +229,40 @@
       if constexpr (LNF) {
         GEMM_POISON(smem + NS * STAGE + 2048 + (d_ti & 1) * 1024);
         glds16(cs_p + n, smem + NS * STAGE + 2048 + (d_ti & 1) * 1024);
-        char* const sst = smem + NS * STAGE + 4096 + (d_ti & 1) * SROWP;
-#pragma unroll
-        for (int i = 0; i < SROWP / 1024; ++i) {
-          GEMM_POISON(sst + i * 1024);
-          glds16(rs_p + (size_t)d_m0 * 2 + i * 256 + lane * 4, sst + i * 1024);
+      }
+    }
+  };
+  constexpr int RPW = LNF ? BM / NW : 1;
+  static_assert(!LNF || (BM % NW == 0 && RPW <= 64 && NS == 2), "row statistics: BM / NW rows per wave, 2 stages");
+  double st_v[3] = {0.0, 0.0, 0.0};
+  bool st_pend = false;
+  int st_par = 0;
+  auto stats_load = [&]() {
+    if constexpr (LNF) {
+      if (d_kt == 0) {
+        const long r = min(d_m0 + wave * RPW + lane, p.M - 1);
+        if (lane < RPW) {
+#pragma unroll
+          for (int c = 0; c < 3; ++c) st_v[c] = rs_p[c * rs_ld + r];
         }
+        st_par = d_ti & 1;
+        st_pend = true;
+      }
+    }
+  };
+  auto stats_finalize = [&](uint32_t lds_base) {
+    if constexpr (LNF) {
+      if (st_pend) {
+        f32x2 ms;
+        float mean, rstd;
+        ln_sums_finalize(st_v[0], st_v[1], st_v[2], p.K, p.ln_eps, mean, rstd);
+        ms[0] = mean;
+        ms[1] = rstd;
+        if (lane < RPW) {
+          const uint32_t a = lds_base + NS * STAGE + 4096 + st_par * SROWP + (uint32_t)(wave * RPW + lane) * 8u;
+          asm volatile("ds_write_b64 %0, %1" ::"v"(a), "v"(ms) : "memory");
+        }
+        st_pend = false;
       }
     }
   };
@@ -251,6 +284,7 @@
   };
   auto dma_step = [&]() {
     if (d_g < total) {
+      stats_load();
       static_for<NP>([&](auto j) { dma_piece(j); });
       dma_bias();
     }
@@ -334,6 +368,7 @@
     (void)next;
     if constexpr (!RS) read_b(b0, nbuf, 0);
     if (dma) {
+      stats_load();
       dma_bias();
       if constexpr (!SPREAD) static_for<NP>([&](auto j) { dma_piece(j); });
     }
@@ -482,6 +517,7 @@
         }
       } else {
         XE* o = (XE*)p.out + out_row(m) + nc;
+        [[maybe_unused]] double sx = 0.0, qhi = 0.0, qlo = 0.0;
         if (nfull) {
 #pragma unroll
           for (int ni = 0; ni < NI; ++ni) {
@@ -490,7 +526,17 @@
               const float4 x = widen4(xr[XALL ? mi : mi % XR][ni]);
               w.x += x.x; w.y += x.y; w.z += x.z; w.w += x.w;
             }
-            stx4(o + ni * 4, w);
+            if constexpr (EPI == EPI_RESID16) {
+              f16x4 h;
+              h[0] = (_Float16)w.x; h[1] = (_Float16)w.y; h[2] = (_Float16)w.z; h[3] = (_Float16)w.w;
+              *(f16x4*)(o + ni * 4) = h;
+              if (so_p != nullptr) {
+#pragma unroll
+                for (int j = 0; j < 4; ++j) ln_sums_add((double)(float)h[j], sx, qhi, qlo);
+              }
+            } else {
+              stx4(o + ni * 4, w);
+            }
           }
         } else {
 #pragma unroll
@@ -500,8 +546,29 @@
               if (nc + ni * 4 + j >= p.N) continue;
               float r = v[ni][j];
               if constexpr (ADDX) r += (float)add_src(m)[ni * 4 + j];
-              o[ni * 4 + j] = (XE)r;
+              const XE xo = (XE)r;
+              o[ni * 4 + j] = xo;
+              if constexpr (EPI == EPI_RESID16) {
+                if (so_p != nullptr) ln_sums_add((double)(float)xo, sx, qhi, qlo);
+              }
             }
+        }
+        if constexpr (EPI == EPI_RESID16) {
+          if (so_p != nullptr) {
+            sx = xsum32_f64(xsum16_f64(sx));
+            qhi = xsum32_f64(xsum16_f64(qhi));
+            qlo = xsum32_f64(xsum16_f64(qlo));
+            if (fq == 0) {
+              unsafeAtomicAdd(so_p + m, sx);
+              unsafeAtomicAdd(so_p + so_ld + m, qhi);
+              unsafeAtomicAdd(so_p + 2 * so_ld + m, qlo);
+            }
+          }
+          if (sc_p != nullptr && n0 + wn == 0 && fq == 0) {
+            sc_p[m] = 0.0;
+            sc_p[sc_ld + m] = 0.0;
+            sc_p[2 * sc_ld + m] = 0.0;
+          }
         }
       }
     }
@@ -557,6 +624,7 @@
 #endif
       }
       after_full_epi = false;
+      stats_finalize(lds0);
 #ifdef CLIPGPU_GEMM_STAMPS
       if (!(p.diag & 8)) __builtin_amdgcn_s_barrier();
 #else
@@ -692,7 +760,13 @@
     if (!GEN || n + 4 <= p.N) csv = *(const f32x4*)(p.cs + n);
     else
       for (int j = 0; j < 4; ++j) csv[j] = n + j < p.N ? p.cs[n + j] : 0.f;
-    rst = *(const f32x2*)(p.rowstats + (long)m * 2);
+    {
+      const double* rs = p.rowsums.p + m;
+      float mean, rstd;
+      ln_sums_finalize(rs[0], rs[p.rowsums.ld], rs[2 * p.rowsums.ld], p.K, p.ln_eps, mean, rstd);
+      rst[0] = mean;
+      rst[1] = rstd;
+    }
   }
   float v[4];
 #pragma unroll
@@ -742,6 +816,13 @@
   if (blocks > 0x7fffffffL) return hipErrorInvalidValue;
   gemm_launch(gemm_skinny_kernel<T, EPI, ACT, U, GEN>, (int)blocks, 256, s, p);
   return hipGetLastError();
+}
+
+inline bool takes_pipe(const GemmParams& p, bool patch, bool st16) {
+  if (!patch && (p.tile == TILE_AUTO || p.tile == TILE_SKINNY) && skinny_ok(p)) return false;
+  if (p.tile == TILE_SKINNY) return false;
+  const int tile = p.tile == TILE_AUTO ? pick_gemm_tile(p.M, p.N, p.K) : p.tile;
+  return tile != TILE_GENERAL && gemm_tile_built(tile) && p.K >= 2 * BK && (!st16 || p.ldo % 8 == 0);
 }
 
 template <typename T, int EPI, int ACT>
@@ -894,9 +975,19 @@
   return dt == DT_BF16 ? launch_typed<__bf16>(epi, act, p, s) : launch_typed<_Float16>(epi, act, p, s);
 }
 
+bool gemm_fuses_stats(int epi, const GemmParams& p) {
+  return epi == EPI_RESID && p.x16 && p.stats_out.p != nullptr && p.N <= kLnSumsMaxD && p.ldo == p.N &&
+         takes_pipe(p, false, false);
+}
+
 hipError_t launch_gemm(DType dt, int asrc, int epi, int act, const GemmParams& p, hipStream_t s) {
   if (p.K % BK != 0 || p.M <= 0 || p.N <= 0) return hipErrorInvalidValue;
-  if (epi == EPI_LNF && (p.bias == nullptr || p.cs == nullptr || p.rowstats == nullptr || p.N % 4 != 0))
+  if (epi == EPI_LNF && (p.bias == nullptr || p.cs == nullptr || p.rowsums.p == nullptr || p.N % 4 != 0 ||
+                         p.K > kLnSumsMaxD || p.rowsums.ld < p.M))
+    return hipErrorInvalidValue;
+  if ((p.stats_out.p != nullptr || p.stats_clear.p != nullptr) &&
+      (!(epi == EPI_RESID && p.x16) || p.stats_out.p == nullptr || p.stats_out.ld < p.M ||
+       (p.stats_clear.p != nullptr && p.stats_clear.ld < p.M) || p.N > kLnSumsMaxD || p.ldo != p.N))
     return hipErrorInvalidValue;
   if (epi == EPI_LNF_BF) return hipErrorInvalidValue;
   if (p.bias != nullptr && p.N % 4 != 0) return hipErrorInvalidValue;
@@ -911,14 +1002,20 @@
       GemmParams q = p;
       q.M = (int)std::min<long>(chunk, p.M - m0);
       q.A = (const char*)p.A + m0 * p.lda * 2;
-      if (epi == EPI_LNF) q.rowstats = p.rowstats + 2 * m0;
+      if (epi == EPI_LNF) q.rowsums = p.rowsums.rows_from(m0);
       const long orow = G > 0 ? m0 / ((long)G * G) * ((long)G * G + p.cls) : m0;
       q.out = (char*)p.out + orow * p.ldo * osz;
-      const hipError_t err = launch_dt(dt, epi, act, q, s);
+      const LnSums so = p.stats_out.rows_from(m0), sc = p.stats_clear.rows_from(m0);
+      const bool fused = so.p != nullptr && gemm_fuses_stats(epi, q);
+      q.stats_out = fused ? so : LnSums();
+      q.stats_clear = fused ? sc : LnSums();
+      hipError_t err = launch_dt(dt, epi, act, q, s);
+      if (err == hipSuccess && so.p != nullptr && !fused) err = launch_ln_sums(q.out, so, sc, q.M, q.N, s);
       if (err != hipSuccess) return err;
     }
     return hipSuccess;
   }
+  if (p.stats_out.p != nullptr && !gemm_fuses_stats(epi, p)) return hipErrorInvalidValue;
   return launch_dt(dt, epi, act, p, s);
 }
 
diff --git a/clip-embedder-rs_amd/csrc/kernels/kernels.hpp b/clip-embedder-rs_amd/csrc/kernels/kernels.hpp
--- a/clip-embedder-rs_amd/csrc/kernels/kernels.hpp
+++ b/clip-embedder-rs_amd/csrc/kernels/kernels.hpp
@@ -30,6 +30,13 @@
 constexpr bool epi_lnf(int e) { return e == EPI_LNF || e == EPI_LNF_BF; }
 constexpr bool epi_st16(int e) { return e == EPI_STORE16 || epi_lnf(e); }
 
+constexpr int kLnSumsMaxD = 4352;
+struct LnSums {
+  double* p = nullptr;
+  long ld = 0;
+  LnSums rows_from(long r) const { return LnSums{p ? p + r : nullptr, ld}; }
+};
+
 struct GemmParams {
   const void* A; long lda;
   const void* W; long ldw;
@@ -45,8 +52,11 @@
   int prio;
   int x16;
   const float* cs;
-  const float* rowstats;
+  LnSums rowsums;
+  float ln_eps;
+  LnSums stats_out, stats_clear;
 };
+bool gemm_fuses_stats(int epi, const GemmParams& p);
 
 enum GemmTile {
   TILE_AUTO = 0,
@@ -85,6 +95,7 @@
                             int causal, hipStream_t s);
 
 hipError_t launch_ln_stats(const void* x, int x16, float eps, float* stats, int rows, int D, hipStream_t s);
+hipError_t launch_ln_sums(const void* x16rows, LnSums sums, LnSums clr, int rows, int D, hipStream_t s);
 hipError_t launch_ln_rows(DType dt, const void* x, int x16, const float* w, const float* b, float eps,
                           void* out16, int rows, int D, hipStream_t s, uint8_t* qs = nullptr);
 
@@ -92,12 +103,12 @@
                                   const float* lnpre_w, const float* lnpre_b,
                                   const float* ln1_w, const float* ln1_b, float eps,
                                   void* h, int B, int tokens, int D, hipStream_t s, uint8_t* qs = nullptr,
-                                  float* stats = nullptr);
+                                  float* stats = nullptr, LnSums sums = LnSums(), LnSums clr = LnSums());
 
 hipError_t launch_text_embed_ln(DType dt, const int64_t* ids, const float* tok, const float* pos,
                                 const float* ln1_w, const float* ln1_b, float eps, void* x, int x16,
                                 void* h, int B, int T, int D, int vocab, hipStream_t s, uint8_t* qs = nullptr,
-                                float* stats = nullptr);
+                                float* stats = nullptr, LnSums sums = LnSums(), LnSums clr = LnSums());
 
 hipError_t launch_pool_ln(DType dt, const void* x, int x16, const int64_t* ids, int tokens,
                           const float* w, const float* b, float eps, void* out16, int B, int D,
diff --git a/clip-embedder-rs_amd/csrc/kernels/rowwise.hip b/clip-embedder-rs_amd/csrc/kernels/rowwise.hip
--- a/clip-embedder-rs_amd/csrc/kernels/rowwise.hip
+++ b/clip-embedder-rs_amd/csrc/kernels/rowwise.hip
@@ -59,6 +59,28 @@
   const float var = wave_sum(q) / (float)D;
   mean_out = mean;
   rstd_out = 1.0f / sqrtf(var + eps);
+}
+
+template <int NV>
+__device__ __forceinline__ void ln_sums_regs(const Row<NV>& in, double& sx, double& qhi, double& qlo) {
+  sx = qhi = qlo = 0.0;
+#pragma unroll
+  for (int i = 0; i < NV; ++i) {
+    ln_sums_add((double)in.v[i].x, sx, qhi, qlo);
+    ln_sums_add((double)in.v[i].y, sx, qhi, qlo);
+    ln_sums_add((double)in.v[i].z, sx, qhi, qlo);
+    ln_sums_add((double)in.v[i].w, sx, qhi, qlo);
+  }
+  sx = wave_sum_f64(sx);
+  qhi = wave_sum_f64(qhi);
+  qlo = wave_sum_f64(qlo);
+}
+__device__ __forceinline__ void store_ln_sums(const LnSums& s, const LnSums& clr, long row, int lane, double sx,
+                                              double qhi, double qlo) {
+  if (lane < 3) {
+    s.p[lane * s.ld + row] = lane == 0 ? sx : lane == 1 ? qhi : qlo;
+    if (clr.p != nullptr) clr.p[lane * clr.ld + row] = 0.0;
+  }
 }
 
 template <int NV>
@@ -201,12 +223,34 @@
 }
 
 template <typename T, int NV, typename XT>
+__global__ __launch_bounds__(256) void ln_sums_kernel(const XT* __restrict__ x, LnSums sums, LnSums clr, int rows,
+                                                      int D) {
+  const int stride = gridDim.x * 4, lane = threadIdx.x & 63;
+  int row = blockIdx.x * 4 + (threadIdx.x >> 6);
+  if (row >= rows) return;
+  const int D4 = D >> 2;
+  Row<NV> r;
+  load_row(x + (long)row * D, D4, lane, r);
+  for (;;) {
+    const int next = row + stride;
+    Row<NV> nr;
+    if (next < rows) load_row(x + (long)next * D, D4, lane, nr);
+    double sx, qhi, qlo;
+    ln_sums_regs(r, sx, qhi, qlo);
+    store_ln_sums(sums, clr, row, lane, sx, qhi, qlo);
+    if (next >= rows) break;
+    row = next;
+    r = nr;
+  }
+}
+
+template <typename T, int NV, typename XT>
 __global__ __launch_bounds__(256) void vision_embed_ln_kernel(XT* __restrict__ x, const float* cls,
                                                               const float* pos, const float* lnpre_w,
                                                               const float* lnpre_b, const float* ln1_w,
                                                               const float* ln1_b, float eps, T* __restrict__ h,
                                                               uint8_t* __restrict__ qs, int rows, int tokens, int D,
-                                                              float* __restrict__ stats) {
+                                                              float* __restrict__ stats, LnSums sums, LnSums clr) {
   const int row = blockIdx.x * 4 + (threadIdx.x >> 6), lane = threadIdx.x & 63;
   if (row >= rows) return;
   const int D4 = D >> 2;
@@ -230,6 +274,14 @@
   round_rowx<XT>(y);
   store_rowx(x + (long)row * D, y, D4, lane);
   if (h == nullptr) {
+    if constexpr (!std::is_same<XT, float>::value) {
+      if (sums.p != nullptr) {
+        double sx, qhi, qlo;
+        ln_sums_regs(y, sx, qhi, qlo);
+        store_ln_sums(sums, clr, row, lane, sx, qhi, qlo);
+        return;
+      }
+    }
     float mean, rstd;
     ln_stats_regs(y, eps, D, lane, mean, rstd);
     if (lane == 0) *(float2*)(stats + 2L * row) = make_float2(mean, rstd);
@@ -244,7 +296,8 @@
                                                             const float* pos, const float* ln1_w,
                                                             const float* ln1_b, float eps, XT* __restrict__ x,
                                                             T* __restrict__ h, uint8_t* __restrict__ qs, int rows,
-                                                            int Tctx, int D, int vocab, float* __restrict__ stats) {
+                                                            int Tctx, int D, int vocab, float* __restrict__ stats,
+                                                            LnSums sums, LnSums clr) {
   const int row = blockIdx.x * 4 + (threadIdx.x >> 6), lane = threadIdx.x & 63;
   if (row >= rows) return;
   const int D4 = D >> 2;
@@ -261,6 +314,14 @@
   round_rowx<XT>(e);
   store_rowx(x + (long)row * D, e, D4, lane);
   if (h == nullptr) {
+    if constexpr (!std::is_same<XT, float>::value) {
+      if (sums.p != nullptr) {
+        double sx, qhi, qlo;
+        ln_sums_regs(e, sx, qhi, qlo);
+        store_ln_sums(sums, clr, row, lane, sx, qhi, qlo);
+        return;
+      }
+    }
     float mean, rstd;
     ln_stats_regs(e, eps, D, lane, mean, rstd);
     if (lane == 0) *(float2*)(stats + 2L * row) = make_float2(mean, rstd);
@@ -397,30 +458,50 @@
   return hipGetLastError();
 }
 
+hipError_t launch_ln_sums(const void* x16rows, LnSums sums, LnSums clr, int rows, int D, hipStream_t s) {
+  if (D % 4 || D > 256 * MAXV || D > kLnSumsMaxD || D <= 0 || rows <= 0 || sums.p == nullptr || sums.ld < rows ||
+      (clr.p != nullptr && clr.ld < rows))
+    return hipErrorInvalidValue;
+  dim3 grid = rows_grid(rows);
+  const int cap = device_cus() * 8;
+  if ((int)grid.x > cap) grid.x = cap;
+  CLIPGPU_ROW_LAUNCH_X(ln_sums_kernel, __bf16, _Float16, grid, D, (const _Float16*)x16rows, sums, clr, rows, D);
+  return hipGetLastError();
+}
+
+static bool stem_stats_ok(const void* h, int x16, const float* stats, const LnSums& sums, const LnSums& clr, int rows,
+                          int D) {
+  if (h != nullptr) return sums.p == nullptr && clr.p == nullptr;
+  if (sums.p == nullptr) return stats != nullptr && clr.p == nullptr;
+  return x16 && D <= kLnSumsMaxD && sums.ld >= rows && (clr.p == nullptr || clr.ld >= rows);
+}
+
 hipError_t launch_vision_embed_ln(DType dt, void* x, int x16, const float* cls, const float* pos, const float* lnpre_w,
                                   const float* lnpre_b, const float* ln1_w, const float* ln1_b, float eps,
-                                  void* h, int B, int tokens, int D, hipStream_t s, uint8_t* qs, float* stats) {
-  if (h == nullptr && stats == nullptr) return hipErrorInvalidValue;
+                                  void* h, int B, int tokens, int D, hipStream_t s, uint8_t* qs, float* stats,
+                                  LnSums sums, LnSums clr) {
+  if (!stem_stats_ok(h, x16, stats, sums, clr, B * tokens, D)) return hipErrorInvalidValue;
   if (D % 4 || D > 256 * MAXV || D <= 0 || (qs != nullptr && D % 32)) return hipErrorInvalidValue;
   const int rows = B * tokens;
   dispatch_dx(dt, x16, [&](auto tp_, auto xp_) {
     CLIPGPU_TX_TYPES;
     CLIPGPU_ROW_LAUNCH_X(vision_embed_ln_kernel, T, XT, rows_grid(rows), D, (XT*)x, cls, pos, lnpre_w, lnpre_b, ln1_w,
-                         ln1_b, eps, (T*)h, qs, rows, tokens, D, stats);
+                         ln1_b, eps, (T*)h, qs, rows, tokens, D, stats, sums, clr);
   });
   return hipGetLastError();
 }
 
 hipError_t launch_text_embed_ln(DType dt, const int64_t* ids, const float* tok, const float* pos,
                                 const float* ln1_w, const float* ln1_b, float eps, void* x, int x16, void* h,
-                                int B, int Tctx, int D, int vocab, hipStream_t s, uint8_t* qs, float* stats) {
-  if (h == nullptr && stats == nullptr) return hipErrorInvalidValue;
+                                int B, int Tctx, int D, int vocab, hipStream_t s, uint8_t* qs, float* stats,
+                                LnSums sums, LnSums clr) {
+  if (!stem_stats_ok(h, x16, stats, sums, clr, B * Tctx, D)) return hipErrorInvalidValue;
   if (D % 4 || D > 256 * MAXV || D <= 0 || (qs != nullptr && D % 32)) return hipErrorInvalidValue;
   const int rows = B * Tctx;
   dispatch_dx(dt, x16, [&](auto tp_, auto xp_) {
     CLIPGPU_TX_TYPES;
     CLIPGPU_ROW_LAUNCH_X(text_embed_ln_kernel, T, XT, rows_grid(rows), D, ids, tok, pos, ln1_w, ln1_b, eps, (XT*)x,
-                         (T*)h, qs, rows, Tctx, D, vocab, stats);
+                         (T*)h, qs, rows, Tctx, D, vocab, stats, sums, clr);
   });
   return hipGetLastError();
 }
diff --git a/clip-embedder-rs_amd/csrc/testing.hip b/clip-embedder-rs_amd/csrc/testing.hip
--- a/clip-embedder-rs_amd/csrc/testing.hip
+++ b/clip-embedder-rs_amd/csrc/testing.hip
@@ -107,6 +107,13 @@
   if (!ok) throw ClipErr(CLIPGPU_ERR_INVALID, msg);
 }
 
+void stats_from_sums(const double* d_sums, int64_t ld, int64_t rows, int64_t D, float eps, float* stats) {
+  std::vector<double> h(3 * ld);
+  down(h.data(), d_sums, h.size() * 8);
+  for (int64_t r = 0; r < rows; ++r)
+    ln_sums_finalize(h[r], h[ld + r], h[2 * ld + r], (int)D, eps, stats[2 * r], stats[2 * r + 1]);
+}
+
 }
 
 extern "C" {
@@ -117,7 +124,7 @@
     const DType dt = dt_of(dtype);
     require(rows > 0 && D > 0 && rows * D < INT32_MAX && x && w && b && out && stats && (q == nullptr) == (qs == nullptr),
             "bad LN arguments");
-    DevBuf dx(rows * D * 4), dw(D * 4), db(D * 4), dO(rows * D * 2), dS(rows * 8), dq(rows * D), ds(rows * (D / 32 + 1));
+    DevBuf dx(rows * D * 4), dw(D * 4), db(D * 4), dO(rows * D * 2), dS(rows * 24), dq(rows * D), ds(rows * (D / 32 + 1));
     up_stream(x16, dx.p, x, rows * D);
     up(dw.p, w, D * 4);
     up(db.p, b, D * 4);
@@ -127,10 +134,12 @@
                "launch_ln_rows (MX)");
     launched(launch_ln_rows(dt, dx.p, x16, dw.as<float>(), db.as<float>(), eps, dO.p, (int)rows, (int)D, nullptr),
              "launch_ln_rows");
-    launched(launch_ln_stats(dx.p, x16, eps, dS.as<float>(), (int)rows, (int)D, nullptr), "launch_ln_stats");
+    if (x16) launched(launch_ln_sums(dx.p, LnSums{dS.as<double>(), (long)rows}, LnSums(), (int)rows, (int)D, nullptr), "launch_ln_sums");
+    else launched(launch_ln_stats(dx.p, x16, eps, dS.as<float>(), (int)rows, (int)D, nullptr), "launch_ln_stats");
     HIP_CHECK(hipDeviceSynchronize());
     down16(dt, out, dO.p, rows * D);
-    down(stats, dS.p, rows * 8);
+    if (x16) stats_from_sums(dS.as<double>(), rows, rows, D, eps, stats);
+    else down(stats, dS.p, rows * 8);
     if (qs != nullptr) {
       down(q, dq.p, rows * D);
       down(qs, ds.p, rows * (D / 32));
@@ -142,17 +151,22 @@
 
 namespace {
 template <typename Go>
-void run_stem(DType dt, int x16, int mode, int64_t rows, int64_t D, const void* dx, Go go, const char* what,
+void run_stem(DType dt, int x16, int mode, int64_t rows, int64_t D, float eps, const void* dx, Go go, const char* what,
               float* x_out, float* h_out, float* stats_out, uint8_t* q_out, uint8_t* qs_out) {
   require(mode >= 0 && mode <= 2 && x_out, "bad stem mode");
   require(mode == 0 ? h_out != nullptr : mode == 1 ? stats_out != nullptr : (q_out && qs_out), "missing stem output");
-  DevBuf dH(rows * D * 2), dS(rows * 8), ds(rows * (D / 32 + 1));
-  launched(go(mode == 1 ? nullptr : dH.p, mode == 2 ? ds.as<uint8_t>() : nullptr, mode == 1 ? dS.as<float>() : nullptr),
+  DevBuf dH(rows * D * 2), dS(rows * 24), ds(rows * (D / 32 + 1));
+  const bool sums = mode == 1 && x16;
+  launched(go(mode == 1 ? nullptr : dH.p, mode == 2 ? ds.as<uint8_t>() : nullptr,
+              mode == 1 && !sums ? dS.as<float>() : nullptr, sums ? LnSums{dS.as<double>(), (long)rows} : LnSums()),
            what);
   HIP_CHECK(hipDeviceSynchronize());
   down_stream(x16, x_out, dx, rows * D);
   if (mode == 0) down16(dt, h_out, dH.p, rows * D);
-  if (mode == 1) down(stats_out, dS.p, rows * 8);
+  if (mode == 1) {
+    if (sums) stats_from_sums(dS.as<double>(), rows, rows, D, eps, stats_out);
+    else down(stats_out, dS.p, rows * 8);
+  }
   if (mode == 2) {
     down(q_out, dH.p, rows * D);
     down(qs_out, ds.p, rows * (D / 32));
@@ -175,11 +189,11 @@
     const float* hs[6] = {cls, pos, lnpre_w, lnpre_b, ln1_w, ln1_b};
     DevBuf* dev[6] = {&dc, &dp, &g0, &b0, &g1, &b1};
     for (int i = 0; i < 6; ++i) up(dev[i]->p, hs[i], D * 4);
-    run_stem(dt, x16, mode, rows, D, dx.p,
-             [&](void* h, uint8_t* qs, float* stats) {
+    run_stem(dt, x16, mode, rows, D, eps, dx.p,
+             [&](void* h, uint8_t* qs, float* stats, LnSums sums) {
                return launch_vision_embed_ln(dt, dx.p, x16, dc.as<float>(), dp.as<float>(), g0.as<float>(),
                                              b0.as<float>(), g1.as<float>(), b1.as<float>(), eps, h, (int)B,
-                                             (int)tokens, (int)D, nullptr, qs, stats);
+                                             (int)tokens, (int)D, nullptr, qs, stats, sums);
              },
              "launch_vision_embed_ln", x_out, h_out, stats_out, q_out, qs_out);
   });
@@ -200,11 +214,11 @@
     up(dp.p, pos, npos * D * 4);
     up(g1.p, ln1_w, D * 4);
     up(b1.p, ln1_b, D * 4);
-    run_stem(dt, x16, mode, rows, D, dx.p,
-             [&](void* h, uint8_t* qs, float* stats) {
+    run_stem(dt, x16, mode, rows, D, eps, dx.p,
+             [&](void* h, uint8_t* qs, float* stats, LnSums sums) {
                return launch_text_embed_ln(dt, di.as<int64_t>(), dtok.as<float>(), dp.as<float>(), g1.as<float>(),
                                            b1.as<float>(), eps, dx.p, x16, h, (int)B, (int)T, (int)D, (int)vocab,
-                                           nullptr, qs, stats);
+                                           nullptr, qs, stats, sums);
              },
              "launch_text_embed_ln", x_out, h_out, stats_out, q_out, qs_out);
   });
@@ -348,20 +362,75 @@
     if (M <= 0 || N <= 0 || K <= 0 || K % 64 || N % 4) throw ClipErr(CLIPGPU_ERR_INVALID, "bad GEMM shape");
     if (tile != 0 && tile != TILE_SKINNY && tile != TILE_GENERAL && !gemm_tile_built(tile))
       throw ClipErr(CLIPGPU_ERR_INVALID, "bad tile");
-    DevBuf dA(M * K * 2), dW(N * K * 2), dB(N * 4), dC(N * 4), dO(M * N * 2), dS((M + 256) * 8);
+    DevBuf dA(M * K * 2), dW(N * K * 2), dB(N * 4), dC(N * 4), dO(M * N * 2), dS(3 * (M + 256) * 8);
+    const LnSums sums{dS.as<double>(), (long)M + 256};
     up16(DT_F16, dA.p, x, M * K);
     up16(DT_F16, dW.p, wf, N * K);
     up(dB.p, bias, N * 4);
     up(dC.p, cs, N * 4);
-    HIP_CHECK(launch_ln_stats(dA.p, 1, eps, dS.as<float>(), (int)M, (int)K, nullptr));
+    launched(launch_ln_sums(dA.p, sums, LnSums(), (int)M, (int)K, nullptr), "launch_ln_sums");
     GemmParams g{};
     g.tile = tile;
     g.A = dA.p; g.lda = K; g.W = dW.p; g.ldw = K; g.bias = dB.as<float>(); g.cs = dC.as<float>();
-    g.rowstats = dS.as<float>();
+    g.rowsums = sums;
+    g.ln_eps = eps;
     g.out = dO.p; g.ldo = N; g.M = (int)M; g.N = (int)N; g.K = (int)K;
     HIP_CHECK(launch_gemm(dt, A_ROWS, EPI_LNF, act, g, nullptr));
     HIP_CHECK(hipDeviceSynchronize());
     down16(dt, out, dO.p, M * N);
+  });
+}
+
+int clipgpu_test_gemm_resid_stats(int dtype, int64_t M, int64_t N, int64_t K, const float* A, const float* W,
+                                  const float* bias, const float* resid, int tile, float* x_out, double* sums_gemm,
+                                  double* sums_pass, int* damage, int* fused) {
+  return guarded([&]() {
+    const DType dt = dt_of(dtype);
+    require(M > 0 && N > 0 && K > 0 && K % 64 == 0 && M * N < INT32_MAX && A && W && resid && x_out && sums_gemm &&
+                sums_pass && damage && fused,
+            "bad GEMM arguments");
+    require(tile == 0 || gemm_tile_built(tile), "bad tile");
+    constexpr size_t GUARD = 4096;
+    const size_t ld = (size_t)M + 256, body = 3 * ld * 8;
+    DevBuf dA(M * K * 2), dW(N * K * 2), dB(N * 4), dX(M * N * 2), dS(body + GUARD), dC(body + GUARD), dP(3 * M * 8);
+    HIP_CHECK(hipMemset(dS.p, 0xA5, body + GUARD));
+    HIP_CHECK(hipMemset(dC.p, 0xA5, body + GUARD));
+    for (int c = 0; c < 3; ++c) HIP_CHECK(hipMemset(dS.as<double>() + c * ld, 0, (size_t)M * 8));
+    up16(dt, dA.p, A, M * K);
+    up16(dt, dW.p, W, N * K);
+    if (bias) up(dB.p, bias, N * 4);
+    up16(DT_F16, dX.p, resid, M * N);
+    GemmParams g{};
+    g.tile = tile;
+    g.A = dA.p; g.lda = K; g.W = dW.p; g.ldw = K; g.bias = bias ? dB.as<float>() : nullptr;
+    g.out = dX.p; g.ldo = N; g.M = (int)M; g.N = (int)N; g.K = (int)K;
+    g.x16 = 1;
+    g.stats_out = LnSums{dS.as<double>(), (long)ld};
+    g.stats_clear = LnSums{dC.as<double>(), (long)ld};
+    *fused = gemm_fuses_stats(EPI_RESID, g) ? 1 : 0;
+    const LnSums so = g.stats_out, sc = g.stats_clear;
+    if (!*fused) g.stats_out = g.stats_clear = LnSums();
+    launched(launch_gemm(dt, A_ROWS, EPI_RESID, ACT_NONE, g, nullptr), "launch_gemm");
+    if (!*fused) launched(launch_ln_sums(dX.p, so, sc, (int)M, (int)N, nullptr), "launch_ln_sums (unfused)");
+    launched(launch_ln_sums(dX.p, LnSums{dP.as<double>(), (long)M}, LnSums(), (int)M, (int)N, nullptr), "launch_ln_sums");
+    HIP_CHECK(hipDeviceSynchronize());
+    down16(DT_F16, x_out, dX.p, M * N);
+    down(sums_pass, dP.p, 3 * M * 8);
+    std::vector<uint64_t> hs((body + GUARD) / 8), hc((body + GUARD) / 8);
+    down(hs.data(), dS.p, body + GUARD);
+    down(hc.data(), dC.p, body + GUARD);
+    const uint64_t pat = 0xA5A5A5A5A5A5A5A5ull;
+    int bad = 0;
+    for (int c = 0; c < 3; ++c) {
+      std::memcpy(sums_gemm + (size_t)c * M, hs.data() + c * ld, (size_t)M * 8);
+      for (size_t r = 0; r < ld; ++r) {
+        if (r < (size_t)M && hc[c * ld + r] != 0) bad |= 1;
+        if (r >= (size_t)M && (hc[c * ld + r] != pat || hs[c * ld + r] != pat)) bad |= 2;
+      }
+    }
+    for (size_t i = 3 * ld; i < hs.size(); ++i)
+      if (hs[i] != pat || hc[i] != pat) bad |= 4;
+    *damage = bad;
   });
 }
 
diff --git a/clip-embedder-rs_amd/open_clip_inference/_lib.py b/clip-embedder-rs_amd/open_clip_inference/_lib.py
--- a/clip-embedder-rs_amd/open_clip_inference/_lib.py
+++ b/clip-embedder-rs_amd/open_clip_inference/_lib.py
@@ -73,6 +73,8 @@
     ("clipgpu_test_topk_key", c_int, [c_float, ctypes.c_uint32, POINTER(c_uint64)]),
     ("clipgpu_test_gemm_lnf", c_int, [c_int, c_int, c_int64, c_int64, c_int64, c_void_p, c_void_p, c_void_p,
                                c_void_p, c_float, c_int, c_void_p]),
+    ("clipgpu_test_gemm_resid_stats", c_int, [c_int, c_int64, c_int64, c_int64, c_void_p, c_void_p, c_void_p, c_void_p,
+                                       c_int, c_void_p, c_void_p, c_void_p, c_void_p, c_void_p]),
     ("clipgpu_test_attention", c_int, [c_int, c_int64, c_int64, c_int64, c_int64, c_int, c_void_p, c_void_p]),
     ("clipgpu_test_layernorm", c_int, [c_int, c_int64, c_int64, c_float, c_void_p, c_void_p, c_void_p, c_void_p]),
     ("clipgpu_test_ln_rows", c_int, [c_int, c_int, c_int64, c_int64, c_float] + [c_void_p] * 7),
diff --git a/clip-embedder-rs_amd/open_clip_inference/engine.py b/clip-embedder-rs_amd/open_clip_inference/engine.py
--- a/clip-embedder-rs_amd/open_clip_inference/engine.py
+++ b/clip-embedder-rs_amd/open_clip_inference/engine.py
@@ -15,7 +15,7 @@
                 ("tuning", ctypes.c_int32), ("communicator", ctypes.c_int32),
                 ("graphs", ctypes.c_int32), ("prune_last", ctypes.c_int32), ("trim_text", ctypes.c_int32),
                 ("gemm_tiles", ctypes.c_int32 * 4), ("patch_tile", ctypes.c_int32), ("mx_layers", ctypes.c_uint32),
-                ("residual", ctypes.c_int32), ("ln_fold", ctypes.c_int32)]
+                ("residual", ctypes.c_int32), ("ln_fold", ctypes.c_int32), ("ln_stats", ctypes.c_int32)]
 
 
 def _tristate(v) -> int:
@@ -43,7 +43,8 @@
                  dtype: str = "bf16", max_batch: int = 256, mx_sites=None, lanes: int = 0, tuning=False,
                  communicator: bool = False, graphs: Optional[bool] = None, prune_last: Optional[bool] = None,
                  trim_text: Optional[bool] = None, gemm_tiles: Optional[Sequence[int]] = None, patch_tile: int = 0,
-                 mx_layers=None, residual: Optional[str] = None, ln_fold: Optional[bool] = None):
+                 mx_layers=None, residual: Optional[str] = None, ln_fold: Optional[bool] = None,
+                 ln_stats: Optional[bool] = None):
         self.model_dir = model_dir
         self.tower = tower
         self.devices = list(devices) if devices else [0]
@@ -53,7 +54,7 @@
                      "graphs": graphs, "prune_last": prune_last, "trim_text": trim_text,
                      "gemm_tiles": list(gemm_tiles) if gemm_tiles else None, "patch_tile": int(patch_tile),
                      "mx_layers": mx_layers, "residual": residual,
-                     "ln_fold": ln_fold}
+                     "ln_fold": ln_fold, "ln_stats": ln_stats}
         dt = {"bf16": _lib.DTYPE_BF16, "f16": _lib.DTYPE_F16, "fp16": _lib.DTYPE_F16, "fp8": _lib.DTYPE_FP8}[dtype]
         devs = (c_int * len(self.devices))(*self.devices)
         opts = Options()
@@ -86,6 +87,7 @@
             raise ValueError('residual: "f32" or "f16"')
         opts.residual = {None: 0, "f32": 1, "f16": 2}[residual]
         opts.ln_fold = _tristate(ln_fold)
+        opts.ln_stats = _tristate(ln_stats)
         h = c_void_p()
         check(lib().clipgpu_create_ex(model_dir.encode(), tower, devs, len(self.devices), dt, self.max_batch,
                                       ctypes.byref(opts), ctypes.byref(h)))
diff --git a/include/clipgpu.h b/include/clipgpu.h
--- a/include/clipgpu.h
+++ b/include/clipgpu.h
@@ -52,6 +52,7 @@
   uint32_t mx_layers;
   int32_t residual;
   int32_t ln_fold;
+  int32_t ln_stats;
 } clipgpu_options;
 int clipgpu_options_init(clipgpu_options* opts);
 int clipgpu_create_ex(const char* model_dir, int tower, const int* device_ids, int n_devices, int dtype,
diff --git a/include/clipgpu_testing.h b/include/clipgpu_testing.h
--- a/include/clipgpu_testing.h
+++ b/include/clipgpu_testing.h
@@ -11,6 +11,10 @@
                       const float* W, const float* bias, const float* resid, float* out);
 int clipgpu_test_gemm_lnf(int dtype, int act, int64_t M, int64_t N, int64_t K, const float* x, const float* wf,
                           const float* cs, const float* bias, float eps, int tile, float* out);
+
+int clipgpu_test_gemm_resid_stats(int dtype, int64_t M, int64_t N, int64_t K, const float* A, const float* W,
+                                  const float* bias, const float* resid, int tile, float* x_out, double* sums_gemm,
+                                  double* sums_pass, int* damage, int* fused);
 
 int clipgpu_test_gemm_chunk_rows(int64_t rows);
 
```

Result: slower. 92220 images/s (-1.5%).
